# ShunyuYao/DFA-NeRF

Hardware: AMD Instinct MI355X
Metric: rays/sec (whole node) at 450x450, 64c+128f samples (higher is better)
Workload: dtype f16; 1 GPU; Obama head NeRF inference, 450x450, 64+128 hierarchical (configs[1]); H=450, W=450, n_coarse=64, n_fine=128, fields=1, frames=8, parallelism=single GPU

## Files before the change

### dfa-nerf_amd/csrc/dfn_api.hip

```cpp
#include <hip/hip_runtime.h>
#include <algorithm>
#include <climits>
#include <cstdio>
#include <cstdlib>
#include <cstring>
#include <mutex>
#include <string>
#include <utility>
#include <vector>

#include "dfanerf.h"
#include "dfn_layout.h"
#include "dfn_misc.h"
#include "dfn_mlp.h"
#include "dfn_params.h"
#include "dfn_plan.h"
#include "dfn_signal.h"
#include "dfn_train.h"

using namespace dfn;

namespace {

thread_local std::string g_err;
// ... 927 lines not shown
    if (!kept) return fail(DFN_E_ARG, "dfn_encode_signal_bwd_kept: kept is NULL");
    return encode_signal_bwd_impl(aud_params, exp_params, att_params, auds, exps, n_total, frame, smo_size, d_out, g_aud, g_exp,
                                  g_att, false, stream, kept);
}
int dfn_encode_signal_bwd_set(const float* aud_params, const float* exp_params, const float* att_params, const float* auds,
                              const float* exps, int n_total, int frame, int smo_size, const float* d_out, float* g_aud,
                              float* g_exp, float* g_att, void* stream) {
    return encode_signal_bwd_impl(aud_params, exp_params, att_params, auds, exps, n_total, frame, smo_size, d_out, g_aud, g_exp,
                                  g_att, true, stream);
}

static int encode_signal_torso_bwd_impl(const float* att_params, const float* poses, int pose_stride, int n_total, int frame,
                                        int smo_size, const float* d_out, float* g_att, bool set, void* stream) {
    if (!poses || !d_out || n_total <= 0 || (pose_stride != 12 && pose_stride != 16))
        return fail(DFN_E_ARG, "dfn_encode_signal_torso_bwd: bad argument");
    if (smo_ok(smo_size, "dfn_encode_signal_torso_bwd") != DFN_OK) return DFN_E_ARG;
    if (smo_size == 0) return DFN_OK;
    if (!att_params || !g_att) return fail(DFN_E_ARG, "dfn_encode_signal_torso_bwd: attention buffers missing");
    return launched(launch_encode_signal_torso_bwd(att_params, poses, pose_stride, n_total, frame, smo_size, d_out, g_att, set,
                                                   (hipStream_t)stream), "encode_signal_torso_bwd_kernel");
}
int dfn_encode_signal_torso_bwd(const float* att_params, const float* poses, int pose_stride, int n_total, int frame,
                                int smo_size, const float* d_out, float* g_att, void* stream) {
    return encode_signal_torso_bwd_impl(att_params, poses, pose_stride, n_total, frame, smo_size, d_out, g_att, false, stream);
}
int dfn_encode_signal_torso_bwd_set(const float* att_params, const float* poses, int pose_stride, int n_total, int frame,
                                    int smo_size, const float* d_out, float* g_att, void* stream) {
    return encode_signal_torso_bwd_impl(att_params, poses, pose_stride, n_total, frame, smo_size, d_out, g_att, true, stream);
}

static int decoder_impl(int tier, int width, int field, const void* packed, const float* bias, const float* points, const float* dirs,
                        long n, float* feat, float* sigma, float* samples, void* act_T, uint32_t* masks, const char* what, void* stream) {
    ProgramInfo pi;
    program_info(tier, prog_field(field), &pi, width);
    DecoderArgs A{};
    A.wblob = (const char*)packed;
    A.nslab = pi.n_slabs;
    A.field = prog_field(field);
    A.bias = bias;
    A.n_bias = pi.n_bias;
    A.points = points;
    A.dirs = dirs;
    A.n_points = n;
    A.feat = feat;
    A.sigma = sigma;
    A.samples = samples;
    A.act_T = act_T;
    A.masks = masks;
    return launched(launch_decoder(tier, A, (hipStream_t)stream, width), what);
}

int dfn_decoder_fwd(int tier, int field, const void* packed, const float* bias, const float* points,
                    const float* dirs, long n, float* feat, float* sigma, void* stream) {
    int width;
    if (take_width(tier, width, "dfn_decoder_fwd") != DFN_OK) return DFN_E_ARG;
    if (!tier_ok(tier) || !field_ok(field) || !packed || !bias || !points || !dirs || !feat || !sigma)
        return fail(DFN_E_ARG, "dfn_decoder_fwd: bad argument");
    if (n <= 0) return DFN_OK;
    return decoder_impl(tier, width, field, packed, bias, points, dirs, n, feat, sigma, nullptr, nullptr, nullptr, "decoder_kernel", stream);
}

int dfn_decoder_train_fwd(int tier, int field, const void* packed, const float* bias, const float* points,
                          const float* dirs, long n, float* feat, float* sigma, float* samples, void* act_T,
                          uint32_t* masks, void* stream) {
    if (no_width(tier, "dfn_decoder_train_fwd") != DFN_OK) return DFN_E_ARG;
    if (!train_tier_ok(tier) || !train_field_ok(field) || !packed || !bias || !points ||
        !dirs || !feat || !sigma || !samples || !act_T || !masks)
        return fail(DFN_E_ARG, "dfn_decoder_train_fwd: bad argument (tiers f32 / bf16, fields head / torso / listener)");
    if (n <= 0) return DFN_OK;
    const long NP = (n + 31) / 32 * 32;
    if (dfn_train_rows(1, 0) * NP >= (1L << 32)) return fail(DFN_E_ARG, "dfn_decoder_train_fwd: too many points per call");
    return decoder_impl(tier, 256, field, packed, bias, points, dirs, n, feat, sigma, samples, act_T, masks, "decoder_kernel(train)", stream);
}

int dfn_get_rays(int H, int W, float focal, float cx, float cy, const float* c2w_host, float* rays_o,
                 float* rays_d, void* stream) {
    return dfn_get_rays_strided(H, W, 1, focal, cx, cy, c2w_host, rays_o, rays_d, stream);
}

int dfn_get_rays_strided(int H, int W, int stride, float focal, float cx, float cy, const float* c2w_host, float* rays_o,
                         float* rays_d, void* stream) {
    if (H <= 0 || W <= 0 || stride <= 0 || H / stride <= 0 || W / stride <= 0 || !c2w_host || !rays_o || !rays_d)
        return fail(DFN_E_ARG, "dfn_get_rays: bad argument");
    return launched(launch_get_rays(H, W, stride, focal, cx, cy, c2w_host, rays_o, rays_d, (hipStream_t)stream), "get_rays_kernel");
}

int dfn_ndc_rays(int H, int W, float focal, float z_near, const float* rays_o, const float* rays_d, long n,
                 float* out_o, float* out_d, void* stream) {
    if (!rays_o || !rays_d || !out_o || !out_d || n < 0) return fail(DFN_E_ARG, "dfn_ndc_rays: bad argument");
    if (n == 0) return DFN_OK;
    return launched(launch_ndc_rays(H, W, focal, z_near, rays_o, rays_d, n, out_o, out_d, (hipStream_t)stream), "ndc_rays_kernel");
}

int dfn_sample_pdf(const float* bins, const float* weights, long R, int nb, int ns, const float* u, float* samples,
                   void* stream) {
    if (!bins || !weights || !samples || R < 0 || ns <= 0) return fail(DFN_E_ARG, "dfn_sample_pdf: bad argument");
    if (nb < 2 || nb > 256) return fail(DFN_E_ARG, "dfn_sample_pdf: need 2 <= nb <= 256");
    if (R == 0) return DFN_OK;
    return launched(launch_sample_pdf(bins, weights, R, nb, ns, u, samples, (hipStream_t)stream), "sample_pdf_kernel");
}

int dfn_composite(const float* sigma, const float* feat, int K, long N, float* sigma_sum, float* feat_w,
                  void* stream) {
    if (!sigma || !feat || !sigma_sum || !feat_w || K < 1 || N < 0) return fail(DFN_E_ARG, "dfn_composite: bad argument");
    if (N == 0) return DFN_OK;
    return launched(launch_composite(sigma, feat, K, N, sigma_sum, feat_w, (hipStream_t)stream), "composite_kernel");
}

int dfn_volume_weights(const float* z, const float* ray, const float* sigma, long R, int S, float last_dist,
                       float* weights, void* stream) {
    if (!z || !ray || !sigma || !weights || R < 0) return fail(DFN_E_ARG, "dfn_volume_weights: bad argument");
    if (S < 1 || S > 1024) return fail(DFN_E_ARG, "dfn_volume_weights: need 1 <= S <= 1024");
    if (R == 0) return DFN_OK;
    return launched(launch_volume_weights(z, ray, sigma, R, S, last_dist, weights, (hipStream_t)stream), "volume_weights_kernel");
}

int dfn_composite_grad(const float* sigma, const float* feat, int K, long N, const float* d_sigma_sum, const float* d_feat_w,
                       float* d_sigma, float* d_feat, void* stream) {
    if (!sigma || !feat || !d_sigma || !d_feat || K < 1 || N < 0) return fail(DFN_E_ARG, "dfn_composite_grad: bad argument");
    if (N == 0) return DFN_OK;
    return launched(launch_composite_grad(sigma, feat, K, N, d_sigma_sum, d_feat_w, d_sigma, d_feat, (hipStream_t)stream), "composite_grad_kernel");
}

int dfn_volume_weights_grad(const float* z, const float* ray, const float* sigma, long R, int S, float last_dist,
                            const float* d_weights, float* d_sigma, void* stream) {
    if (!z || !ray || !sigma || !d_weights || !d_sigma || R < 0)
        return fail(DFN_E_ARG, "dfn_volume_weights_grad: bad argument");
    if (S < 1 || S > 1024) return fail(DFN_E_ARG, "dfn_volume_weights_grad: need 1 <= S <= 1024");
    if (R == 0) return DFN_OK;
    return launched(launch_volume_weights_grad(z, ray, sigma, R, S, last_dist, d_weights, d_sigma, (hipStream_t)stream), "volume_weights_grad_kernel");
}

int dfn_to8b(const float* x, long n, uint8_t* out, void* stream) {
    if (!x || !out || n < 0) return fail(DFN_E_ARG, "dfn_to8b: bad argument");
    if (n == 0) return DFN_OK;
    return launched(launch_to8b(x, n, out, (hipStream_t)stream), "to8b_kernel");
}

int dfn_debug_mfma_chain(int tier, int lds_reads_per_2, int valu_per_2, const void* fragments, const void* operands_b, int iters,
                         int blocks, float* out, uint64_t* clock, void* stream) {
    if (no_width(tier, "dfn_debug_mfma_chain") != DFN_OK) return DFN_E_ARG;
    if ((tier != DFN_TIER_BF16 && tier != DFN_TIER_F16) || !fragments || !operands_b || !out || !clock || iters <= 0 || blocks <= 0)
        return fail(DFN_E_ARG, "dfn_debug_mfma_chain: bad argument");
    return launched(launch_mfma_chain(tier == DFN_TIER_F16, lds_reads_per_2, valu_per_2, fragments, operands_b, iters, blocks, out,
                                      (unsigned long long*)clock, (hipStream_t)stream),
                    "mfma_chain_kernel (variants: (0, 0) and (2, 4))");
}

int dfn_debug_clock_probe(uint64_t* probe) {
    g_clock_probe = (unsigned long long*)probe;
    return DFN_OK;
}

int dfn_debug_mfma_layout(float* out, void* stream) {
    if (!out) return fail(DFN_E_ARG, "dfn_debug_mfma_layout: bad argument");
    return launched(launch_mfma_probe(out, (hipStream_t)stream), "mfma_probe_kernel");
}

}
```

### dfa-nerf_amd/csrc/dfn_layout.h

```cpp
#pragma once
#include <stdint.h>
#include "dfn_devguard.h"

#if defined(__HIPCC__)
#define DFN_HD __host__ __device__ inline
#else
#define DFN_HD inline
#endif

namespace dfn {

enum Tier : int { TIER_F32 = 0, TIER_BF16 = 1, TIER_F16 = 2, TIER_F16X3 = 3 };
constexpr int TIER_W128 = 0x200, TIER_MASK = 0xff;
constexpr int TIER_AUX = 0x400;
constexpr int TIER_RAYS = 0x800;
constexpr int TIER_E4M3 = 0x100;
DFN_HD constexpr bool tier_trainable(int tier) { return tier == TIER_F32 || tier == TIER_BF16; }
DFN_HD constexpr bool tier_is16(int tier) { return tier == TIER_BF16 || tier == TIER_F16; }
DFN_HD constexpr bool tier_frag16(int tier) { return tier != TIER_F32; }
DFN_HD constexpr int tier_split(int tier) { return tier == TIER_F16X3 ? 2 : 1; }
DFN_HD int tier_E(int tier) { return tier_frag16(tier) ? 8 : 4; }
DFN_HD int tier_UPT(int tier) { return tier_frag16(tier) ? 2 : 4; }
DFN_HD int tier_elem_bytes(int tier) { return tier_frag16(tier) ? 2 : 4; }
constexpr float SPLIT_SCALE = 2048.0f, SPLIT_INV = 1.0f / 2048.0f;

constexpr int FRAG_BYTES = 1024;
constexpr int SLAB_FRAGS = 32;
constexpr int SLAB_BYTES = SLAB_FRAGS * FRAG_BYTES;

DFN_HD int tile_feat(int h, int r) { return (r & 3) + 8 * (r >> 2) + 4 * h; }
DFN_HD void tile_feat_inv(int f, int* h, int* r) {
    *h = (f >> 2) & 1;
    *r = (f & 3) + 4 * (f >> 3);
}
DFN_HD int kslot_to_slot(int tier, int u, int h, int e) {
    const int E = tier_E(tier), UPT = tier_UPT(tier);
    const int t = u / UPT, r = (u % UPT) * E + e;
    return 32 * t + tile_feat(h, r);
}

constexpr int HID = 256, ZDIM = 256, NPE = 60, NPEV = 24, NSIG = 96, NET = 42, DH = 64;

enum ParamId : int {
    P_DE0_W, P_DE0_B, P_DE1_W, P_DE1_B, P_DE2_W, P_DE2_B, P_DE3_W, P_DE3_B, P_DE4_W, P_DE4_B,
    P_DEO_W, P_DEO_B,
    P_DS0_W, P_DS0_B, P_DS1_W, P_DS1_B, P_DS2_W, P_DS2_B, P_DS3_W, P_DS3_B, P_DS4_W, P_DS4_B,
    P_DSO_W, P_DSO_B,
    P_DESK_W, P_DESK_B, P_DSSK_W, P_DSSK_B,
    P_FCIN_W, P_FCIN_B, P_FCINL_W, P_FCINL_B, P_FCINT_W, P_FCINT_B,
    P_FCZ_W, P_FCZ_B,
    P_BLK0_W, P_BLK0_B, P_BLK1_W, P_BLK1_B, P_BLK2_W, P_BLK2_B, P_BLK3_W, P_BLK3_B,
    P_BLK4_W, P_BLK4_B, P_BLK5_W, P_BLK5_B, P_BLK6_W, P_BLK6_B,
    P_FCZSK_W, P_FCZSK_B, P_FCPSK_W, P_FCPSK_B, P_FCPSKL_W, P_FCPSKL_B, P_FCPSKT_W, P_FCPSKT_B,
    P_SIGMA_W, P_SIGMA_B, P_FCZV_W, P_FCZV_B, P_FEATV_W, P_FEATV_B, P_FCV_W, P_FCV_B,
    P_FEATO_W, P_FEATO_B,
    P_COUNT
};

struct ParamShape { int rows, cols; };

DFN_HD constexpr ParamShape param_shape(int id) {
    switch (id) {
    case P_DE0_W: case P_DS0_W: return {DH, NPE + NET};
    case P_DE1_W: case P_DE2_W: case P_DE3_W: case P_DE4_W:
    case P_DS1_W: case P_DS2_W: case P_DS3_W: case P_DS4_W: return {DH, DH};
    case P_DE0_B: case P_DE1_B: case P_DE2_B: case P_DE3_B: case P_DE4_B:
    case P_DS0_B: case P_DS1_B: case P_DS2_B: case P_DS3_B: case P_DS4_B:
    case P_DESK_B: case P_DSSK_B: return {DH, 1};
    case P_DEO_W: return {NPE, DH};
    case P_DEO_B: return {NPE, 1};
    case P_DSO_W: return {NET, DH};
    case P_DSO_B: return {NET, 1};
    case P_DESK_W: return {DH, NPE};
    case P_DSSK_W: return {DH, NET};
    case P_FCIN_W: case P_FCPSK_W: return {HID, NPE + NSIG};
    case P_FCINL_W: case P_FCPSKL_W: return {HID, NPE};
    case P_FCINT_W: case P_FCPSKT_W: return {HID, NPE + NET};
    case P_FCZ_W: case P_FCZSK_W: case P_FCZV_W: return {HID, ZDIM};
    case P_BLK0_W: case P_BLK1_W: case P_BLK2_W: case P_BLK3_W: case P_BLK4_W: case P_BLK5_W:
    case P_BLK6_W: case P_FEATV_W: return {HID, HID};
    case P_SIGMA_W: return {1, HID};
    case P_SIGMA_B: return {1, 1};
    case P_FCV_W: return {HID, NPEV};
    case P_FEATO_W: return {3, HID};
    case P_FEATO_B: return {3, 1};
    default: return {HID, 1};
    }
}

DFN_HD constexpr int param_numel(int id) { return param_shape(id).rows * param_shape(id).cols; }
struct ParamOffsets { int v[P_COUNT + 1]; };
DFN_HD constexpr ParamOffsets make_param_offsets() {
    ParamOffsets t = {};
    int off = 0;
    for (int i = 0; i < P_COUNT; ++i) {
        t.v[i] = off;
        off += param_numel(i);
    }
    t.v[P_COUNT] = off;
    return t;
}
DFN_HD constexpr int param_offset(int id) {
    constexpr ParamOffsets T = make_param_offsets();
    return T.v[id];
}
static_assert(make_param_offsets().v[P_COUNT] == 955242, "flat decoder parameter count");
constexpr int N_DECODER_PARAMS = 955242;

DFN_HD int pe_slot_to_ref(int slot) { return slot < NPE ? slot : -1; }
DFN_HD int view_slot_to_ref(int slot) { return slot < NPEV ? slot : -1; }

enum Field : int { FIELD_HEAD = 0, FIELD_TORSO = 1 };

struct ProgramInfo {
    int n_frags;
    int n_slabs;
    int n_bias;
};

}
```

### dfa-nerf_amd/csrc/dfn_misc.h

```cpp
#pragma once
#include <hip/hip_runtime.h>
#include "dfanerf.h"

namespace dfn {
struct PrepareJobs {
    const float* params;
    int tier;
    const int* plan[4]; void* out[4]; long n[4]; int pack_blocks[4];
    const float* sig[2]; const float* zs[2]; const float* za[2]; float* bias[2]; int nb[2]; int fold_blocks[2];
};
hipError_t launch_prepare(PrepareJobs J, hipStream_t st);
hipError_t launch_pack(const int* plan, const float* params, void* out, long n, int tier, hipStream_t st);
hipError_t launch_fold_bwd(int field, const float* params, const float* sig, const float* zs, const float* za,
                           const float* dbias, float* grad_flat, float* dsig, int n, hipStream_t st);
hipError_t launch_fold_bwd_sig(int field, const float* params, const float* dbias, float* dsig, bool overwrite,
                               hipStream_t st);
int sig_term_elements(int field, int* out);
hipError_t launch_fold(int field, const float* params, const float* sig, const float* zs, const float* za,
                       float* out, int n, hipStream_t st);
hipError_t launch_get_rays(int H, int W, int stride, float focal, float cx, float cy, const float* c2w_host, float* ro,
                           float* rd, hipStream_t st);
hipError_t launch_ndc_rays(int H, int W, float focal, float z_near, const float* ro, const float* rd, long n,
                           float* oo, float* od, hipStream_t st);
hipError_t launch_sample_pdf(const float* bins, const float* weights, long R, int nb, int ns, const float* u,
                             float* out, hipStream_t st);
hipError_t launch_composite(const float* sigma, const float* feat, int K, long N, float* ssum, float* fw,
                            hipStream_t st);
hipError_t launch_volume_weights(const float* z, const float* ray, const float* sigma, long R, int S,
                                 float last_dist, float* w, hipStream_t st);
hipError_t launch_composite_grad(const float* sigma, const float* feat, int K, long N, const float* d_ssum, const float* d_fw,
                                 float* d_sigma, float* d_feat, hipStream_t st);
hipError_t launch_volume_weights_grad(const float* z, const float* ray, const float* sigma, long R, int S, float last_dist,
                                      const float* d_w, float* d_sigma, hipStream_t st);
hipError_t launch_zero_words(unsigned* p, long n, hipStream_t st);
hipError_t launch_mfma_chain(bool f16, int lds2, int valu2, const void* frags, const void* b, int iters, int blocks, float* out,
                             unsigned long long* clk, hipStream_t st);
hipError_t launch_to8b(const float* x, long n, unsigned char* out, hipStream_t st);
hipError_t launch_mfma_probe(float* out, hipStream_t st);
hipError_t launch_adam_multi(const DfnAdamItem* items, const void* chunks, int n_chunks, float lr, double beta1, double beta2,
                             float eps, float bias_c1, float bias_c2_sqrt, hipStream_t st);
}
```

### dfa-nerf_amd/csrc/dfn_misc.hip

```cpp
#include <hip/hip_runtime.h>
#include <algorithm>
#include <hip/hip_bf16.h>
#include "dfn_layout.h"
#include "dfn_mlp.h"
#include "dfn_misc.h"

namespace dfn {

__device__ __forceinline__ void pack_body(const int* __restrict__ plan, const float* __restrict__ params, void* out, long n,
                                          int tier, long i) {
    if (i >= n) return;
    const int src = plan[i];
    const float v = src >= 0 ? params[src] : 0.f;
    if (tier == TIER_BF16) ((__bf16*)out)[i] = (__bf16)v;
    else if (tier == TIER_F16) ((_Float16*)out)[i] = (_Float16)v;
    else if (tier == TIER_F16X3) {
        const _Float16 hi = (_Float16)v;
        ((_Float16*)out)[i] = ((i >> 9) & 1) ? (_Float16)((v - (float)hi) * SPLIT_SCALE) : hi;
    } else ((float*)out)[i] = v;
}
__global__ void pack_kernel(const int* __restrict__ plan, const float* __restrict__ params, void* out, long n,
                            int tier) {
    pack_body(plan, params, out, n, tier, (long)blockIdx.x * blockDim.x + threadIdx.x);
}
// ... 510 lines not shown
            B = b + f * B;
            F = f * F;
        }
    }
    float sF = F, sB = B;
    for (int d = 1; d < 64; d <<= 1) {
        const float oF = __shfl_down(sF, d), oB = __shfl_down(sB, d);
        if (lane + d < 64) { sB = sB + sF * oB; sF = sF * oF; }
    }
    float G = __shfl_down(sB, 1);
    if (lane == 63) G = 0.f;
    for (int k = per < 16 ? per - 1 : 15; k >= 0; --k) {
        const int s = s0 + k;
        if (s < S) {
            const float T = exc * pre[k];
            const float d_alpha = T * (gw[k] - G);
            d_sigma[r * S + s] = sigma[r * S + s] > 0.f ? d_alpha * dist[k] * ex[k] : 0.f;
            G = gw[k] * alpha[k] + __fadd_rn(__fsub_rn(1.0f, alpha[k]), 1e-10f) * G;
        }
    }
}
hipError_t launch_volume_weights_grad(const float* z, const float* ray, const float* sigma, long R, int S, float last_dist,
                                      const float* d_w, float* d_sigma, hipStream_t st) {
    hipLaunchKernelGGL(volume_weights_grad_kernel, dim3((unsigned)((R + 3) / 4)), dim3(256), 0, st, z, ray, sigma, R, S,
                       last_dist, d_w, d_sigma);
    return hipGetLastError();
}

__global__ void zero_words_kernel(unsigned* p, long n) {
    const long n4 = n >> 2;
    uint4* q = (uint4*)p;
    for (long i = (long)blockIdx.x * blockDim.x + threadIdx.x; i < n4; i += (long)gridDim.x * blockDim.x) q[i] = make_uint4(0, 0, 0, 0);
    if (blockIdx.x == 0 && threadIdx.x < (n & 3)) p[(n4 << 2) + threadIdx.x] = 0;
}
hipError_t launch_zero_words(unsigned* p, long n, hipStream_t st) {
    const long n4 = n >> 2;
    const int blocks = (int)std::min<long>(1024, std::max<long>(1, (n4 + 255) / 256));
    hipLaunchKernelGGL(zero_words_kernel, dim3(blocks), dim3(256), 0, st, p, n);
    return hipGetLastError();
}

typedef unsigned pc_u32x4 __attribute__((ext_vector_type(4)));
typedef __bf16 pc_bf16x8 __attribute__((ext_vector_type(8)));
typedef _Float16 pc_f16x8 __attribute__((ext_vector_type(8)));
template <bool F16, int LDS2, int VALU2>
__global__ __launch_bounds__(512) void mfma_chain_kernel(const pc_u32x4* __restrict__ frag_src, const pc_u32x4* __restrict__ b_src,
                                                         int iters, float* out, unsigned long long* clk) {
    extern __shared__ pc_u32x4 pc_slab[];
    const int lane = threadIdx.x & 63;
    for (int i = threadIdx.x; i < 32 * 64; i += 512) pc_slab[i] = frag_src[i];
    __syncthreads();
    pc_u32x4 b[4];
    for (int k = 0; k < 4; ++k) b[k] = b_src[(threadIdx.x * 4 + k) & 4095];
    f32x16 acc0 = {}, acc1 = {};
    pc_u32x4 a0 = pc_slab[lane], a1 = pc_slab[64 + lane];
    unsigned e0 = b[0][0], e1 = b[1][1], e2 = b[2][2], e3 = b[3][3];
    const unsigned long long c0 = __builtin_readcyclecounter(), r0 = __builtin_amdgcn_s_memrealtime();
    for (int it = 0; it < iters; ++it) {
#pragma unroll
        for (int k = 0; k < 16; ++k) {
            const int f = (2 * k) % 32;
            if (LDS2 >= 1) a0 = pc_slab[f * 64 + lane];
            if (LDS2 >= 2) a1 = pc_slab[(f + 1) * 64 + lane];
            if constexpr (F16) {
                acc0 = __builtin_amdgcn_mfma_f32_32x32x16_f16(__builtin_bit_cast(pc_f16x8, a0), __builtin_bit_cast(pc_f16x8, b[k & 3]), acc0, 0, 0, 0);
                acc1 = __builtin_amdgcn_mfma_f32_32x32x16_f16(__builtin_bit_cast(pc_f16x8, a1), __builtin_bit_cast(pc_f16x8, b[(k + 1) & 3]), acc1, 0, 0, 0);
            } else {
                acc0 = __builtin_amdgcn_mfma_f32_32x32x16_bf16(__builtin_bit_cast(pc_bf16x8, a0), __builtin_bit_cast(pc_bf16x8, b[k & 3]), acc0, 0, 0, 0);
                acc1 = __builtin_amdgcn_mfma_f32_32x32x16_bf16(__builtin_bit_cast(pc_bf16x8, a1), __builtin_bit_cast(pc_bf16x8, b[(k + 1) & 3]), acc1, 0, 0, 0);
            }
#pragma unroll
            for (int v = 0; v < VALU2; ++v) {
                unsigned& x = (v & 3) == 0 ? e0 : (v & 3) == 1 ? e1 : (v & 3) == 2 ? e2 : e3;
                if (v & 1) asm volatile("v_pk_max_i16 %0, %1, %2" : "=v"(x) : "v"(x), "v"(e0 ^ e2));
                else asm volatile("v_cvt_pk_bf16_f32 %0, %1, %2" : "=v"(x) : "v"(__builtin_bit_cast(float, x)), "v"(__builtin_bit_cast(float, x ^ 0x3f800000u)));
            }
        }
    }
    const unsigned long long c1 = __builtin_readcyclecounter(), r1 = __builtin_amdgcn_s_memrealtime();
    float sum = 0.f;
    for (int r = 0; r < 16; ++r) sum += acc0[r] + acc1[r];
    out[blockIdx.x * blockDim.x + threadIdx.x] = sum + (float)(e0 ^ e1 ^ e2 ^ e3);
    if (blockIdx.x == gridDim.x / 2 && threadIdx.x == 0) { clk[0] = c1 - c0; clk[1] = r1 - r0; }
}
hipError_t launch_mfma_chain(bool f16, int lds2, int valu2, const void* frags, const void* b, int iters, int blocks, float* out,
                             unsigned long long* clk, hipStream_t st) {
    constexpr int lds = 150 * 1024;
#define PC_GO(F, L, V)                                                                                                        \
    {                                                                                                                         \
        hipError_t e = hipFuncSetAttribute((const void*)mfma_chain_kernel<F, L, V>, hipFuncAttributeMaxDynamicSharedMemorySize, lds); \
        if (e != hipSuccess) return e;                                                                                        \
        hipLaunchKernelGGL((mfma_chain_kernel<F, L, V>), dim3(blocks), dim3(512), lds, st, (const pc_u32x4*)frags,              \
                           (const pc_u32x4*)b, iters, out, clk);                                                              \
        return hipGetLastError();                                                                                             \
    }
    if (lds2 == 0 && valu2 == 0) { if (f16) PC_GO(true, 0, 0) else PC_GO(false, 0, 0) }
    if (lds2 == 2 && valu2 == 4) { if (f16) PC_GO(true, 2, 4) else PC_GO(false, 2, 4) }
    if (lds2 == 1 && valu2 == 4) { if (f16) PC_GO(true, 1, 4) else PC_GO(false, 1, 4) }
    if (lds2 == 0 && valu2 == 4) { if (f16) PC_GO(true, 0, 4) else PC_GO(false, 0, 4) }
    if (lds2 == 2 && valu2 == 0) { if (f16) PC_GO(true, 2, 0) else PC_GO(false, 2, 0) }
    if (lds2 == 1 && valu2 == 2) { if (f16) PC_GO(true, 1, 2) else PC_GO(false, 1, 2) }
    if (lds2 == 2 && valu2 == 2) { if (f16) PC_GO(true, 2, 2) else PC_GO(false, 2, 2) }
#undef PC_GO
    return hipErrorInvalidValue;
}

__global__ void to8b_kernel(const float* x, long n, unsigned char* out) {
    const long i = (long)blockIdx.x * blockDim.x + threadIdx.x;
    if (i >= n) return;
    const float v = fminf(fmaxf(x[i], 0.f), 1.f);
    out[i] = (unsigned char)(int)__fmul_rn(255.0f, v);
}
hipError_t launch_to8b(const float* x, long n, unsigned char* out, hipStream_t st) {
    hipLaunchKernelGGL(to8b_kernel, dim3((unsigned)((n + 255) / 256)), dim3(256), 0, st, x, n, out);
    return hipGetLastError();
}

__global__ void mfma_probe_kernel(float* out) {
    const int lane = threadIdx.x, i = lane & 31, h = lane >> 5;
    {
        bf16x8 a, b;
        for (int e = 0; e < 8; ++e) {
            a[e] = (__bf16)((h == 1 && e == 5) ? (float)(i + 1) : 0.f);
            b[e] = (__bf16)((h == 1 && e == 5) ? (float)(2 * i + 1) : 0.f);
        }
        f32x16 c;
        for (int r = 0; r < 16; ++r) c[r] = 0.f;
        c = __builtin_amdgcn_mfma_f32_32x32x16_bf16(a, b, c, 0, 0, 0);
        for (int r = 0; r < 16; ++r) out[(tile_feat(h, r)) * 32 + i] = c[r];
    }
    {
        const float a = (h == 1) ? (float)(i + 1) : 0.f, b = (h == 1) ? (float)(2 * i + 1) : 0.f;
        f32x16 c;
        for (int r = 0; r < 16; ++r) c[r] = 0.f;
        c = __builtin_amdgcn_mfma_f32_32x32x2f32(a, b, c, 0, 0, 0);
        for (int r = 0; r < 16; ++r) out[1024 + (tile_feat(h, r)) * 32 + i] = c[r];
    }
    {
        f16x8 a, b;
        for (int e = 0; e < 8; ++e) {
            a[e] = (_Float16)((h == 1 && e == 5) ? (float)(i + 1) : 0.f);
            b[e] = (_Float16)((h == 1 && e == 5) ? (float)(2 * i + 1) : 0.f);
        }
        f32x16 c;
        for (int r = 0; r < 16; ++r) c[r] = 0.f;
        c = __builtin_amdgcn_mfma_f32_32x32x16_f16(a, b, c, 0, 0, 0);
        for (int r = 0; r < 16; ++r) out[2048 + (tile_feat(h, r)) * 32 + i] = c[r];
    }
}
hipError_t launch_mfma_probe(float* out, hipStream_t st) {
    hipLaunchKernelGGL(mfma_probe_kernel, dim3(1), dim3(64), 0, st, out);
    return hipGetLastError();
}


__global__ __launch_bounds__(256) void adam_multi_kernel(const DfnAdamItem* items, const int2* chunks, float lr, float beta2,
                                                          float om_beta1, float om_beta2, float eps, float bias_c1,
                                                          float bias_c2_sqrt) {
    const int2 ch = chunks[blockIdx.x];
    const DfnAdamItem it = items[ch.x];
    const long i0 = (long)ch.y * DFN_ADAM_CHUNK;
    const long i1 = (i0 + DFN_ADAM_CHUNK < it.n) ? i0 + DFN_ADAM_CHUNK : it.n;
    const float step_size = lr / bias_c1;
    for (long i = i0 + threadIdx.x; i < i1; i += 256) {
        const float g = it.grad[i];
        float m = it.exp_avg[i], v = it.exp_avg_sq[i];
        m = m + (g - m) * om_beta1;
        v = beta2 * v + om_beta2 * g * g;
        const float denom = sqrtf(v) / bias_c2_sqrt + eps;
        it.param[i] -= step_size * m / denom;
        it.exp_avg[i] = m;
        it.exp_avg_sq[i] = v;
    }
}
hipError_t launch_adam_multi(const DfnAdamItem* items, const void* chunks, int n_chunks, float lr, double beta1, double beta2,
                             float eps, float bias_c1, float bias_c2_sqrt, hipStream_t st) {
    if (n_chunks <= 0) return hipSuccess;
    hipLaunchKernelGGL(adam_multi_kernel, dim3(n_chunks), dim3(256), 0, st, items, (const int2*)chunks, lr, (float)beta2,
                       (float)(1.0 - beta1), (float)(1.0 - beta2), eps, bias_c1, bias_c2_sqrt);
    return hipGetLastError();
}

}
```

### dfa-nerf_amd/csrc/dfn_mlp.h

```cpp
#pragma once
#include <hip/hip_runtime.h>
#include <type_traits>
#include "dfn_layout.h"

namespace dfn {

typedef float f32x16 __attribute__((ext_vector_type(16)));
typedef float f32x4 __attribute__((ext_vector_type(4)));
typedef __bf16 bf16x8 __attribute__((ext_vector_type(8)));
typedef _Float16 f16x8 __attribute__((ext_vector_type(8)));
typedef unsigned u32x4 __attribute__((ext_vector_type(4)));

#define DFN_DEV __device__ __forceinline__
#ifndef DFN_ASM_FETCH
#define DFN_ASM_FETCH 1
#endif
#define DFN_LDS __attribute__((address_space(3)))
typedef DFN_LDS char lds_char;
typedef const __attribute__((address_space(1))) char gchar_c;
typedef DFN_LDS float lds_f32;
typedef DFN_LDS f32x4 lds_f32x4;
typedef DFN_LDS u32x4 lds_u32x4;

template <int TIER> struct TierCfg;
template <> struct TierCfg<TIER_BF16> {
    static constexpr int E = 8, UPT = 2, WAVES = 8, THREADS = 512, LOADS_PER_SLAB = 4;
};
template <> struct TierCfg<TIER_F16> : TierCfg<TIER_BF16> {};
template <> struct TierCfg<TIER_F32> {
    static constexpr int E = 4, UPT = 4, WAVES = 4, THREADS = 256, LOADS_PER_SLAB = 8;
};
template <> struct TierCfg<TIER_F16X3> {
    static constexpr int E = 8, UPT = 2, WAVES = 4, THREADS = 256, LOADS_PER_SLAB = 8;
};

constexpr int RING_SLOTS = 3;
constexpr int RING_BYTES = RING_SLOTS * SLAB_BYTES;

template <int TIER, int NT> struct Vec;
template <int NT> struct Vec<TIER_BF16, NT> {
    bf16x8 u[2 * NT];
    DFN_DEV void set(int L, float x) { u[L >> 3][L & 7] = (__bf16)x; }
    DFN_DEV float get(int L) const { return (float)u[L >> 3][L & 7]; }
};
template <int NT> struct Vec<TIER_F16, NT> {
    f16x8 u[2 * NT];
    DFN_DEV void set(int L, float x) { u[L >> 3][L & 7] = (_Float16)x; }
    DFN_DEV float get(int L) const { return (float)u[L >> 3][L & 7]; }
};
template <int NT> struct Vec<TIER_F32, NT> {
    float v[16 * NT];
    DFN_DEV void set(int L, float x) { v[L] = x; }
    DFN_DEV float get(int L) const { return v[L]; }
};
template <int NT> struct Vec<TIER_F16X3, NT> {
    f16x8 u[2 * NT];
    f16x8 l[2 * NT];
    DFN_DEV void set(int L, float x) {
        const _Float16 hi = (_Float16)x;
        u[L >> 3][L & 7] = hi;
        l[L >> 3][L & 7] = (_Float16)((x - (float)hi) * SPLIT_SCALE);
    }
    DFN_DEV float get(int L) const { return (float)u[L >> 3][L & 7] + (float)l[L >> 3][L & 7] * SPLIT_INV; }
};

struct Stream {
    const char* base0;
    const char* base1;
    int nslab0, nslab1;
    unsigned sched;
    const char* pf_ptr;
    int pf_left;
    int pass;
    const char* next_ptr;
    int next_left;
    unsigned pf_slot;
    unsigned rd_off;
    unsigned rd_slot;
    unsigned rd_vaddr;
    int pf_owed;
#ifdef DFN_TIMING
    unsigned long long t_wait, t_bar, t_issue, t_epi;
#endif
};

template <int TIER, bool ASM = false>
DFN_DEV void stream_issue_piece(const Stream& s, lds_char* ring, int wave, int lane, int k) {
    using C = TierCfg<TIER>;
    const int f = k * C::WAVES + wave;
    if constexpr (ASM) {
        const unsigned dst = __builtin_amdgcn_readfirstlane((unsigned)(unsigned long)ring + s.pf_slot * SLAB_BYTES +
                                                            (unsigned)f * FRAG_BYTES);
        const gchar_c* sb = (const gchar_c*)(s.pf_ptr + f * FRAG_BYTES);
        const unsigned voff = (unsigned)lane * 16u;
        asm volatile("s_mov_b32 m0, %2\n\ts_nop 0\n\tglobal_load_lds_dwordx4 %0, %1" ::"v"(voff), "s"(sb), "s"(dst) : "memory", "m0");
    } else {
        __builtin_amdgcn_global_load_lds(
            (const __attribute__((address_space(1))) void*)(s.pf_ptr + (size_t)lane * 16 + f * FRAG_BYTES),
            (DFN_LDS void*)(ring + s.pf_slot * SLAB_BYTES + f * FRAG_BYTES), 16, 0, 0);
    }
}
DFN_DEV void stream_cursor_next(Stream& s) {
    s.pf_slot = (s.pf_slot + 1 == RING_SLOTS) ? 0u : s.pf_slot + 1;
    const int left = s.pf_left - 1;
    const bool wrap = left == 0;
    s.pf_ptr = wrap ? s.next_ptr : s.pf_ptr + SLAB_BYTES;
    s.pf_left = wrap ? s.next_left : left;
}
DFN_DEV void stream_pass_begin(Stream& s) {
    const int np = s.pass + 1;
    const int f = (np < 32) ? ((s.sched >> np) & 1u) : 0;
    s.next_ptr = f ? s.base1 : s.base0;
    s.next_left = f ? s.nslab1 : s.nslab0;
    s.pass = np;
}
template <int TIER, bool ASM = false>
DFN_DEV void stream_issue(Stream& s, lds_char* ring, int wave, int lane) {
#pragma unroll
    for (int k = 0; k < TierCfg<TIER>::LOADS_PER_SLAB; ++k) stream_issue_piece<TIER, ASM>(s, ring, wave, lane, k);
    stream_cursor_next(s);
}
template <int TIER, bool ASM = false>
DFN_DEV void stream_flush(Stream& s, lds_char* ring, int wave, int lane) {
    constexpr int L = TierCfg<TIER>::LOADS_PER_SLAB;
    if (s.pf_owed > 0) {
        for (int k = L - s.pf_owed; k < L; ++k) stream_issue_piece<TIER, ASM>(s, ring, wave, lane, k);
        stream_cursor_next(s);
        s.pf_owed = 0;
    }
}

template <int TIER, bool ASM = false>
DFN_DEV void stream_begin(Stream& s, lds_char* ring, int wave, int lane) {
    s.pf_ptr = s.base0;
    s.pf_left = s.nslab0;
    s.pass = 0;
    s.next_ptr = s.base0;
    s.next_left = s.nslab0;
    s.pf_slot = 0;
    s.rd_slot = RING_SLOTS - 1;
    s.rd_off = 0;
    s.rd_vaddr = 0;
    s.pf_owed = 0;
    stream_issue<TIER, ASM>(s, ring, wave, lane);
    stream_issue<TIER, ASM>(s, ring, wave, lane);
}

template <int TIER>
DFN_DEV void slab_advance(Stream& s, lds_char* ring, int wave, int lane) {
    using C = TierCfg<TIER>;
#ifdef DFN_TIMING
    const unsigned long long t0 = __builtin_readcyclecounter();
#endif
#ifdef DFN_EXP_VMCNT
    asm volatile("s_waitcnt vmcnt(%0) lgkmcnt(0)" ::"n"(DFN_EXP_VMCNT) : "memory");
#else
    asm volatile("s_waitcnt vmcnt(%0) lgkmcnt(0)" ::"n"(C::LOADS_PER_SLAB) : "memory");
#endif
#ifdef DFN_TIMING
    const unsigned long long t1 = __builtin_readcyclecounter();
#endif
    __builtin_amdgcn_s_barrier();
    asm volatile("" ::: "memory");
#ifdef DFN_TIMING
    const unsigned long long t2 = __builtin_readcyclecounter();
    s.t_wait += t1 - t0; s.t_bar += t2 - t1;
#endif
    s.rd_slot = (s.rd_slot + 1 == RING_SLOTS) ? 0u : s.rd_slot + 1;
    s.rd_off = s.rd_slot * SLAB_BYTES;
    s.rd_vaddr = (unsigned)(unsigned long)ring + (unsigned)lane * 16u + s.rd_off;
    s.pf_owed += C::LOADS_PER_SLAB;
}

struct Rec {
    void* act_T;
    unsigned* masks;
    int rows;
    long pass;
    int mask_dwords;
};

template <bool REC, bool ASMF = false, bool ASMD = false, bool PIPE = false, bool ACT4 = false> struct CtxT {
    static constexpr bool rec_on = REC;
    static constexpr bool act_fp4 = ACT4;
#ifndef DFN_TRAIN_ASMF
#define DFN_TRAIN_ASMF 1
#endif
    static constexpr bool asm_fetch = (ASMF || (REC && DFN_TRAIN_ASMF != 0)) && (!REC || DFN_TRAIN_ASMF != 0) && (DFN_ASM_FETCH != 0);
    static constexpr bool asm_dma = asm_fetch || ASMD;
    static constexpr bool pipe = PIPE && !REC;
    lds_char* ring;
    int wave, lane, half;
    Rec rec;
};
typedef CtxT<false> Ctx;

template <int TIER> struct ActT;
template <> struct ActT<TIER_BF16> { typedef __bf16 type; };
template <> struct ActT<TIER_F16> { typedef _Float16 type; };
template <> struct ActT<TIER_F32> { typedef float type; };

typedef __attribute__((address_space(1))) char gchar;
DFN_DEV gchar* uniform_ptr(const void* p) {
    const unsigned long v = (unsigned long)p;
    const unsigned lo = __builtin_amdgcn_readfirstlane((unsigned)v), hi = __builtin_amdgcn_readfirstlane((unsigned)(v >> 32));
    return (gchar*)(((unsigned long)hi << 32) | lo);
}
#define DFN_GSTORE(INSN, TAIL, ubase, voff, off, x)                                                                            \
    do {                                                                                                                       \
        gchar* ub_ = (ubase) + ((off) & ~4095);                                                                                \
        asm volatile(INSN " %0, %1, %2 offset:%3" TAIL ::"v"(voff), "v"(x), "s"(ub_), "n"((off) & 4095));                      \
    } while (0)
#define DFN_GSTORE_B32_NT(ubase, voff, off, x) DFN_GSTORE("global_store_dword", " nt", ubase, voff, off, x)
#define DFN_GSTORE_B32(ubase, voff, off, x) DFN_GSTORE("global_store_dword", "", ubase, voff, off, x)
#define DFN_GSTORE_B64_NT(ubase, voff, off, x) DFN_GSTORE("global_store_dwordx2", " nt", ubase, voff, off, x)
#define DFN_GSTORE_B128_NT(ubase, voff, off, x) DFN_GSTORE("global_store_dwordx4", " nt\n\ts_nop 1", ubase, voff, off, x)

#ifndef DFN_DPP_ASM
#define DFN_DPP_ASM 1
#endif
constexpr int REC8_SCALE_BYTES = 128;
DFN_HD constexpr long rec8_tile_bytes(int rows) { return (long)rows * 32 + REC8_SCALE_BYTES; }
DFN_HD constexpr int act_row_bytes(bool fp4) { return fp4 ? 16 : 32; }
DFN_HD constexpr long act_tile_bytes(int rows, bool fp4) { return (long)rows * act_row_bytes(fp4) + REC8_SCALE_BYTES; }
struct Q8 {
    float scale;
    unsigned e8;
};
typedef unsigned short u16x2 __attribute__((ext_vector_type(2)));
typedef __bf16 bf16x2_q __attribute__((ext_vector_type(2)));
template <int NT, bool NONNEG = false, bool FP4 = false> DFN_DEV Q8 q8_of_tiles(const Vec<TIER_BF16, NT>& v, int t0, int n) {
    typedef unsigned u32x4_ __attribute__((ext_vector_type(4)));
    u16x2 m4[4] = {{0, 0}, {0, 0}, {0, 0}, {0, 0}};
#pragma unroll
    for (int t = 0; t < NT; ++t)
        if (t >= t0 && t < t0 + n)
#pragma unroll
            for (int h = 0; h < 2; ++h) {
                const u32x4_ q = __builtin_bit_cast(u32x4_, v.u[2 * t + h]);
#pragma unroll
                for (int e = 0; e < 4; ++e) {
                    const unsigned a = NONNEG ? q[e] : q[e] & 0x7fff7fffu;
                    m4[e] = __builtin_elementwise_max(m4[e], __builtin_bit_cast(u16x2, a));
                }
            }
    const u16x2 m = __builtin_elementwise_max(__builtin_elementwise_max(m4[0], m4[1]), __builtin_elementwise_max(m4[2], m4[3]));
    unsigned x = max((unsigned)m[0], (unsigned)m[1]);
#if !DFN_DPP_ASM
    x = max(x, (unsigned)__builtin_amdgcn_update_dpp((int)x, (int)x, 0xB1, 0xf, 0xf, false));
    x = max(x, (unsigned)__builtin_amdgcn_update_dpp((int)x, (int)x, 0x4E, 0xf, 0xf, false));
    x = max(x, (unsigned)__builtin_amdgcn_update_dpp((int)x, (int)x, 0x141, 0xf, 0xf, false));
    x = max(x, (unsigned)__builtin_amdgcn_update_dpp((int)x, (int)x, 0x140, 0xf, 0xf, false));
#else
    asm("s_nop 1\n\tv_max_u32_dpp %0, %0, %0 quad_perm:[1,0,3,2] row_mask:0xf bank_mask:0xf\n\t"
        "s_nop 1\n\tv_max_u32_dpp %0, %0, %0 quad_perm:[2,3,0,1] row_mask:0xf bank_mask:0xf\n\t"
        "s_nop 1\n\tv_max_u32_dpp %0, %0, %0 row_half_mirror row_mask:0xf bank_mask:0xf\n\t"
        "s_nop 1\n\tv_max_u32_dpp %0, %0, %0 row_mirror row_mask:0xf bank_mask:0xf\n\ts_nop 0"
        : "+v"(x));
#endif
    const unsigned a = max(max((unsigned)__builtin_amdgcn_readlane((int)x, 0), (unsigned)__builtin_amdgcn_readlane((int)x, 16)),
                           max((unsigned)__builtin_amdgcn_readlane((int)x, 32), (unsigned)__builtin_amdgcn_readlane((int)x, 48)));
    const unsigned E = a >> 7;
    Q8 q;
#ifdef DFN_REC8_NOAMAX
    q.e8 = 120u;
    q.scale = __builtin_bit_cast(float, q.e8 << 23);
    return q;
#endif
    if constexpr (FP4) {
        const unsigned e = E + ((a & 0x7fu) > 64u ? 1u : 0u);
        q.e8 = e > 3u ? e - 2u : 1u;
    } else {
        q.e8 = E > 8u ? E - 7u : 1u;
    }
    q.scale = __builtin_bit_cast(float, q.e8 << 23);
    return q;
}
template <int NT, class CT>
DFN_DEV void store_tile4(void* arr, int rows, long tile, int row0, const Vec<TIER_BF16, NT>& v, int t, int t_first, const Q8& q,
                         const CT& c) {
    typedef unsigned u32x4_ __attribute__((ext_vector_type(4)));
    typedef unsigned u32x2_ __attribute__((ext_vector_type(2)));
    u32x2_ out;
#pragma unroll
    for (int k = 0; k < 2; ++k) {
        const u32x4_ w = __builtin_bit_cast(u32x4_, v.u[2 * t + k]);
        const unsigned w0 = w[0], w1 = w[1], w2 = w[2], w3 = w[3];
        unsigned o = 0;
        o = __builtin_amdgcn_cvt_scalef32_pk_fp4_bf16(o, __builtin_bit_cast(bf16x2_q, w0), q.scale, 0);
        o = __builtin_amdgcn_cvt_scalef32_pk_fp4_bf16(o, __builtin_bit_cast(bf16x2_q, w1), q.scale, 1);
        o = __builtin_amdgcn_cvt_scalef32_pk_fp4_bf16(o, __builtin_bit_cast(bf16x2_q, w2), q.scale, 2);
        o = __builtin_amdgcn_cvt_scalef32_pk_fp4_bf16(o, __builtin_bit_cast(bf16x2_q, w3), q.scale, 3);
        out[k] = o;
    }
#ifdef DFN_REC8_NOSTORE
    asm volatile("" ::"v"(out));
    return;
#endif
    gchar* ubase = uniform_ptr((char*)arr + tile * act_tile_bytes(rows, true) + (long)row0 * 16);
    const unsigned voff = (unsigned)((c.lane & 31) * 16 + c.half * 8);
    DFN_GSTORE_B64_NT(ubase, voff, (t - t_first) * 512, out);
}
template <int NT, class CT>
DFN_DEV void store_tile_act(void* arr, int rows, long tile, int row0, const Vec<TIER_BF16, NT>& v, int t, int t_first, const Q8& q,
                            const CT& c);
template <class CT>
DFN_DEV void store_scale_act(void* arr, int rows, long tile, int row0, int t0, int t_first, int n, const Q8& q, const CT& c) {
    gchar* sb = uniform_ptr((char*)arr + tile * act_tile_bytes(rows, CT::act_fp4) + (long)rows * act_row_bytes(CT::act_fp4) + (row0 >> 5) + (t0 - t_first));
    if (c.lane < n) *(__attribute__((address_space(1))) unsigned char*)(sb + c.lane) = (unsigned char)q.e8;
}
template <int NT, class CT>
DFN_DEV void store_tile8(void* arr, int rows, long tile, int row0, const Vec<TIER_BF16, NT>& v, int t, int t_first, const Q8& q,
                         const CT& c) {
    typedef unsigned u32x4_ __attribute__((ext_vector_type(4)));
    typedef short s16x2_ __attribute__((ext_vector_type(2)));
    u32x4_ out;
#pragma unroll
    for (int k = 0; k < 4; ++k) {
        const u32x4_ w = __builtin_bit_cast(u32x4_, v.u[2 * t + (k >> 1)]);
        const unsigned w_lo = w[2 * (k & 1)], w_hi = w[2 * (k & 1) + 1];
        s16x2_ o;
        o = __builtin_amdgcn_cvt_scalef32_pk_fp8_bf16(o, __builtin_bit_cast(bf16x2_q, w_lo), q.scale, false);
        o = __builtin_amdgcn_cvt_scalef32_pk_fp8_bf16(o, __builtin_bit_cast(bf16x2_q, w_hi), q.scale, true);
        out[k] = __builtin_bit_cast(unsigned, o);
    }
#ifdef DFN_REC8_NOSTORE
    asm volatile("" ::"v"(out));
    return;
#endif
    gchar* ubase = uniform_ptr((char*)arr + tile * rec8_tile_bytes(rows) + (long)row0 * 32);
    const unsigned voff = (unsigned)((c.lane & 31) * 32 + c.half * 16);
    DFN_GSTORE_B128_NT(ubase, voff, (t - t_first) * 1024, out);
}
template <class CT>
DFN_DEV void store_scale8(void* arr, int rows, long tile, int row0, int t0, int t_first, int n, const Q8& q, const CT& c) {
    gchar* sb = uniform_ptr((char*)arr + tile * rec8_tile_bytes(rows) + (long)rows * 32 + (row0 >> 5) + (t0 - t_first));
    if (c.lane < n) *(__attribute__((address_space(1))) unsigned char*)(sb + c.lane) = (unsigned char)q.e8;
}
template <int NT, class CT>
DFN_DEV void store_tile_act(void* arr, int rows, long tile, int row0, const Vec<TIER_BF16, NT>& v, int t, int t_first, const Q8& q,
                            const CT& c) {
    if constexpr (CT::act_fp4) store_tile4<NT>(arr, rows, tile, row0, v, t, t_first, q, c);
    else store_tile8<NT>(arr, rows, tile, row0, v, t, t_first, q, c);
}
template <int TIER, int NT, class CT, bool ACT = false>
DFN_DEV void store_tiles_T(void* arr, int rows, long tile, int row0, const Vec<TIER, NT>& v, int t0, int n, const CT& c) {
    typedef typename ActT<TIER>::type T;
    gchar* ubase = uniform_ptr((T*)arr + (tile * rows + row0) * 32);
    if constexpr (TIER == TIER_BF16) {
#pragma unroll
        for (int t = 0; t < NT; t += 2)
            if (t >= t0 && t < t0 + n) {
                const int np = (t + 1 < t0 + n && t + 1 < NT) ? 2 : 1;
                const Q8 q = q8_of_tiles<NT, false, ACT && CT::act_fp4>(v, t, np);
                if constexpr (ACT) store_scale_act(arr, rows, tile, row0, t, t0, np, q, c);
                else store_scale8(arr, rows, tile, row0, t, t0, np, q, c);
#pragma unroll
                for (int k = 0; k < 2; ++k)
                    if (k < np && t + k < NT) {
                        if constexpr (ACT) store_tile_act<NT>(arr, rows, tile, row0, v, t + k, t0, q, c);
                        else store_tile8<NT>(arr, rows, tile, row0, v, t + k, t0, q, c);
                    }
            }
    } else {
#ifdef DFN_REC32_NOSTORE
        return;
#endif
#pragma unroll
        for (int L = 0; L < 16 * NT; ++L)
            if ((L >> 4) >= t0 && (L >> 4) < t0 + n) {
                const int f = 32 * ((L >> 4) - t0) + tile_feat(0, L & 15);
                const unsigned voff = (unsigned)(4 * c.half * 32 + (c.lane & 31)) * (unsigned)sizeof(T);
                if constexpr (sizeof(T) == 4) {
                    const float x = v.get(L);
                    DFN_GSTORE_B32_NT(ubase, voff, f * 128, x);
                } else {
                    __builtin_nontemporal_store((T)v.get(L), (__attribute__((address_space(1))) T*)(ubase + f * 32 * (int)sizeof(T) + voff));
                }
            }
    }
}
template <int TIER, int NT, class CT, bool ACT = false>
DFN_DEV void store_vec_T(void* arr, int rows, long tile, int row0, const Vec<TIER, NT>& v, const CT& c) {
    store_tiles_T<TIER, NT, CT, ACT>(arr, rows, tile, row0, v, 0, NT, c);
}
template <int TIER, int NT, class CT>
DFN_DEV void rec_vec(const CT& c, int row0, const Vec<TIER, NT>& v) {
    if constexpr (!CT::rec_on) return;
    else store_vec_T<TIER, NT, CT, true>(c.rec.act_T, c.rec.rows, c.rec.pass, row0, v, c);
}

template <class CT>
DFN_DEV void store_val_T32(void* arr, int rows, long tile, int row0, int L, float x, const CT& c) {
#ifdef DFN_REC32_NOSTORE
    return;
#endif
    gchar* ubase = uniform_ptr((float*)arr + (tile * rows + row0) * 32);
    const int f = 32 * (L >> 4) + tile_feat(0, L & 15);
    const unsigned voff = (unsigned)(4 * c.half * 32 + (c.lane & 31)) * 4u;
    DFN_GSTORE_B32_NT(ubase, voff, f * 128, x);
}

#ifndef DFN_TRUNK_UNROLL
#define DFN_TRUNK_UNROLL 0
#endif
#ifndef DFN_PF_DEPTH
#define DFN_PF_DEPTH 4
#endif
constexpr int PF_DEPTH = DFN_PF_DEPTH;
template <int TIER, class CT> constexpr bool use_asm_fetch() { return tier_is16(TIER) && CT::asm_fetch; }
#ifndef DFN_F32_PIN_FRAGS
#define DFN_F32_PIN_FRAGS 1
#endif
#ifndef DFN_X3_PIN_FRAGS
#define DFN_X3_PIN_FRAGS 1
#endif
#ifndef DFN_F32_ASM_DMA
#define DFN_F32_ASM_DMA 1
#endif
template <int TIER, class CT> constexpr bool use_asm_dma() { return tier_is16(TIER) ? CT::asm_dma : (DFN_F32_ASM_DMA != 0 || CT::asm_dma); }

#define DFN_FRAG_CASE(K)                                                                                      \
    case K:                                                                                                   \
        asm volatile("ds_read_b128 %0, %1 offset:%2" : "=v"(dst) : "v"(vaddr), "n"((K) * FRAG_BYTES) : "memory"); \
        break;
DFN_DEV void frag_read(u32x4& dst, unsigned vaddr, int pos) {
    switch (pos) {
        DFN_FRAG_CASE(0) DFN_FRAG_CASE(1) DFN_FRAG_CASE(2) DFN_FRAG_CASE(3) DFN_FRAG_CASE(4) DFN_FRAG_CASE(5)
        DFN_FRAG_CASE(6) DFN_FRAG_CASE(7) DFN_FRAG_CASE(8) DFN_FRAG_CASE(9) DFN_FRAG_CASE(10) DFN_FRAG_CASE(11)
        DFN_FRAG_CASE(12) DFN_FRAG_CASE(13) DFN_FRAG_CASE(14) DFN_FRAG_CASE(15) DFN_FRAG_CASE(16) DFN_FRAG_CASE(17)
        DFN_FRAG_CASE(18) DFN_FRAG_CASE(19) DFN_FRAG_CASE(20) DFN_FRAG_CASE(21) DFN_FRAG_CASE(22) DFN_FRAG_CASE(23)
        DFN_FRAG_CASE(24) DFN_FRAG_CASE(25) DFN_FRAG_CASE(26) DFN_FRAG_CASE(27) DFN_FRAG_CASE(28) DFN_FRAG_CASE(29)
        DFN_FRAG_CASE(30) DFN_FRAG_CASE(31)
        default: __builtin_unreachable();
    }
}
#undef DFN_FRAG_CASE
DFN_DEV void frag_wait(u32x4& r, int younger) {
    switch (younger) {
        case 0: asm volatile("s_waitcnt lgkmcnt(0)" : "+v"(r)); break;
        case 1: asm volatile("s_waitcnt lgkmcnt(1)" : "+v"(r)); break;
        case 2: asm volatile("s_waitcnt lgkmcnt(2)" : "+v"(r)); break;
        case 3: asm volatile("s_waitcnt lgkmcnt(3)" : "+v"(r)); break;
        case 4: asm volatile("s_waitcnt lgkmcnt(4)" : "+v"(r)); break;
        case 5: asm volatile("s_waitcnt lgkmcnt(5)" : "+v"(r)); break;
        case 6: asm volatile("s_waitcnt lgkmcnt(6)" : "+v"(r)); break;
        default: asm volatile("s_waitcnt lgkmcnt(7)" : "+v"(r)); break;
    }
}
static_assert(PF_DEPTH >= 1 && PF_DEPTH <= 8, "frag_wait covers up to 7 younger reads");
static_assert((PF_DEPTH & (PF_DEPTH - 1)) == 0, "PF_DEPTH must be a power of two");

struct NoHook { DFN_DEV void operator()() const {} };
struct NoSide { DFN_DEV void operator()(int) const {} };

template <int TIER> struct Fetch {
    u32x4 buf[PF_DEPTH];
    template <class CT> DFN_DEV void load(int slot, int fp, Stream& s, const CT& c) { load(slot, fp, s, c, NoHook{}); }
    template <class CT, class H> DFN_DEV void load(int slot, int fp, Stream& s, const CT& c, H&& hook) {
        using C = TierCfg<TIER>;
        constexpr int GAP = SLAB_FRAGS / C::LOADS_PER_SLAB;
        if (fp % SLAB_FRAGS == 0) {
            slab_advance<TIER>(s, c.ring, c.wave, c.lane);
            hook();
        }
        if constexpr (use_asm_fetch<TIER, CT>()) frag_read(buf[slot], s.rd_vaddr, fp % SLAB_FRAGS);
        else buf[slot] = *(const lds_u32x4*)(c.ring + c.lane * 16 + s.rd_off + (fp % SLAB_FRAGS) * FRAG_BYTES);
#ifdef DFN_EXP_DBLLDS
        {
            const u32x4 dup = *(const volatile lds_u32x4*)(c.ring + c.lane * 16 + s.rd_off + ((fp + 1) % SLAB_FRAGS) * FRAG_BYTES);
            asm volatile("" ::"v"(dup));
        }
#endif
        if (fp % GAP == GAP / 2) {
            const int k = (fp % SLAB_FRAGS) / GAP;
            stream_issue_piece<TIER, use_asm_dma<TIER, CT>()>(s, c.ring, c.wave, c.lane, k);
            --s.pf_owed;
            if (k == C::LOADS_PER_SLAB - 1) stream_cursor_next(s);
        }
    }
    template <class CT> DFN_DEV void prime(Stream& s, const CT& c) {
        stream_flush<TIER, use_asm_dma<TIER, CT>()>(s, c.ring, c.wave, c.lane);
        stream_pass_begin(s);
#pragma unroll
        for (int i = 0; i < PF_DEPTH; ++i) load(i, i, s, c);
    }
};

template <int TIER, int G, int KU, int NTB, int TAIL = -1, class CT, class H = NoHook, class SD = NoSide>
DFN_DEV void gemm_group(f32x16 (&acc)[G], const Vec<TIER, NTB>& b, int& f, Fetch<TIER>& fe, Stream& s,
                        const CT& c, H&& hook = H{}, SD&& side = SD{}) {
    if constexpr (TIER == TIER_F16X3) {
        constexpr int D = PF_DEPTH;
        f32x16 accx[G];
#pragma unroll
        for (int g = 0; g < G; ++g)
#pragma unroll
            for (int r = 0; r < 16; ++r) accx[g][r] = 0.f;
#pragma unroll
        for (int ku = 0; ku < KU; ++ku) {
#pragma unroll
            for (int g = 0; g < G; ++g) {
                const int left = ((KU - ku) * G - g) * 2 - 1;
                const u32x4 ah = fe.buf[f % D];
                if (TAIL < 0 || left + TAIL >= D) fe.load(f % D, f + D, s, c, hook);
                ++f;
                const u32x4 al = fe.buf[f % D];
                if (TAIL < 0 || left - 1 + TAIL >= D) fe.load(f % D, f + D, s, c, hook);
                ++f;
                const f16x8 wh = __builtin_bit_cast(f16x8, ah), wl = __builtin_bit_cast(f16x8, al);
                acc[g] = __builtin_amdgcn_mfma_f32_32x32x16_f16(wh, b.u[ku], acc[g], 0, 0, 0);
                accx[g] = __builtin_amdgcn_mfma_f32_32x32x16_f16(wh, b.l[ku], accx[g], 0, 0, 0);
                accx[g] = __builtin_amdgcn_mfma_f32_32x32x16_f16(wl, b.u[ku], accx[g], 0, 0, 0);
#ifdef DFN_GEMM_SCHEDBAR
                __builtin_amdgcn_sched_barrier(DFN_GEMM_SCHEDBAR);
#else
                if constexpr (!CT::rec_on && (DFN_X3_PIN_FRAGS != 0)) __builtin_amdgcn_sched_barrier(0);
#endif
            }
            side(ku);
#ifdef DFN_PIPE_SCHEDBAR
            if constexpr (!std::is_same<typename std::decay<SD>::type, NoSide>::value) __builtin_amdgcn_sched_barrier(0);
#endif
        }
#pragma unroll
        for (int g = 0; g < G; ++g)
#pragma unroll
            for (int r = 0; r < 16; ++r) acc[g][r] = __builtin_fmaf(accx[g][r], SPLIT_INV, acc[g][r]);
    } else {
#pragma unroll
        for (int ku = 0; ku < KU; ++ku) {
#pragma unroll
            for (int g = 0; g < G; ++g) {
                const int left = (KU - ku) * G - g - 1;
                constexpr bool ASM = use_asm_fetch<TIER, CT>();
                if constexpr (ASM) {
                    const int after = (TAIL < 0) ? PF_DEPTH : left + TAIL;
                    frag_wait(fe.buf[f % PF_DEPTH], after < PF_DEPTH - 1 ? after : PF_DEPTH - 1);
                }
                const u32x4 a = fe.buf[f % PF_DEPTH];
                if constexpr (!ASM) {
                    if (TAIL < 0 || left + TAIL >= PF_DEPTH) fe.load(f % PF_DEPTH, f + PF_DEPTH, s, c, hook);
                }
                if constexpr (TIER == TIER_BF16) {
                    acc[g] = __builtin_amdgcn_mfma_f32_32x32x16_bf16(__builtin_bit_cast(bf16x8, a), b.u[ku],
                                                                     acc[g], 0, 0, 0);
                } else if constexpr (TIER == TIER_F16) {
                    acc[g] = __builtin_amdgcn_mfma_f32_32x32x16_f16(__builtin_bit_cast(f16x8, a), b.u[ku],
                                                                    acc[g], 0, 0, 0);
                } else {
                    const f32x4 af = __builtin_bit_cast(f32x4, a);
#pragma unroll
                    for (int e = 0; e < 4; ++e)
                        acc[g] = __builtin_amdgcn_mfma_f32_32x32x2f32(af[e], b.v[4 * ku + e], acc[g], 0, 0, 0);
                }
                if constexpr (ASM) {
                    if (TAIL < 0 || left + TAIL >= PF_DEPTH) fe.load(f % PF_DEPTH, f + PF_DEPTH, s, c, hook);
                }
#ifdef DFN_GEMM_SCHEDBAR
                if constexpr (!ASM) __builtin_amdgcn_sched_barrier(DFN_GEMM_SCHEDBAR);
#else
                if constexpr (!ASM && TIER == TIER_F32 && !CT::rec_on && (DFN_F32_PIN_FRAGS != 0)) __builtin_amdgcn_sched_barrier(0);
#endif
                ++f;
            }
            side(ku);
#ifdef DFN_PIPE_SCHEDBAR
            if constexpr (!std::is_same<typename std::decay<SD>::type, NoSide>::value) __builtin_amdgcn_sched_barrier(0);
#endif
        }
    }
}

DFN_DEV float relu_(float x) { return __builtin_bit_cast(float, max(__builtin_bit_cast(int, x), 0)); }

template <int G>
DFN_DEV void acc_init(f32x16 (&acc)[G], const lds_f32* bias_lds, int half) {
#ifdef DFN_EXP_NOINIT
#pragma unroll
    for (int g = 0; g < G; ++g)
#pragma unroll
        for (int r = 0; r < 16; ++r) acc[g][r] = 0.f;
    return;
#endif
#pragma unroll
    for (int g = 0; g < G; ++g) {
        const lds_f32x4* p = (const lds_f32x4*)(bias_lds + g * 32 + half * 16);
#pragma unroll
        for (int q = 0; q < 4; ++q) {
            const f32x4 v = p[q];
#pragma unroll
            for (int e = 0; e < 4; ++e) acc[g][4 * q + e] = v[e];
        }
    }
}
template <int G>
DFN_DEV void acc_relu_add(f32x16 (&acc)[G], const lds_f32* bias_lds, int half) {
#pragma unroll
    for (int g = 0; g < G; ++g) {
        const lds_f32x4* p = (const lds_f32x4*)(bias_lds + g * 32 + half * 16);
#pragma unroll
        for (int q = 0; q < 4; ++q) {
            const f32x4 v = p[q];
#pragma unroll
            for (int e = 0; e < 4; ++e) acc[g][4 * q + e] = relu_(acc[g][4 * q + e]) + v[e];
        }
    }
}
typedef short s16x2 __attribute__((ext_vector_type(2)));
typedef __bf16 bf16x2 __attribute__((ext_vector_type(2)));
typedef float f32x2 __attribute__((ext_vector_type(2)));
typedef _Float16 f16x2 __attribute__((ext_vector_type(2)));
template <int TIER, int G, int NT, bool RELU>
DFN_DEV void acc_to_vec(const f32x16 (&acc)[G], Vec<TIER, NT>& v, int t0) {
#ifdef DFN_EXP_NOEPI
    {
#pragma unroll
        for (int g = 0; g < G; ++g) v.set(16 * (t0 + g), acc[g][0]);
        return;
    }
#endif
    if constexpr (tier_is16(TIER)) {
        typedef typename std::conditional<TIER == TIER_F16, f16x2, bf16x2>::type pk2;
        typedef typename std::conditional<TIER == TIER_F16, f16x8, bf16x8>::type pk8;
#pragma unroll
        for (int g = 0; g < G; ++g) {
#pragma unroll
            for (int h = 0; h < 2; ++h) {
                unsigned w[4];
#pragma unroll
                for (int e = 0; e < 4; ++e) {
                    const f32x2 x = {acc[g][8 * h + 2 * e], acc[g][8 * h + 2 * e + 1]};
                    const pk2 pk = __builtin_convertvector(x, pk2);
                    if constexpr (RELU) {
                        const s16x2 m = __builtin_elementwise_max(__builtin_bit_cast(s16x2, pk), (s16x2)(0));
                        w[e] = __builtin_bit_cast(unsigned, m);
                    } else {
                        w[e] = __builtin_bit_cast(unsigned, pk);
                    }
                }
                const u32x4 q = {w[0], w[1], w[2], w[3]};
                v.u[2 * (t0 + g) + h] = __builtin_bit_cast(pk8, q);
            }
        }
    } else if constexpr (TIER == TIER_F16X3) {
#pragma unroll
        for (int g = 0; g < G; ++g) {
#pragma unroll
            for (int h = 0; h < 2; ++h) {
                unsigned wh[4], wl[4];
#pragma unroll
                for (int e = 0; e < 4; ++e) {
                    f32x2 x = {acc[g][8 * h + 2 * e], acc[g][8 * h + 2 * e + 1]};
                    if constexpr (RELU) x = f32x2{relu_(x[0]), relu_(x[1])};
                    const f16x2 hi = __builtin_convertvector(x, f16x2);
                    const f32x2 d = (x - __builtin_convertvector(hi, f32x2)) * SPLIT_SCALE;
                    const f16x2 lo = __builtin_convertvector(d, f16x2);
                    wh[e] = __builtin_bit_cast(unsigned, hi);
                    wl[e] = __builtin_bit_cast(unsigned, lo);
                }
                const u32x4 qh = {wh[0], wh[1], wh[2], wh[3]}, ql = {wl[0], wl[1], wl[2], wl[3]};
                v.u[2 * (t0 + g) + h] = __builtin_bit_cast(f16x8, qh);
                v.l[2 * (t0 + g) + h] = __builtin_bit_cast(f16x8, ql);
            }
        }
    } else {
#pragma unroll
        for (int g = 0; g < G; ++g)
#pragma unroll
            for (int r = 0; r < 16; ++r) {
                const float x = RELU ? relu_(acc[g][r]) : acc[g][r];
                v.set(16 * (t0 + g) + r, x);
            }
    }
}

template <int TIER, int NT, class CT>
DFN_DEV void rec_vals(const CT& c, int row0, const Vec<TIER, NT>& out, int t0) {
    if constexpr (CT::rec_on)
        if (row0 >= 0) store_tiles_T<TIER, NT, CT, true>(c.rec.act_T, c.rec.rows, c.rec.pass, row0, out, t0, 2, c);
}
DFN_HD constexpr int mask_pos(int b) { return ((b & 1) << 4) | (b >> 1); }
template <class CT>
DFN_DEV void rec_mask_pair(const CT& c, int mask_dword, const f32x16 (&acc)[2]) {
#ifdef DFN_REC_NOMASK
    return;
#endif
    if constexpr (CT::rec_on) {
        if (mask_dword >= 0) {
            unsigned bits = 0;
#pragma unroll
            for (int b = 0; b < 32; ++b) bits |= (acc[b >> 4][b & 15] > 0.f) ? (1u << mask_pos(b)) : 0u;
            gchar* mb = uniform_ptr(c.rec.masks + ((long)c.rec.pass * c.rec.mask_dwords + mask_dword) * 64);
            DFN_GSTORE_B32(mb, (unsigned)c.lane * 4u, 0, bits);
        }
    }
}

template <int TIER, int NT, class CT>
DFN_DEV void rec_mask_pair_packed(const CT& c, int mask_dword, const Vec<TIER, NT>& out, int t0) {
#ifdef DFN_REC_NOMASK
    return;
#endif
    if constexpr (CT::rec_on && tier_is16(TIER)) {
        if (mask_dword >= 0) {
            typedef unsigned u32x4_ __attribute__((ext_vector_type(4)));
            unsigned b2[2] = {0, 0};
#pragma unroll
            for (int k = 0; k < 4; ++k) {
                const u32x4_ q = __builtin_bit_cast(u32x4_, out.u[2 * t0 + k]);
#pragma unroll
                for (int e = 0; e < 4; ++e) {
                    const unsigned w = q[e];
                    unsigned t;
                    asm("v_pk_min_u16 %0, %1, %2" : "=v"(t) : "v"(w), "s"(0x00010001u));
                    asm("v_lshl_or_b32 %0, %1, %2, %0" : "+v"(b2[e & 1]) : "v"(t), "n"(4 * k + e));
                }
            }
            const unsigned bits = b2[0] | b2[1];
#ifdef DFN_REC_NOMASKSTORE
            asm volatile("" ::"v"(bits));
            return;
#endif
            gchar* mb = uniform_ptr(c.rec.masks + ((long)c.rec.pass * c.rec.mask_dwords + mask_dword) * 64);
            DFN_GSTORE_B32(mb, (unsigned)c.lane * 4u, 0, bits);
        }
    }
}

template <int TIER, int NT, bool RELU>
DFN_DEV void epi_word(const f32x16 (&acc)[2], Vec<TIER, NT>& v, int t0, int w) {
    typedef typename std::conditional<TIER == TIER_F16, f16x2, bf16x2>::type pk2;
    typedef typename std::conditional<TIER == TIER_F16, f16x8, bf16x8>::type pk8;
    const int g = w >> 3, h = (w >> 2) & 1, e = w & 3;
    const f32x2 x = {acc[g][8 * h + 2 * e], acc[g][8 * h + 2 * e + 1]};
    const pk2 pk = __builtin_convertvector(x, pk2);
    unsigned word;
    if constexpr (RELU) word = __builtin_bit_cast(unsigned, __builtin_elementwise_max(__builtin_bit_cast(s16x2, pk), (s16x2)(0)));
    else word = __builtin_bit_cast(unsigned, pk);
    u32x4 q = __builtin_bit_cast(u32x4, v.u[2 * (t0 + g) + h]);
    q[e] = word;
    v.u[2 * (t0 + g) + h] = __builtin_bit_cast(pk8, q);
}
DFN_DEV void init_quad(f32x16 (&acc)[2], const lds_f32* bias_lds, int half, int q) {
    const int g = q >> 2, qq = q & 3;
    const f32x4 v = ((const lds_f32x4*)(bias_lds + g * 32 + half * 16))[qq];
#pragma unroll
    for (int e = 0; e < 4; ++e) acc[g][4 * qq + e] = v[e];
}
template <int TIER, int OT, int KU, bool RELU> struct PipeSide {
    static constexpr int ES = KU / 2 > 0 ? KU / 2 : 1, WPS = (16 + ES - 1) / ES;
    static constexpr int BS = KU - ES > 0 ? KU - ES : 1, QPS = (8 + BS - 1) / BS;
    f32x16 (&other)[2];
    Vec<TIER, OT>& out;
    const lds_f32* bias_next;
    int t_prev;
    int half;
    DFN_DEV void operator()(int ku) const {
        if (t_prev >= 0 && ku < ES) {
#pragma unroll
            for (int w = 0; w < WPS; ++w)
                if (ku * WPS + w < 16) epi_word<TIER, OT, RELU>(other, out, t_prev, ku * WPS + w);
        }
        if (bias_next && ku >= ES) {
#pragma unroll
            for (int q = 0; q < QPS; ++q)
                if ((ku - ES) * QPS + q < 8) init_quad(other, bias_next, half, (ku - ES) * QPS + q);
        }
    }
};
template <int TIER, int OT, int KU, int NTB, bool RELU, class CT>
DFN_DEV void layer_pipe(Vec<TIER, OT>& out, const Vec<TIER, NTB>& in, const lds_f32* bias, int& f, Fetch<TIER>& fe,
                        Stream& s, const CT& c) {
    static_assert(OT % 2 == 0 && KU >= 2, "tile pairs");
    f32x16 acc[2][2];
    acc_init<2>(acc[0], bias, c.half);
#pragma unroll
    for (int tg = 0; tg < OT / 2; ++tg) {
        const int cur = tg & 1;
        const PipeSide<TIER, OT, KU, RELU> side = {acc[cur ^ 1], out, tg + 1 < OT / 2 ? bias + (tg + 1) * 64 : nullptr,
                                                   tg > 0 ? 2 * (tg - 1) : -1, c.half};
        gemm_group<TIER, 2, KU, NTB>(acc[cur], in, f, fe, s, c, NoHook{}, side);
        if (KU - PipeSide<TIER, OT, KU, RELU>::ES < 1 && tg + 1 < OT / 2) acc_init<2>(acc[cur ^ 1], bias + (tg + 1) * 64, c.half);
    }
    acc_to_vec<TIER, 2, OT, RELU>(acc[(OT / 2 - 1) & 1], out, OT - 2);
}

#ifndef DFN_REC_SPREAD
#define DFN_REC_SPREAD 1
#endif
template <int TIER, int OT, int KU, class CT, bool NONNEG> struct RecSide {
    const CT& c;
    const Vec<TIER, OT>& out;
    int rec_row, prev;
    mutable Q8 q;
    static constexpr int S0 = KU > 1 ? 1 : 0, S1 = KU > 2 ? 1 + (KU - 1) / 2 : S0;
    DFN_DEV void operator()(int ku) const {
        if constexpr (CT::rec_on && TIER == TIER_BF16) {
            if (prev < 0 || rec_row < 0) return;
            if (ku == 0) {
                q = q8_of_tiles<OT, NONNEG, CT::act_fp4>(out, 2 * prev, 2);
                store_scale_act(c.rec.act_T, c.rec.rows, c.rec.pass, rec_row, 2 * prev, 0, 2, q, c);
            }
            if (ku == S0) store_tile_act<OT>(c.rec.act_T, c.rec.rows, c.rec.pass, rec_row, out, 2 * prev, 0, q, c);
            if (ku == S1) store_tile_act<OT>(c.rec.act_T, c.rec.rows, c.rec.pass, rec_row, out, 2 * prev + 1, 0, q, c);
        }
    }
};

#ifndef DFN_REC32_SPREAD
#define DFN_REC32_SPREAD 1
#endif
template <int OT, int KU, class CT> struct RecSide32 {
    const CT& c;
    const Vec<TIER_F32, OT>& out;
    int rec_row, mask_dword, prev;
    unsigned& bits;
    static constexpr int VPS = (32 + KU - 1) / KU;
    DFN_DEV void operator()(int ku) const {
        if constexpr (CT::rec_on) {
            if (prev < 0) return;
#pragma unroll
            for (int w = 0; w < VPS; ++w) {
                const int b = ku * VPS + w;
                if (b < 32) {
                    const float x = out.v[32 * prev + b];
                    if (rec_row >= 0) store_val_T32(c.rec.act_T, c.rec.rows, c.rec.pass, rec_row + 64 * prev, b, x, c);
#ifndef DFN_REC_NOMASK
                    if (mask_dword >= 0) bits |= (x > 0.f) ? (1u << mask_pos(b)) : 0u;
#endif
                }
            }
#ifndef DFN_REC_NOMASK
            if (ku == KU - 1 && mask_dword >= 0) {
                gchar* mb = uniform_ptr(c.rec.masks + ((long)c.rec.pass * c.rec.mask_dwords + mask_dword) * 64);
                DFN_GSTORE_B32(mb, (unsigned)c.lane * 4u, 0, bits);
            }
#endif
        }
    }
};

template <int TIER, int OT, int KU, int NTB, bool RELU, class CT>
DFN_DEV void layer(Vec<TIER, OT>& out, const Vec<TIER, NTB>& in, const lds_f32* bias, int& f, Fetch<TIER>& fe,
                   Stream& s, const CT& c, int rec_row = -1, int rec_mask = -1) {
    static_assert(OT % 2 == 0, "tile pairs");
    if constexpr (CT::pipe && tier_is16(TIER) && OT >= 4 && KU >= 2) {
        layer_pipe<TIER, OT, KU, NTB, RELU>(out, in, bias, f, fe, s, c);
        return;
    }
    if constexpr (CT::rec_on && TIER == TIER_F32 && (DFN_REC32_SPREAD != 0) && KU >= 8) {
        unsigned bits = 0;
#pragma unroll
        for (int tg = 0; tg < OT / 2; ++tg) {
            f32x16 acc[2];
            acc_init<2>(acc, bias + tg * 64, c.half);
            bits = 0;
            gemm_group<TIER, 2, KU, NTB>(acc, in, f, fe, s, c, NoHook{},
                                         RecSide32<OT, KU, CT>{c, out, rec_row, (rec_mask < 0 || tg == 0) ? -1 : rec_mask + tg - 1, tg - 1, bits});
            acc_to_vec<TIER, 2, OT, RELU>(acc, out, 2 * tg);
            if (tg == OT / 2 - 1) rec_mask_pair(c, rec_mask < 0 ? -1 : rec_mask + tg, acc);
        }
        if (rec_row >= 0) rec_vals<TIER>(c, rec_row + 64 * (OT / 2 - 1), out, OT - 2);
        return;
    }
    constexpr bool SPREAD = CT::rec_on && TIER == TIER_BF16 && (DFN_REC_SPREAD != 0);
    bool pend = false;
#pragma unroll
    for (int tg = 0; tg < OT / 2; ++tg) {
        f32x16 acc[2];
        acc_init<2>(acc, bias + tg * 64, c.half);
        if constexpr (SPREAD) {
            gemm_group<TIER, 2, KU, NTB>(acc, in, f, fe, s, c, NoHook{}, RecSide<TIER, OT, KU, CT, RELU>{c, out, rec_row, tg - 1, {}});
        } else {
            auto flush = [&] {
                if (pend) rec_vals<TIER>(c, rec_row + 64 * (tg - 1), out, 2 * (tg - 1));
                pend = false;
            };
            gemm_group<TIER, 2, KU, NTB>(acc, in, f, fe, s, c, flush);
            flush();
        }
        acc_to_vec<TIER, 2, OT, RELU>(acc, out, 2 * tg);
        if constexpr (RELU && tier_is16(TIER)) rec_mask_pair_packed<TIER, OT>(c, rec_mask < 0 ? -1 : rec_mask + tg, out, 2 * tg);
        else rec_mask_pair(c, rec_mask < 0 ? -1 : rec_mask + tg, acc);
        pend = CT::rec_on && rec_row >= 0;
    }
    if (pend) rec_vals<TIER>(c, rec_row + 64 * (OT / 2 - 1), out, OT - 2);
}
template <int TIER, int OT, int KU, int NTB, int KU2, int NTB2, class CT>
DFN_DEV void layer_skip(Vec<TIER, OT>& out, const Vec<TIER, NTB>& in, const lds_f32* bias,
                        const Vec<TIER, NTB2>& in2, const lds_f32* bias2, int& f, Fetch<TIER>& fe,
                        Stream& s, const CT& c, int rec_row = -1, int mask_dword0 = -1) {
    bool pend = false;
#pragma unroll
    for (int tg = 0; tg < OT / 2; ++tg) {
        f32x16 acc[2];
        acc_init<2>(acc, bias + tg * 64, c.half);
        auto flush = [&] {
            if (pend) rec_vals<TIER>(c, rec_row + 64 * (tg - 1), out, 2 * (tg - 1));
            pend = false;
        };
        gemm_group<TIER, 2, KU, NTB>(acc, in, f, fe, s, c, flush);
        rec_mask_pair(c, mask_dword0 < 0 ? -1 : mask_dword0 + tg, acc);
        acc_relu_add<2>(acc, bias2 + tg * 64, c.half);
        gemm_group<TIER, 2, KU2, NTB2>(acc, in2, f, fe, s, c, flush);
        flush();
        acc_to_vec<TIER, 2, OT, false>(acc, out, 2 * tg);
        pend = CT::rec_on && rec_row >= 0;
    }
    if (pend) rec_vals<TIER>(c, rec_row + 64 * (OT / 2 - 1), out, OT - 2);
}

__device__ __constant__ float PE_FREQ[10] = {
    (float)(1.0 * 3.14159265358979323846),   (float)(2.0 * 3.14159265358979323846),
    (float)(4.0 * 3.14159265358979323846),   (float)(8.0 * 3.14159265358979323846),
    (float)(16.0 * 3.14159265358979323846),  (float)(32.0 * 3.14159265358979323846),
    (float)(64.0 * 3.14159265358979323846),  (float)(128.0 * 3.14159265358979323846),
    (float)(256.0 * 3.14159265358979323846), (float)(512.0 * 3.14159265358979323846)};

template <int TIER, int NT, int NCOL>
DFN_DEV void posenc(Vec<TIER, NT>& v, const float (&p)[3], int half) {
    const float ph[3] = {p[0] * 0.5f, p[1] * 0.5f, p[2] * 0.5f};
#pragma unroll
    for (int L = 0; L < 16 * NT; ++L) {
        const int c0 = 32 * (L >> 4) + tile_feat(0, L & 15), c1 = c0 + 4;
        const bool ok0 = c0 < NCOL, ok1 = c1 < NCOL;
        if (!ok0 && !ok1) {
            v.set(L, 0.f);
            continue;
        }
        const int o0 = ok0 ? c0 / 6 : 0, o1 = ok1 ? c1 / 6 : 0;
        const int a0 = (c0 % 6) % 3, a1 = (c1 % 6) % 3;
        const bool cos0 = (c0 % 6) >= 3, cos1 = (c1 % 6) >= 3;
        float val;
        if constexpr (TIER == TIER_F32 || TIER == TIER_F16X3) {
            const float x = half ? __fmul_rn(PE_FREQ[o1], ph[a1]) : __fmul_rn(PE_FREQ[o0], ph[a0]);
            if (cos0 == cos1) {
                val = cos0 ? cosf(x) : sinf(x);
            } else {
                float sv, cv;
                sincosf(x, &sv, &cv);
                val = (half ? cos1 : cos0) ? cv : sv;
            }
        } else {
            const float r0 = ph[a0] * ((float)(1 << o0) * 0.5f), r1 = ph[a1] * ((float)(1 << o1) * 0.5f);
            const float q0 = cos0 ? 0.25f : 0.f, q1 = cos1 ? 0.25f : 0.f;
            const float rev = __builtin_amdgcn_fractf(half ? r1 : r0) + (half ? q1 : q0);
            val = __builtin_amdgcn_sinf(rev);
        }
        const bool ok = half ? ok1 : ok0;
        v.set(L, ok ? val : 0.f);
    }
}

template <int TIER, int HT = 8> struct Prog {
    static_assert(HT == 8 || HT == 4, "hidden tiles: 8 (256 wide) or 4 (128 wide)");
    static constexpr int UPT = TierCfg<TIER>::UPT;
    static constexpr int KU_PE = 2 * UPT, KU_VIEW = UPT, KU_ACT = HT * UPT, KU_D = 2 * UPT, KU_PD = 4 * UPT;
    static constexpr int FS = tier_split(TIER);
    static constexpr int F_LAYER = HT * KU_ACT * FS;
    static constexpr int F_TAIL = ((HT + 1) * (KU_ACT + KU_VIEW) + KU_ACT) * FS;
    static constexpr int H_FRAGS = HT * KU_PE * FS + 7 * F_LAYER + HT * KU_PE * FS + F_TAIL;
    static constexpr int H_SLABS = (H_FRAGS + SLAB_FRAGS - 1) / SLAB_FRAGS;
    static constexpr int H_B_IN = 0, H_B_L1 = 256, H_B_SKIP = 5 * 256, H_B_L5 = 6 * 256, H_B_VIEW = 9 * 256,
                         H_B_OUT = 9 * 256 + 288, H_NBIAS = 9 * 256 + 288 + 32;
    static constexpr int F_D = 2 * KU_D * FS;
    static constexpr int T_F_DEFORM = 4 * KU_PE * FS + 10 * F_D + 2 * KU_PE * FS;
    static constexpr int T_FRAGS = T_F_DEFORM + HT * KU_PD * FS + 7 * F_LAYER + HT * KU_PD * FS + F_TAIL;
    static constexpr int T_SLABS = (T_FRAGS + SLAB_FRAGS - 1) / SLAB_FRAGS;
    static constexpr int T_B_E0 = 0, T_B_S0 = 64, T_B_E1 = 128, T_B_S1 = 192, T_B_E2 = 256, T_B_S2 = 320,
                         T_B_E3 = 384, T_B_ESKIP = 448, T_B_S3 = 512, T_B_SSKIP = 576, T_B_E4 = 640,
                         T_B_S4 = 704, T_B_EO = 768, T_B_SO = 832, T_B_IN = 896;
    static constexpr int T_B_L1 = T_B_IN + 256, T_B_SKIP = T_B_IN + 5 * 256, T_B_L5 = T_B_IN + 6 * 256,
                         T_B_VIEW = T_B_IN + 9 * 256, T_B_OUT = T_B_VIEW + 288, T_NBIAS = T_B_OUT + 32;
};

struct DhatRef {
    const volatile lds_f32* p;
    int stride;
    DFN_DEV void load(float (&d)[3]) const {
        d[0] = p[0];
        d[1] = p[stride];
        d[2] = p[2 * stride];
    }
};

struct RecMap {
    static constexpr int T_A0 = 0, T_H = 8 * 256, T_VIEW = 9 * 256, T_ROWS = 9 * 256 + 32;
    static constexpr int TM_A0 = 0, TM_A4R = 4 * 4, TM_A5 = 5 * 4, TM_H = 8 * 4, TM_DWORDS = 9 * 4;
    static constexpr int H_PE = 0, H_TRUNK = 64, H_ROWS = 64 + T_ROWS, H_MTRUNK = 0, H_MDWORDS = TM_DWORDS;
    static constexpr int S_PE = 0, S_D0 = 64, S_PD = 64 + 640, S_TRUNK = S_PD + 128, S_ROWS = S_TRUNK + T_ROWS;
    static constexpr int S_MD0 = 0, S_MTRUNK = 10, S_MDWORDS = 10 + TM_DWORDS;
};

struct MlpOut {
    float sigma, r, g, b;
};

DFN_DEV float sigmoidf_(float x) { return 1.0f / (1.0f + expf(-x)); }

template <int TIER, int NTP, int KUP, int HT, class CT>
DFN_DEV MlpOut mlp_trunk(Vec<TIER, HT>& act, const Vec<TIER, NTP>& pvec, const DhatRef& dref,
                         const lds_f32* bias, int b_l1, int b_skip, int b_l5, int b_view, int b_out,
                         int f_l1, Fetch<TIER>& fe, Stream& s, const CT& c, int r_trunk, int m_trunk) {
    using P = Prog<TIER, HT>;
    Vec<TIER, HT> nxt;
    const auto blk_bias = [&](int k) { return bias + (k < 4 ? b_l1 + 256 * k : b_l5 + 256 * (k - 4)); };
    const auto blk_row = [&](int k) { return r_trunk + RecMap::T_A0 + 256 * (k + 1); };
    const auto blk_mask = [&](int k) { return m_trunk + (k < 4 ? RecMap::TM_A0 + 4 * (k + 1) : RecMap::TM_A5 + 4 * (k - 4)); };
    int f = f_l1;
    constexpr bool SAME_PHASE = P::F_LAYER % SLAB_FRAGS == 0 && (HT * KUP * P::FS) % SLAB_FRAGS == 0;
    static_assert(SAME_PHASE || HT != 8, "the 256-wide program resets the fragment index per layer");
    static_assert(P::F_LAYER % PF_DEPTH == 0 && (HT * KUP * P::FS) % PF_DEPTH == 0, "register ring turns");
    constexpr bool STRAIGHT = (DFN_TRUNK_UNROLL != 0) || !SAME_PHASE;
    if constexpr (!SAME_PHASE) {
        static_assert(!CT::rec_on, "the 128-wide program is inference only (no recorder rows for it)");
#define DFN_PLAIN(OUT, IN, K) layer<TIER, HT, P::KU_ACT, HT, true>(OUT, IN, blk_bias(K), f, fe, s, c)
        DFN_PLAIN(nxt, act, 0);
        DFN_PLAIN(act, nxt, 1);
        DFN_PLAIN(nxt, act, 2);
        layer_skip<TIER, HT, P::KU_ACT, HT, KUP, NTP>(act, nxt, bias + b_l1 + 256 * 3, pvec, bias + b_skip, f, fe, s, c);
        DFN_PLAIN(nxt, act, 4);
        DFN_PLAIN(act, nxt, 5);
        DFN_PLAIN(nxt, act, 6);
#undef DFN_PLAIN
    } else {
#if DFN_TRUNK_UNROLL
#define DFN_PLAIN(OUT, IN, K) f = f_l1; layer<TIER, HT, P::KU_ACT, HT, true>(OUT, IN, blk_bias(K), f, fe, s, c, blk_row(K), blk_mask(K))
    DFN_PLAIN(nxt, act, 0);
    DFN_PLAIN(act, nxt, 1);
    DFN_PLAIN(nxt, act, 2);
    f = f_l1;
    layer_skip<TIER, HT, P::KU_ACT, HT, KUP, NTP>(act, nxt, bias + b_l1 + 256 * 3, pvec, bias + b_skip, f, fe, s, c,
                                                  r_trunk + RecMap::T_A0 + 256 * 4, m_trunk + RecMap::TM_A4R);
    DFN_PLAIN(nxt, act, 4);
    DFN_PLAIN(act, nxt, 5);
    DFN_PLAIN(nxt, act, 6);
#undef DFN_PLAIN
#else
    for (int l = 0; l < 3; ++l) {
        f = f_l1;
        layer<TIER, HT, P::KU_ACT, HT, true>(nxt, act, bias + b_l1 + 256 * l, f, fe, s, c,
                                             r_trunk + RecMap::T_A0 + 256 * (l + 1), m_trunk + RecMap::TM_A0 + 4 * (l + 1));
        act = nxt;
    }
    f = f_l1;
    layer_skip<TIER, HT, P::KU_ACT, HT, KUP, NTP>(nxt, act, bias + b_l1 + 256 * 3, pvec, bias + b_skip, f, fe, s, c,
                                                  r_trunk + RecMap::T_A0 + 256 * 4, m_trunk + RecMap::TM_A4R);
    act = nxt;
    for (int l = 0; l < 3; ++l) {
        f = f_l1;
        layer<TIER, HT, P::KU_ACT, HT, true>(nxt, act, bias + b_l5 + 256 * l, f, fe, s, c,
                                             r_trunk + RecMap::T_A0 + 256 * (5 + l), m_trunk + RecMap::TM_A5 + 4 * l);
        act = nxt;
    }
#endif
    }
    Vec<TIER, HT>& a7 = STRAIGHT ? nxt : act;
    Vec<TIER, HT>& hid = STRAIGHT ? act : nxt;
    MlpOut o;
    {
        Vec<TIER, 1> vview;
        float dhat[3];
        dref.load(dhat);
        posenc<TIER, 1, NPEV>(vview, dhat, c.half);
        rec_vec<TIER, 1>(c, r_trunk + RecMap::T_VIEW, vview);
        bool pend = false;
        int ptg = 0;
        auto flush = [&] {
            if (pend) rec_vals<TIER>(c, r_trunk + RecMap::T_H + 64 * ptg, hid, 2 * ptg);
            pend = false;
        };
#pragma unroll
        for (int tg = 0; tg < HT / 2; ++tg) {
            f32x16 acc[2];
            acc_init<2>(acc, bias + b_view + tg * 64, c.half);
            gemm_group<TIER, 2, P::KU_ACT, HT>(acc, a7, f, fe, s, c, flush);
            gemm_group<TIER, 2, P::KU_VIEW, 1>(acc, vview, f, fe, s, c, flush);
            flush();
            acc_to_vec<TIER, 2, HT, true>(acc, hid, 2 * tg);
            if constexpr (tier_is16(TIER)) rec_mask_pair_packed<TIER, HT>(c, m_trunk + RecMap::TM_H + tg, hid, 2 * tg);
            else rec_mask_pair(c, m_trunk + RecMap::TM_H + tg, acc);
            pend = CT::rec_on;
            ptg = tg;
        }
        f32x16 acc1[1];
        acc_init<1>(acc1, bias + b_view + 256, c.half);
        gemm_group<TIER, 1, P::KU_ACT, HT>(acc1, a7, f, fe, s, c, flush);
        gemm_group<TIER, 1, P::KU_VIEW, 1>(acc1, vview, f, fe, s, c, flush);
        flush();
        o.sigma = acc1[0][0];
    }
    {
        f32x16 acc1[1];
        acc_init<1>(acc1, bias + b_out, c.half);
        gemm_group<TIER, 1, P::KU_ACT, HT, 0>(acc1, hid, f, fe, s, c);
        o.r = sigmoidf_(acc1[0][0]);
        o.g = sigmoidf_(acc1[0][1]);
        o.b = sigmoidf_(acc1[0][2]);
    }
    return o;
}

template <int TIER, int HT = 8, class CT>
DFN_DEV MlpOut mlp_head(const float (&p)[3], const DhatRef& dhat, const lds_f32* bias, Stream& s,
                        const CT& c) {
    using P = Prog<TIER, HT>;
    Vec<TIER, 2> pe;
    posenc<TIER, 2, NPE>(pe, p, c.half);
    rec_vec<TIER, 2>(c, RecMap::H_PE, pe);
    Vec<TIER, HT> act;
    int f = 0;
    Fetch<TIER> fe;
    fe.prime(s, c);
    layer<TIER, HT, P::KU_PE, 2, true>(act, pe, bias + P::H_B_IN, f, fe, s, c, RecMap::H_TRUNK + RecMap::T_A0,
                                      RecMap::H_MTRUNK + RecMap::TM_A0);
    return mlp_trunk<TIER, 2, P::KU_PE>(act, pe, dhat, bias, P::H_B_L1, P::H_B_SKIP, P::H_B_L5, P::H_B_VIEW,
                                        P::H_B_OUT, f % SLAB_FRAGS, fe, s, c, RecMap::H_TRUNK, RecMap::H_MTRUNK);
}

template <int TIER, int HT = 8, class CT>
DFN_DEV MlpOut mlp_torso(const float (&p)[3], const DhatRef& dhat, const lds_f32* bias, Stream& s,
                         const CT& c) {
    using P = Prog<TIER, HT>;
    Vec<TIER, 2> pe;
    posenc<TIER, 2, NPE>(pe, p, c.half);
    rec_vec<TIER, 2>(c, RecMap::S_PE, pe);
    Vec<TIER, 2> ve, vs, vn;
    int f = 0;
    Fetch<TIER> fe;
    fe.prime(s, c);
#define DFN_RD(k) RecMap::S_D0 + 64 * (k), RecMap::S_MD0 + (k)
    layer<TIER, 2, P::KU_PE, 2, true>(ve, pe, bias + P::T_B_E0, f, fe, s, c, DFN_RD(0));
    layer<TIER, 2, P::KU_PE, 2, true>(vs, pe, bias + P::T_B_S0, f, fe, s, c, DFN_RD(1));
    layer<TIER, 2, P::KU_D, 2, true>(vn, ve, bias + P::T_B_E1, f, fe, s, c, DFN_RD(2));  ve = vn;
    layer<TIER, 2, P::KU_D, 2, true>(vn, vs, bias + P::T_B_S1, f, fe, s, c, DFN_RD(3));  vs = vn;
    layer<TIER, 2, P::KU_D, 2, true>(vn, ve, bias + P::T_B_E2, f, fe, s, c, DFN_RD(4));  ve = vn;
    layer<TIER, 2, P::KU_D, 2, true>(vn, vs, bias + P::T_B_S2, f, fe, s, c, DFN_RD(5));  vs = vn;
    layer_skip<TIER, 2, P::KU_D, 2, P::KU_PE, 2>(vn, ve, bias + P::T_B_E3, pe, bias + P::T_B_ESKIP, f, fe, s, c,
                                                 DFN_RD(6));
    ve = vn;
    {
        f32x16 acc[2];
        acc_init<2>(acc, bias + P::T_B_S3, c.half);
        gemm_group<TIER, 2, P::KU_D, 2>(acc, vs, f, fe, s, c);
        rec_mask_pair(c, RecMap::S_MD0 + 7, acc);
        acc_relu_add<2>(acc, bias + P::T_B_SSKIP, c.half);
        acc_to_vec<TIER, 2, 2, false>(acc, vn, 0);
        rec_vals<TIER>(c, RecMap::S_D0 + 64 * 7, vn, 0);
        vs = vn;
    }
    layer<TIER, 2, P::KU_D, 2, true>(vn, ve, bias + P::T_B_E4, f, fe, s, c, DFN_RD(8));  ve = vn;
    layer<TIER, 2, P::KU_D, 2, true>(vn, vs, bias + P::T_B_S4, f, fe, s, c, DFN_RD(9));  vs = vn;
#undef DFN_RD
    Vec<TIER, 4> pd;
    {
        f32x16 acc[2];
        acc_init<2>(acc, bias + P::T_B_EO, c.half);
        gemm_group<TIER, 2, P::KU_D, 2>(acc, ve, f, fe, s, c);
#pragma unroll
        for (int L = 0; L < 32; ++L) pd.set(L, acc[L >> 4][L & 15] + pe.get(L));
        acc_init<2>(acc, bias + P::T_B_SO, c.half);
        gemm_group<TIER, 2, P::KU_D, 2>(acc, vs, f, fe, s, c);
#pragma unroll
        for (int L = 0; L < 32; ++L) pd.set(32 + L, acc[L >> 4][L & 15]);
    }
    rec_vec<TIER, 4>(c, RecMap::S_PD, pd);
    Vec<TIER, HT> act;
    layer<TIER, HT, P::KU_PD, 4, true>(act, pd, bias + P::T_B_IN, f, fe, s, c, RecMap::S_TRUNK + RecMap::T_A0,
                                      RecMap::S_MTRUNK + RecMap::TM_A0);
    return mlp_trunk<TIER, 4, P::KU_PD>(act, pd, dhat, bias, P::T_B_L1, P::T_B_SKIP, P::T_B_L5, P::T_B_VIEW,
                                        P::T_B_OUT, f % SLAB_FRAGS, fe, s, c, RecMap::S_TRUNK, RecMap::S_MTRUNK);
}

}
```

### dfa-nerf_amd/csrc/dfn_render_kernels.h

```cpp
#pragma once
#include <hip/hip_runtime.h>
#include "dfn_layout.h"
#include "dfn_mlp.h"
#include "dfn_params.h"

namespace dfn {

DFN_DEV float mul_(float a, float b) { return __fmul_rn(a, b); }
DFN_DEV float add_(float a, float b) { return __fadd_rn(a, b); }
DFN_DEV float sub_(float a, float b) { return __fsub_rn(a, b); }
DFN_DEV float div_(float a, float b) { return __fdiv_rn(a, b); }

DFN_DEV float linspace01(int i, int n) {
    const float step = div_(1.0f, (float)(n - 1));
    return (i < n / 2) ? mul_(step, (float)i) : fmaf(-step, (float)(n - 1 - i), 1.0f);
}

DFN_DEV void wave_lds_fence() {
    __builtin_amdgcn_fence(__ATOMIC_RELEASE, "wavefront");
    __builtin_amdgcn_wave_barrier();
    __builtin_amdgcn_fence(__ATOMIC_ACQUIRE, "wavefront");
}

DFN_DEV void make_ray(const float* pose, int pix, int W, float focal, float cx, float cy, float (&o)[3],
                      float (&d)[3]) {
    const int y = pix / W, x = pix - y * W;
    const float dx = div_(sub_((float)x, cx), focal);
    const float dy = div_(-sub_((float)y, cy), focal);
    const float dz = -1.0f;
#pragma unroll
    for (int k = 0; k < 3; ++k) {
        d[k] = add_(add_(mul_(dx, pose[4 * k + 0]), mul_(dy, pose[4 * k + 1])), mul_(dz, pose[4 * k + 2]));
        o[k] = pose[4 * k + 3];
    }
}

DFN_DEV float norm3(const float (&d)[3]) {
    return sqrtf(add_(add_(mul_(d[0], d[0]), mul_(d[1], d[1])), mul_(d[2], d[2])));
}

enum RayState : int {
    RS_OH = 0, RS_DH = 3, RS_OT = 6, RS_DT = 9, RS_NH = 12, RS_NT = 13, RS_DHAT_H = 14, RS_DHAT_T = 17,
    RS_BG = 20, RS_TH = 23, RS_TC = 24, RS_RGB_H = 25, RS_RGB_C = 28, RS_COUNT = 32
};

DFN_DEV float integrate_tile(volatile lds_f32* st, int rs_T, int rs_rgb, float sigma, float dist,
                             const float (&col)[3], int n, int lane) {
    const float alpha = sub_(1.0f, expf(-mul_(add_(fmaxf(sigma, 0.f), 1e-6f), dist)));
    const float v = add_(sub_(1.0f, alpha), 1e-10f);
    float inc = v;
#pragma unroll
    for (int dlt = 1; dlt < 32; dlt <<= 1) {
        const float up = __shfl_up(inc, dlt, 32);
        if (n >= dlt) inc *= up;
    }
    float exc = __shfl_up(inc, 1, 32);
    if (n == 0) exc = 1.0f;
    const float T = st[rs_T];
    const float w = alpha * (T * exc);
    float part[3];
#pragma unroll
    for (int k = 0; k < 3; ++k) {
        float x = w * col[k];
#pragma unroll
        for (int dlt = 16; dlt >= 1; dlt >>= 1) x += __shfl_xor(x, dlt, 32);
        part[k] = x;
    }
    const float Tn = T * __shfl(inc, 31, 32);
    const float r0 = st[rs_rgb + 0] + part[0], r1 = st[rs_rgb + 1] + part[1], r2 = st[rs_rgb + 2] + part[2];
    wave_lds_fence();
    if (lane == 0) {
        st[rs_T] = Tn;
        st[rs_rgb + 0] = r0;
        st[rs_rgb + 1] = r1;
        st[rs_rgb + 2] = r2;
    }
    wave_lds_fence();
    return w;
}

template <int TIER, bool TWO = false> struct KernelLds {
    using P = Prog<TIER>;
    static constexpr int BIAS_H = RING_BYTES;
    static constexpr int BIAS_T = BIAS_H + P::H_NBIAS * 4;
    static constexpr int SCRATCH = BIAS_T + P::T_NBIAS * 4;
    static constexpr int Z_ALL = 0, M_OFF = 192, M_STRIDE = 192, RANK8 = 960, STATE = 992, KEEPC = 1024;
    static constexpr int PARK_H = 256;
    static constexpr int SCRATCH_FLOATS = TWO ? 1280 : 1024;
    static constexpr int SCRATCH_PER_WAVE = SCRATCH_FLOATS * 4;
    static constexpr int TOTAL = SCRATCH + TierCfg<TIER>::WAVES * SCRATCH_PER_WAVE;
    static_assert(TOTAL <= 160 * 1024, "LDS budget");
};

template <int TW, bool TWO, int TRAIN, bool ACT4 = true>
__global__ __launch_bounds__(TierCfg<(TW & TIER_MASK)>::THREADS, TierCfg<(TW & TIER_MASK)>::THREADS / 256) void render_kernel(
    const RenderArgs A) {
    constexpr int TIER = TW & TIER_MASK, HT = (TW & TIER_W128) ? 4 : 8;
    static_assert(HT == 8 || TRAIN == 0, "the 128-wide program is inference only");
    constexpr bool AUX = (TW & TIER_AUX) != 0;
    static_assert(!AUX || TRAIN == 0, "the aux outputs are inference only");
    constexpr bool RAYS = (TW & TIER_RAYS) != 0;
    static_assert(!RAYS || TRAIN == 0, "caller-supplied rays are inference only");
    static_assert(!RAYS || !AUX, "no aux form for caller-supplied rays");
    using C = TierCfg<TIER>;
    using L = KernelLds<TIER, TWO>;
    using P = Prog<TIER, HT>;
    extern __shared__ __attribute__((aligned(16))) char smem[];
    const int tid = threadIdx.x;
    const int lane = tid & 63;
    const int wave = __builtin_amdgcn_readfirstlane(tid >> 6);
    const int n = lane & 31;
    const DfnFrame& F = A.frame;
    lds_char* lds = (lds_char*)smem;
#ifndef DFN_PIPE
#define DFN_PIPE 1
#endif
#ifndef DFN_PIPE_TWO
#define DFN_PIPE_TWO 0
#endif
#ifndef DFN_PIPE_TWO_HEAD
#define DFN_PIPE_TWO_HEAD 1
#endif
    typedef CtxT<TRAIN != 0, TRAIN == 0, TRAIN != 0, (DFN_PIPE != 0) && TRAIN == 0 && (!TWO || DFN_PIPE_TWO != 0), TRAIN != 0 && ACT4> CtxK;
    CtxK ctx = {lds, wave, lane, lane >> 5, {}};
    typedef CtxT<TRAIN != 0, TRAIN == 0, TRAIN != 0, (DFN_PIPE != 0) && TRAIN == 0 && (!TWO || DFN_PIPE_TWO != 0 || DFN_PIPE_TWO_HEAD != 0), TRAIN != 0 && ACT4> CtxH;
    constexpr bool two = TWO;
    const int NF = TRAIN == 1 ? 0 : F.n_fine;
    const bool hier = NF > 0;
    const int KF = NF / 32;
    const int NC = F.n_coarse;
    const int S = NC + NF;

    Stream s;
    s.base0 = A.wblob[0];
    s.base1 = A.wblob[1];
    s.nslab0 = A.nslab[0];
    s.nslab1 = A.nslab[1];
    const int KC = NC / 32;
    s.sched = two ? ((0xAAu & ((1u << (2 * KC)) - 1u)) | (((1u << KF) - 1u) << (2 * KC + KF))) : 0u;
#ifdef DFN_TIMING
    s.t_wait = s.t_bar = s.t_issue = 0;
    unsigned long long T_mlp = 0, T_pdf = 0;
    const unsigned long long T_start = __builtin_readcyclecounter();
    const unsigned long long R_start = __builtin_amdgcn_s_memrealtime();
#endif
#ifdef DFN_PRIO_YOUNG
    if (wave >= C::WAVES / 2) __builtin_amdgcn_s_setprio(1);
#endif
    const bool probe = A.clock_probe && blockIdx.x == gridDim.x / 2 && wave == 0;
    unsigned long long probe_c0 = 0, probe_r0 = 0;
    if (probe) {
        probe_c0 = __builtin_readcyclecounter();
        probe_r0 = __builtin_amdgcn_s_memrealtime();
    }
    stream_begin<TIER, use_asm_dma<TIER, CtxK>()>(s, lds, wave, lane);
    {
        lds_f32* bl = (lds_f32*)(lds + L::BIAS_H);
        const int nb = P::H_NBIAS + (TWO ? P::T_NBIAS : 0);
        for (int i = tid; i < nb; i += C::THREADS) bl[i] = A.bias[i];
    }
    const lds_f32* bias_h = (const lds_f32*)(lds + L::BIAS_H);
    const lds_f32* bias_t = (const lds_f32*)(lds + L::BIAS_T);

    lds_f32* scr = (lds_f32*)(lds + L::SCRATCH + wave * L::SCRATCH_PER_WAVE);
    lds_f32* zall = scr + L::Z_ALL;
    lds_f32* zc = zall;
    lds_f32* M = scr + L::M_OFF;
    lds_f32* tmp = M;
    lds_f32* cdf = M + 64;
    lds_f32* zf = M + 128;
    DFN_LDS unsigned char* rank8 = (DFN_LDS unsigned char*)(scr + L::RANK8);
    volatile lds_f32* st = scr + L::STATE;

    const int r_raw = blockIdx.x * C::WAVES + wave;
    const bool valid = r_raw < F.ray_count;
    {
        const int r = valid ? r_raw : F.ray_count - 1;
        int pix;
        if constexpr (RAYS) pix = r;
        else pix = A.pix_index ? A.pix_index[r] : F.ray_begin + r;
        float bg[3];
        if (A.bg_u8) {
#pragma unroll
            for (int k = 0; k < 3; ++k) bg[k] = div_((float)A.bg_u8[(size_t)pix * 3 + k], 255.0f);
        } else {
#pragma unroll
            for (int k = 0; k < 3; ++k) bg[k] = A.bg_f32[(size_t)pix * 3 + k];
        }
        float oh[3], dh[3], ot[3], dt[3];
        float z_near = F.z_near, z_far = F.z_far;
        if constexpr (RAYS) {
            const float* row = A.rays + (size_t)r * (TWO ? 12 : 6);
#pragma unroll
            for (int k = 0; k < 3; ++k) {
                oh[k] = row[k];
                dh[k] = row[3 + k];
                ot[k] = TWO ? row[6 + k] : oh[k];
                dt[k] = TWO ? row[9 + k] : dh[k];
            }
            if (A.bounds) {
                z_near = A.bounds[(size_t)r * 2];
                z_far = A.bounds[(size_t)r * 2 + 1];
            }
        } else {
            make_ray(F.pose, pix, F.W, F.focal, F.cx, F.cy, oh, dh);
            make_ray(F.pose_body, pix, F.W, F.focal, F.cx, F.cy, ot, dt);
        }
        const float nh = norm3(dh), nt = norm3(dt);
        if (lane == 0) {
#pragma unroll
            for (int k = 0; k < 3; ++k) {
                st[RS_OH + k] = oh[k];
                st[RS_DH + k] = dh[k];
                st[RS_OT + k] = ot[k];
                st[RS_DT + k] = dt[k];
                st[RS_DHAT_H + k] = div_(dh[k], nh);
                st[RS_DHAT_T + k] = div_(dt[k], nt);
                st[RS_BG + k] = bg[k];
            }
            st[RS_NH] = nh;
            st[RS_NT] = nt;
            st[RS_TH] = 1.0f;
            st[RS_TC] = 1.0f;
#pragma unroll
            for (int k = 0; k < 3; ++k) st[RS_RGB_H + k] = st[RS_RGB_C + k] = 0.f;
        }
        for (int i = lane; i < NC; i += 64) {
            const float t = linspace01(i, NC);
            zall[i] = add_(mul_(z_near, sub_(1.0f, t)), mul_(z_far, t));
        }
    }
    __syncthreads();

    const bool cbg = F.concate_bg != 0;
    const DhatRef dref_h = {st + RS_DHAT_H, 1}, dref_t = {st + RS_DHAT_T, 1};

    auto head_inputs = [&](float sg_h, float (&fh)[3], bool last, float& s1) {
        if (cbg && last) { fh[0] = st[RS_BG]; fh[1] = st[RS_BG + 1]; fh[2] = st[RS_BG + 2]; }
        s1 = fmaxf(sg_h, 0.f);
        if (cbg && last) s1 = add_(s1, 1e-6f);
    };
    auto combine = [&](float sg_h, const float (&fh)[3], float sg_t, const float (&ft)[3], bool last, float& ssum,
                       float (&fm)[3]) {
        if (cbg && last) sg_t = 0.f;
        const float sh = fmaxf(sg_h, 0.f);
        float stt = fmaxf(sg_t, 0.f);
        if (cbg && last) stt = add_(stt, 1e-6f);
        ssum = add_(sh, stt);
        const float den = (ssum == 0.f) ? 1e-4f : ssum;
        const float wh = div_(sh, den), wt = div_(stt, den);
#pragma unroll
        for (int k = 0; k < 3; ++k) fm[k] = add_(mul_(fh[k], wh), mul_(ft[k], wt));
    };
    float acc_h = 0.f, dep_h = 0.f, acc_c = 0.f, dep_c = 0.f;
    auto aux_tile = [&](float& acc, float& dep, float w, float z, bool fg) {
        float a = fg ? w : 0.f, d = fg ? mul_(w, z) : 0.f;
#pragma unroll
        for (int dlt = 16; dlt >= 1; dlt >>= 1) {
            a += __shfl_xor(a, dlt, 32);
            d += __shfl_xor(d, dlt, 32);
        }
        acc = __int_as_float(__builtin_amdgcn_readfirstlane(__float_as_int(acc + a)));
        dep = __int_as_float(__builtin_amdgcn_readfirstlane(__float_as_int(dep + d)));
    };
    auto composite_merged = [&](bool head_image, float* w_out) {
        for (int t = 0; t < S / 32; ++t) {
            const int si = t * 32 + n;
            const float z = ((volatile lds_f32*)zall)[si];
            const bool last = (si == S - 1);
            const float znext = ((volatile lds_f32*)zall)[last ? si : si + 1];
            const float dz = last ? F.last_dist : sub_(znext, z);
            const volatile lds_f32* Mv = M;
            float sg = Mv[si], col[3] = {Mv[L::M_STRIDE + si], Mv[2 * L::M_STRIDE + si], Mv[3 * L::M_STRIDE + si]};
            float w;
            if (head_image) {
                float s1;
                head_inputs(sg, col, last, s1);
// ... 251 lines not shown
                const float ft[3] = {b.r, b.g, b.b};
                combine(sg_h, fh, b.sigma, ft, last, ssum, fm);
                M[ri] = ssum;
                M[L::M_STRIDE + ri] = fm[0];
                M[2 * L::M_STRIDE + ri] = fm[1];
                M[3 * L::M_STRIDE + ri] = fm[2];
            }
            if (++tile < KF) continue;
            if (lane < NC) {
#pragma unroll
                for (int q = 0; q < 4; ++q) M[q * L::M_STRIDE + rank_c] = keepc[q * 64 + lane];
            }
            wave_lds_fence();
            composite_merged(false, A.w_com);
            break;
        }
    }
#ifdef DFN_TIMING
    if (!AUX && valid && lane == 0 && A.z_out) {
        const unsigned long long T_end = __builtin_readcyclecounter();
        const unsigned long long R_end = __builtin_amdgcn_s_memrealtime();
        float* o = A.z_out + (size_t)r_raw * S + 64;
        o[0] = (float)(T_end - T_start); o[1] = (float)(R_end - R_start); o[2] = (float)T_mlp; o[3] = (float)T_pdf;
        o[4] = (float)s.t_wait; o[5] = (float)s.t_bar; o[6] = (float)s.t_issue; o[7] = (float)wave;
    }
#endif
    if (valid && lane == 0) {
        if (A.out_u8) {
            unsigned char* o8h = (unsigned char*)A.rgb_head;
            unsigned char* o8c = (unsigned char*)A.rgb_com;
#pragma unroll
            for (int k = 0; k < 3; ++k) {
                o8h[(size_t)r_raw * 3 + k] = (unsigned char)(int)mul_(255.0f, fminf(fmaxf(st[RS_RGB_H + k], 0.f), 1.f));
                if (two && o8c)
                    o8c[(size_t)r_raw * 3 + k] = (unsigned char)(int)mul_(255.0f, fminf(fmaxf(st[RS_RGB_C + k], 0.f), 1.f));
            }
        } else {
#pragma unroll
            for (int k = 0; k < 3; ++k) {
                A.rgb_head[(size_t)r_raw * 3 + k] = st[RS_RGB_H + k];
                if (two && A.rgb_com) A.rgb_com[(size_t)r_raw * 3 + k] = st[RS_RGB_C + k];
            }
        }
    }
    if constexpr (AUX) {
        if (valid && lane == 0) {
            if (A.out_u8) {
                if (A.alpha8_head) A.alpha8_head[r_raw] = (unsigned char)(int)mul_(255.0f, fminf(fmaxf(acc_h, 0.f), 1.f));
                if (A.depth16_head)
                    A.depth16_head[r_raw] = (unsigned short)(int)mul_(65535.0f, fminf(fmaxf(div_(dep_h, F.z_far), 0.f), 1.f));
                if (two) {
                    if (A.alpha8_com) A.alpha8_com[r_raw] = (unsigned char)(int)mul_(255.0f, fminf(fmaxf(acc_c, 0.f), 1.f));
                    if (A.depth16_com)
                        A.depth16_com[r_raw] = (unsigned short)(int)mul_(65535.0f, fminf(fmaxf(div_(dep_c, F.z_far), 0.f), 1.f));
                }
            } else {
                A.aux_head[(size_t)r_raw * 2 + 0] = acc_h;
                A.aux_head[(size_t)r_raw * 2 + 1] = dep_h;
                if (two && A.aux_com) {
                    A.aux_com[(size_t)r_raw * 2 + 0] = acc_c;
                    A.aux_com[(size_t)r_raw * 2 + 1] = dep_c;
                }
            }
        }
    }
    if constexpr (TRAIN != 0) {
        if (A.loss.losses) {
            const int total = 3 * F.ray_count;
            if (lane == 0) {
                float se_h = 0.f, se_c = 0.f;
                if (valid) {
                    const int pix = A.pix_index ? A.pix_index[r_raw] : F.ray_begin + r_raw;
                    const float scale = div_(2.0f, (float)total);
                    unsigned char th[3], tc[3];
#pragma unroll
                    for (int k = 0; k < 3; ++k) {
                        th[k] = A.loss.img_head[(size_t)pix * 3 + k];
                        tc[k] = A.loss.img_com[(size_t)pix * 3 + k];
                    }
#pragma unroll
                    for (int k = 0; k < 3; ++k) {
                        const float dh = sub_(st[RS_RGB_H + k], div_((float)th[k], 255.0f));
                        const float dc = sub_(st[RS_RGB_C + k], div_((float)tc[k], 255.0f));
                        se_h = add_(se_h, mul_(dh, dh));
                        se_c = add_(se_c, mul_(dc, dc));
                        A.loss.d_rgb_head[(size_t)r_raw * 3 + k] = mul_(scale, dh);
                        A.loss.d_rgb_com[(size_t)r_raw * 3 + k] = mul_(scale, dc);
                    }
                }
                st[RS_TH] = se_h;
                st[RS_TC] = se_c;
            }
            __syncthreads();
            const int nwg = gridDim.x;
            float* part = A.loss.workspace;
            unsigned* ticket = (unsigned*)(A.loss.workspace + 2 * nwg);
            volatile lds_f32* st0 = (lds_f32*)(lds + L::SCRATCH) + L::STATE;
            if (tid == 0) {
                float a = 0.f, b = 0.f;
                for (int w = 0; w < C::WAVES; ++w) {
                    volatile lds_f32* sw = (lds_f32*)(lds + L::SCRATCH + w * L::SCRATCH_PER_WAVE) + L::STATE;
                    a = add_(a, sw[RS_TH]);
                    b = add_(b, sw[RS_TC]);
                }
                part[blockIdx.x] = a;
                part[nwg + blockIdx.x] = b;
                __threadfence();
                st0[RS_NH] = (atomicAdd(ticket, 1u) == (unsigned)nwg - 1u) ? 1.0f : 0.0f;
            }
            __syncthreads();
            if (st0[RS_NH] != 0.0f && wave == 0) {
                __threadfence();
                float a = 0.f, b = 0.f;
                for (int k = lane; k < nwg; k += 64) {
                    a = add_(a, ((volatile float*)part)[k]);
                    b = add_(b, ((volatile float*)part)[nwg + k]);
                }
#pragma unroll
                for (int m = 32; m >= 1; m >>= 1) {
                    a = add_(a, __shfl_xor(a, m, 64));
                    b = add_(b, __shfl_xor(b, m, 64));
                }
                if (lane == 0) {
                    const float lh = div_(a, (float)total), lc = div_(b, (float)total);
                    A.loss.losses[0] = lh;
                    A.loss.losses[1] = lc;
                    A.loss.losses[2] = add_(lc, lh);
                    *ticket = 0u;
                }
            }
        }
    }
    if (probe && lane == 0) {
        A.clock_probe[0] = __builtin_readcyclecounter() - probe_c0;
        A.clock_probe[1] = __builtin_amdgcn_s_memrealtime() - probe_r0;
    }
    asm volatile("s_waitcnt vmcnt(0)" ::: "memory");
}

template <int TW, bool TORSO, bool REC = false>
__global__ __launch_bounds__(TierCfg<(TW & TIER_MASK)>::THREADS, TierCfg<(TW & TIER_MASK)>::THREADS / 256) void decoder_kernel(
    const DecoderArgs A) {
    constexpr int TIER = TW & TIER_MASK, HT = (TW & TIER_W128) ? 4 : 8;
    static_assert(HT == 8 || !REC, "the 128-wide program is inference only");
    using C = TierCfg<TIER>;
    using L = KernelLds<TIER>;
    extern __shared__ __attribute__((aligned(16))) char smem[];
    const int tid = threadIdx.x;
    const int lane = tid & 63;
    const int wave = __builtin_amdgcn_readfirstlane(tid >> 6);
    const int n = lane & 31;
    lds_char* lds = (lds_char*)smem;
    typedef CtxT<REC, HT != 8, REC> CtxD;
    CtxD ctx = {lds, wave, lane, lane >> 5, {}};
    ctx.rec.act_T = nullptr;
    ctx.rec.masks = nullptr;

    Stream s;
    s.base0 = s.base1 = A.wblob;
    s.nslab0 = s.nslab1 = A.nslab;
    s.sched = 0;
    stream_begin<TIER, use_asm_dma<TIER, CtxD>()>(s, lds, wave, lane);
    constexpr bool torso = TORSO;
    lds_f32* bias_l = (lds_f32*)(lds + (torso ? L::BIAS_T : L::BIAS_H));
    for (int i = tid; i < A.n_bias; i += C::THREADS) bias_l[i] = A.bias[i];

    lds_f32* scr = (lds_f32*)(lds + L::SCRATCH + wave * L::SCRATCH_PER_WAVE);
    volatile lds_f32* dl = scr + 544;
    const long n_tiles = (A.n_points + 31) / 32;
    const long tile_raw = (long)blockIdx.x * C::WAVES + wave;
    const long tile = tile_raw < n_tiles ? tile_raw : n_tiles - 1;
    const long pt_raw = tile * 32 + n;
    const long pt = pt_raw < A.n_points ? pt_raw : A.n_points - 1;
    float p[3];
    {
        float d[3];
#pragma unroll
        for (int k = 0; k < 3; ++k) {
            p[k] = A.points[pt * 3 + k];
            d[k] = A.dirs[pt * 3 + k];
        }
        const float nd = norm3(d);
#pragma unroll
        for (int k = 0; k < 3; ++k) dl[64 * k + lane] = div_(d[k], nd);
    }
    __syncthreads();
    const DhatRef dref = {dl + lane, 64};
    if constexpr (REC)
        ctx.rec = {A.act_T, A.masks, torso ? RecMap::S_ROWS : RecMap::H_ROWS, tile, torso ? RecMap::S_MDWORDS : RecMap::H_MDWORDS};
    MlpOut o;
    if constexpr (torso) o = mlp_torso<TIER, HT>(p, dref, bias_l, s, ctx);
    else o = mlp_head<TIER, HT>(p, dref, bias_l, s, ctx);
    if (lane < 32) {
        if (tile_raw < n_tiles && pt_raw < A.n_points) {
            A.feat[pt_raw * 3 + 0] = o.r;
            A.feat[pt_raw * 3 + 1] = o.g;
            A.feat[pt_raw * 3 + 2] = o.b;
            A.sigma[pt_raw] = o.sigma;
        }
        if constexpr (REC) {
            float* so = A.samples + pt_raw * 8 + (torso ? 4 : 0);
            so[0] = o.sigma; so[1] = o.r; so[2] = o.g; so[3] = o.b;
        }
    }
    asm volatile("s_waitcnt vmcnt(0)" ::: "memory");
}

template <typename K> static hipError_t set_lds(K kernel, int lds) {
    return hipFuncSetAttribute((const void*)kernel, hipFuncAttributeMaxDynamicSharedMemorySize, lds);
}
template <int TIER, bool TWO, int TRAIN = 0, bool ACT4 = true, int W128 = 0> static hipError_t launch_render_t(const RenderArgs& A, hipStream_t st) {
    static_assert((W128 & ~(TIER_W128 | TIER_AUX | TIER_RAYS)) == 0 && (W128 == 0 || TRAIN == 0), "widths / aux / rays: inference only");
    using C = TierCfg<TIER>;
    const int lds = KernelLds<TIER, TWO>::TOTAL;
    static bool attr_done = false;
    if (!attr_done) {
        hipError_t e = set_lds(render_kernel<TIER | W128, TWO, TRAIN, ACT4>, lds);
        if (e != hipSuccess) return e;
        attr_done = true;
    }
    const int blocks = (A.frame.ray_count + C::WAVES - 1) / C::WAVES;
    hipLaunchKernelGGL((render_kernel<TIER | W128, TWO, TRAIN, ACT4>), dim3(blocks), dim3(C::THREADS), lds, st, A);
    return hipGetLastError();
}
template <int TIER, bool TORSO, bool REC = false, int W128 = 0> static hipError_t launch_decoder_t(const DecoderArgs& A, hipStream_t st) {
    static_assert(W128 == 0 || (W128 == TIER_W128 && !REC), "widths");
    using C = TierCfg<TIER>;
    const int lds = KernelLds<TIER>::TOTAL;
    static bool attr_done = false;
    if (!attr_done) {
        hipError_t e = set_lds(decoder_kernel<TIER | W128, TORSO, REC>, lds);
        if (e != hipSuccess) return e;
        attr_done = true;
    }
    const long per_block = (long)C::WAVES * 32;
    const int blocks = (int)((A.n_points + per_block - 1) / per_block);
    hipLaunchKernelGGL((decoder_kernel<TIER | W128, TORSO, REC>), dim3(blocks), dim3(C::THREADS), lds, st, A);
    return hipGetLastError();
}

template <int TIER, int FLAGS> hipError_t launch_render_tier(const RenderArgs& A, hipStream_t st) {
    if constexpr (FLAGS == TIER_E4M3) {
        return A.frame.n_fine > 0 ? launch_render_t<TIER, true, 2, false>(A, st) : launch_render_t<TIER, true, 1, false>(A, st);
    } else {
        if constexpr ((FLAGS & TIER_RAYS) != 0) {
            if (!A.use_rays || A.aux || !A.rays) return hipErrorInvalidValue;
        } else if constexpr ((FLAGS & TIER_AUX) != 0) {
            if (A.samples_out || !A.aux) return hipErrorInvalidValue;
        } else if (A.samples_out) {
            if constexpr (FLAGS == 0 && tier_trainable(TIER))
                return A.frame.n_fine > 0 ? launch_render_t<TIER, true, 2>(A, st) : launch_render_t<TIER, true, 1>(A, st);
            else return hipErrorInvalidValue;
        }
        return A.frame.fields == 2 ? launch_render_t<TIER, true, 0, true, FLAGS>(A, st) : launch_render_t<TIER, false, 0, true, FLAGS>(A, st);
    }
}
template <int TIER, int FLAGS> hipError_t launch_decoder_tier(const DecoderArgs& A, hipStream_t st) {
    if constexpr ((FLAGS & ~TIER_W128) != 0) return hipErrorInvalidValue;
    else {
        if (A.act_T) {
            if constexpr (FLAGS == 0 && tier_trainable(TIER))
                return A.field == FIELD_TORSO ? launch_decoder_t<TIER, true, true>(A, st) : launch_decoder_t<TIER, false, true>(A, st);
            else return hipErrorInvalidValue;
        }
        return A.field == FIELD_TORSO ? launch_decoder_t<TIER, true, false, FLAGS>(A, st) : launch_decoder_t<TIER, false, false, FLAGS>(A, st);
    }
}

}
```

### dfa-nerf_amd/dfanerf/_lib.py

```python
import ctypes as C
import os

import torch

_HERE = os.path.dirname(os.path.abspath(__file__))
LIB_PATH = os.environ.get("DFN_LIB") or os.path.join(_HERE, "libdfanerf.so")

TIER_F32, TIER_BF16, TIER_F16, TIER_F16X3 = 0, 1, 2, 3
TRAIN_ACT_E4M3 = 0x100
WIDTH_128 = 0x200
WIDTH_128_TIERS = (TIER_F32, TIER_F16, TIER_F16X3)
ACT_E4M3, ACT_E2M1 = 0, 1
FIELD_HEAD, FIELD_TORSO, FIELD_LISTENER = 0, 1, 2
N_DECODER_PARAMS = 955242
DECODER_UNUSED_PREFIXES = ("expnet.", "w2lnet.")


class DfnFrame(C.Structure):
    _fields_ = [("pose", C.c_float * 12), ("pose_body", C.c_float * 12), ("H", C.c_int), ("W", C.c_int),
                ("focal", C.c_float), ("cx", C.c_float), ("cy", C.c_float), ("z_near", C.c_float),
                ("z_far", C.c_float), ("last_dist", C.c_float), ("ray_begin", C.c_int), ("ray_count", C.c_int),
                ("n_coarse", C.c_int), ("n_fine", C.c_int), ("fields", C.c_int), ("concate_bg", C.c_int)]


class DfnTrainLoss(C.Structure):
    _fields_ = [("img_head", C.c_void_p), ("img_com", C.c_void_p), ("d_rgb_head", C.c_void_p), ("d_rgb_com", C.c_void_p),
                ("losses", C.c_void_p), ("workspace", C.c_void_p)]


class DfnError(RuntimeError):
    pass


def _load():
    if not os.path.exists(LIB_PATH):
        raise ImportError(
            f"{LIB_PATH} not found: build the HIP library first "
            f"(python -c 'import __graft_entry__ as g; g.build()' or dfa-nerf_amd/build.sh). "
            f"There is no CPU fallback for the render path.")
    lib = C.CDLL(LIB_PATH)
    vp, fp, ip, lg, i32 = C.c_void_p, C.c_void_p, C.c_void_p, C.c_long, C.c_int
    sig = {
        "dfn_last_error": (C.c_char_p, []),
        "dfn_version": (C.c_char_p, []),
        "dfn_packed_bytes": (lg, [i32, i32]),
        "dfn_pack_weights": (i32, [i32, i32, fp, vp, vp]),
        "dfn_pack_plan": (lg, [i32, i32, ip, lg]),
        "dfn_bias_floats": (lg, [i32, i32]),
        "dfn_encode_signal": (i32, [fp, fp, fp, fp, fp, i32, ip, i32, i32, fp, vp]),
        "dfn_encode_signal_torso": (i32, [fp, fp, i32, i32, ip, i32, i32, fp, vp]),
        "dfn_encode_signal_bwd": (i32, [fp, fp, fp, fp, fp, i32, i32, i32, fp, fp, fp, fp, vp]),
        "dfn_encode_signal_torso_bwd": (i32, [fp, fp, i32, i32, i32, i32, fp, fp, vp]),
        "dfn_encode_signal_bwd_set": (i32, [fp, fp, fp, fp, fp, i32, i32, i32, fp, fp, fp, fp, vp]),
        "dfn_encode_signal_keep": (i32, [fp, fp, fp, fp, fp, i32, ip, i32, fp, fp, vp]),
        "dfn_encode_signal_keep_floats": (lg, []),
        "dfn_encode_signal_bwd_kept": (i32, [fp, fp, fp, fp, fp, i32, i32, i32, fp, fp, fp, fp, fp, vp]),
        "dfn_encode_signal_torso_bwd_set": (i32, [fp, fp, i32, i32, i32, i32, fp, fp, vp]),
        "dfn_fold_bias": (i32, [i32, i32, fp, fp, fp, fp, fp, vp]),
        "dfn_fold_bias_bwd": (i32, [i32, i32, fp, fp, fp, fp, fp, fp, fp, vp]),
        "dfn_adam_multi": (i32, [vp, vp, i32, C.c_float, C.c_double, C.c_double, C.c_float, C.c_float, C.c_float, vp]),
        "dfn_render_fwd": (i32, [i32, C.POINTER(DfnFrame), vp, vp, fp, fp, fp, vp, ip, fp, fp, fp, fp, fp, vp]),
        "dfn_render_fwd_u8": (i32, [i32, C.POINTER(DfnFrame), vp, vp, fp, fp, fp, vp, ip, vp, vp, vp]),
        "dfn_render_fwd_aux": (i32, [i32, C.POINTER(DfnFrame), vp, vp, fp, fp, fp, vp, ip, fp, fp, fp, fp, vp]),
        "dfn_render_fwd_u8_aux": (i32, [i32, C.POINTER(DfnFrame), vp, vp, fp, fp, fp, vp, ip, vp, vp, vp, vp, vp, vp, vp]),
        "dfn_render_rays_fwd": (i32, [i32, C.POINTER(DfnFrame), vp, vp, fp, fp, fp, fp, fp, vp, fp, fp, fp, fp, fp, vp]),
        "dfn_render_rays_fwd_u8": (i32, [i32, C.POINTER(DfnFrame), vp, vp, fp, fp, fp, fp, fp, vp, vp, vp, vp]),
        "dfn_decoder_fwd": (i32, [i32, i32, vp, fp, fp, fp, lg, fp, fp, vp]),
        "dfn_decoder_train_fwd": (i32, [i32, i32, vp, fp, fp, fp, lg, fp, fp, fp, vp, vp, vp]),
        "dfn_get_rays": (i32, [i32, i32, C.c_float, C.c_float, C.c_float, C.POINTER(C.c_float), fp, fp, vp]),
        "dfn_get_rays_strided": (i32, [i32, i32, i32, C.c_float, C.c_float, C.c_float, C.POINTER(C.c_float), fp, fp, vp]),
        "dfn_ndc_rays": (i32, [i32, i32, C.c_float, C.c_float, fp, fp, lg, fp, fp, vp]),
        "dfn_sample_pdf": (i32, [fp, fp, lg, i32, i32, fp, fp, vp]),
        "dfn_composite": (i32, [fp, fp, i32, lg, fp, fp, vp]),
        "dfn_volume_weights": (i32, [fp, fp, fp, lg, i32, C.c_float, fp, vp]),
        "dfn_composite_grad": (i32, [fp, fp, i32, lg, fp, fp, fp, fp, vp]),
        "dfn_volume_weights_grad": (i32, [fp, fp, fp, lg, i32, C.c_float, fp, fp, vp]),
        "dfn_to8b": (i32, [fp, lg, vp, vp]),
        "dfn_debug_mfma_layout": (i32, [fp, vp]),
        "dfn_debug_clock_probe": (i32, [vp]),
        "dfn_debug_mfma_chain": (i32, [i32, i32, i32, vp, vp, i32, i32, fp, vp, vp]),
        "dfn_train_rows": (lg, [i32, i32]),
        "dfn_packed_bwd_bytes": (lg, [i32, i32]),
        "dfn_pack_weights_bwd": (i32, [i32, i32, fp, vp, vp]),
        "dfn_train_prepare": (i32, [i32, fp, fp, fp, fp, fp, vp, vp, vp, vp, fp, fp, vp]),
        "dfn_train_fwd": (i32, [i32, C.POINTER(DfnFrame), vp, vp, fp, fp, fp, vp, ip, fp, fp, fp, vp, vp, vp, vp, vp]),
        "dfn_train_fwd_hier": (i32, [i32, C.POINTER(DfnFrame), vp, vp, fp, fp, fp, vp, ip, fp, fp, fp, vp, vp, vp, vp, fp, vp, vp]),
        "dfn_train_loss_floats": (lg, [i32]),
        "dfn_train_fwd_loss": (i32, [i32, C.POINTER(DfnFrame), vp, vp, fp, fp, fp, vp, ip, fp, fp, fp, vp, vp, vp, vp,
                                     C.POINTER(DfnTrainLoss), vp]),
        "dfn_train_fwd_hier_loss": (i32, [i32, C.POINTER(DfnFrame), vp, vp, fp, fp, fp, vp, ip, fp, fp, fp, vp, vp, vp, vp, fp,
                                          vp, C.POINTER(DfnTrainLoss), vp]),
        "dfn_composite_bwd_hier": (i32, [C.POINTER(DfnFrame), ip, fp, vp, fp, fp, vp, fp, fp, fp, vp]),
        "dfn_composite_bwd_hier_z": (i32, [C.POINTER(DfnFrame), ip, fp, vp, fp, fp, vp, fp, fp, fp, fp, lg, vp]),
        "dfn_sample_pixels": (i32, [i32, i32, i32, i32, ip, C.c_uint64, C.c_uint64, ip, ip, vp]),
        "dfn_mse_loss_u8": (i32, [fp, fp, vp, vp, ip, i32, fp, fp, fp, vp]),
        "dfn_composite_bwd": (i32, [C.POINTER(DfnFrame), ip, fp, vp, fp, fp, fp, fp, vp]),
        "dfn_composite_bwd_z": (i32, [C.POINTER(DfnFrame), ip, fp, vp, fp, fp, fp, fp, fp, lg, vp]),
        "dfn_mlp_bwd": (i32, [i32, i32, vp, fp, fp, vp, lg, vp, vp]),
        "dfn_wgrad_plan": (lg, [i32, i32, ip, lg]),
        "dfn_weight_grad": (i32, [i32, i32, vp, vp, lg, fp, fp, vp]),
        "dfn_weight_bias_grad": (i32, [i32, i32, vp, vp, lg, fp, fp, fp, vp]),
        "dfn_weight_bias_grad_fmt": (i32, [i32, i32, i32, vp, vp, lg, fp, fp, fp, vp]),
        "dfn_weight_bias_grad_partials": (i32, [i32, i32, i32, vp, vp, lg, fp, fp, vp]),
        "dfn_weight_bias_grad_reduce": (i32, [i32, i32, lg, fp, fp, fp, vp]),
        "dfn_weight_bias_grad_partials_part": (i32, [i32, i32, i32, vp, vp, lg, fp, fp, i32, vp]),
        "dfn_bias_grad": (i32, [i32, i32, vp, lg, fp, fp, vp]),
        "dfn_zero_async": (i32, [vp, lg, vp]),
        "dfn_signal_grad": (i32, [i32, i32, fp, vp, lg, fp, fp, vp]),
    }
    for name, (res, args) in sig.items():
        fn = getattr(lib, name)
        fn.restype = res
        fn.argtypes = args
    if b"DEV" in lib.dfn_version() and not os.environ.get("DFN_LIB"):
        raise ImportError(f"{LIB_PATH} was built with developer switches ({lib.dfn_version().decode()}): rebuild it with "
                          "dfa-nerf_amd/build.sh --clean (no DFN_EXTRA_FLAGS), or select a variant library explicitly with DFN_LIB")
    return lib, sorted(sig)


lib, EXPORTS = _load()


def check(rc, what=""):
    if rc < 0:
        raise DfnError(f"{what}: {lib.dfn_last_error().decode()} (code {rc})")
    return rc


def pack_plan(tier, field):
    import numpy as np
    n = check(lib.dfn_pack_plan(tier, field, None, 0), "dfn_pack_plan")
    out = np.empty(n, np.int32)
    check(lib.dfn_pack_plan(tier, field, out.ctypes.data, n), "dfn_pack_plan")
    return out
```

### dfa-nerf_amd/dfanerf/engine.py

```python
import ctypes as C
import os

import numpy as np
import torch

from . import _lib
from ._lib import (DECODER_UNUSED_PREFIXES, DfnFrame, FIELD_HEAD, FIELD_LISTENER, FIELD_TORSO, N_DECODER_PARAMS, TIER_BF16, TIER_F16, TIER_F16X3,
                   TIER_F32, WIDTH_128, WIDTH_128_TIERS, check, lib)

TIERS = {"f32": TIER_F32, "bf16": TIER_BF16, "f16": TIER_F16, "f16x3": TIER_F16X3, TIER_F32: TIER_F32, TIER_BF16: TIER_BF16,
         TIER_F16: TIER_F16, TIER_F16X3: TIER_F16X3}
F16_RANGE_TIERS = (TIER_F16, TIER_F16X3)


def tier_name(tier):
    t = TIERS[tier]
    return next(k for k, v in TIERS.items() if isinstance(k, str) and v == t)


def _stream():
    return C.c_void_p(torch.cuda.current_stream().cuda_stream)


def _ptr(t):
# ... 308 lines not shown
        pix_index = pix_index.to(device=dev, dtype=torch.int32).contiguous()
    net = (packed.tier_arg, C.byref(frame), _ptr(packed.packed[FIELD_HEAD]), _ptr(packed.packed.get(FIELD_TORSO)) if two else None,
           _ptr(bias), bias_t)
    return net, bgs, pix_index, out_h, out_c


def render(packed, bias, frame, bg, pix_index=None, want_weights=False, out_head=None, out_com=None, want_z=False,
           want_aux=False, rays=None, bounds=None):
    if rays is None and bounds is not None:
        raise ValueError("render: bounds are per-ray depth ranges of supplied rays (rays=)")
    if rays is not None:
        rays, bounds = _rays_inputs("render", packed, frame, bg, rays, bounds, pix_index=pix_index, want_aux=want_aux)
    if want_aux and (want_weights or want_z):
        raise ValueError("render: want_aux cannot be combined with want_weights / want_z (dfn_render_fwd_aux has no per-sample "
                         "outputs; call render() twice, or reduce the weights yourself)")
    net, bgs, pix_index, rgb_h, rgb_c = _launch_inputs("render", torch.float32, packed, bias, frame, bg, pix_index, out_head, out_com)
    dev, n, two = packed.device, frame.ray_count, frame.fields == 2
    if want_aux:
        aux_h = torch.empty(n, 2, dtype=torch.float32, device=dev)
        aux_c = torch.empty(n, 2, dtype=torch.float32, device=dev) if two else None
        check(lib.dfn_render_fwd_aux(*net, *bgs, _ptr(pix_index), _ptr(rgb_h), _ptr(rgb_c), _ptr(aux_h), _ptr(aux_c), _stream()),
              "dfn_render_fwd_aux")
        return rgb_h, rgb_c, aux_h, aux_c
    S = frame.n_coarse + frame.n_fine
    w_h = torch.empty(n, S, dtype=torch.float32, device=dev) if want_weights else None
    w_c = torch.empty(n, S, dtype=torch.float32, device=dev) if (want_weights and two) else None
    z_v = torch.empty(n, S, dtype=torch.float32, device=dev) if want_z else None
    outs = (_ptr(rgb_h), _ptr(rgb_c), _ptr(w_h), _ptr(w_c), _ptr(z_v), _stream())
    if rays is not None:
        check(lib.dfn_render_rays_fwd(*net, _ptr(rays), _ptr(bounds), *bgs, *outs), "dfn_render_rays_fwd")
    else:
        check(lib.dfn_render_fwd(*net, *bgs, _ptr(pix_index), *outs), "dfn_render_fwd")
    out = (rgb_h, rgb_c)
    if want_weights:
        out += (w_h, w_c)
    if want_z:
        out += (z_v,)
    return out


def render_u8(packed, bias, frame, bg, pix_index=None, out_head=None, out_com=None, want_alpha=False, want_depth=False,
              rays=None, bounds=None):
    if rays is None and bounds is not None:
        raise ValueError("render_u8: bounds are per-ray depth ranges of supplied rays (rays=)")
    if rays is not None:
        rays, bounds = _rays_inputs("render_u8", packed, frame, bg, rays, bounds, pix_index=pix_index, want_alpha=want_alpha,
                                    want_depth=want_depth)
    net, bgs, pix_index, out_h, out_c = _launch_inputs("render_u8", torch.uint8, packed, bias, frame, bg, pix_index, out_head, out_com)
    dev, n, two = packed.device, frame.ray_count, frame.fields == 2
    if want_alpha or want_depth:
        a_h = torch.empty(n, dtype=torch.uint8, device=dev) if want_alpha else None
        a_c = torch.empty(n, dtype=torch.uint8, device=dev) if (want_alpha and two) else None
        d_h = torch.empty(n, dtype=torch.uint16, device=dev) if want_depth else None
        d_c = torch.empty(n, dtype=torch.uint16, device=dev) if (want_depth and two) else None
        check(lib.dfn_render_fwd_u8_aux(*net, *bgs, _ptr(pix_index), _ptr(out_h), _ptr(out_c), _ptr(a_h), _ptr(a_c), _ptr(d_h),
                                        _ptr(d_c), _stream()), "dfn_render_fwd_u8_aux")
        out = (out_h, out_c)
        if want_alpha:
            out += (a_h, a_c)
        if want_depth:
            out += (d_h, d_c)
        return out
    if rays is not None:
        check(lib.dfn_render_rays_fwd_u8(*net, _ptr(rays), _ptr(bounds), *bgs, _ptr(out_h), _ptr(out_c), _stream()), "dfn_render_rays_fwd_u8")
    else:
        check(lib.dfn_render_fwd_u8(*net, *bgs, _ptr(pix_index), _ptr(out_h), _ptr(out_c), _stream()), "dfn_render_fwd_u8")
    return out_h, out_c


def decoder_forward(packed, field, bias, points, dirs):
    dev = packed.device
    pts = _f32c(points, dev).reshape(-1, 3)
    dr = _f32c(dirs, dev).reshape(-1, 3)
    n = pts.shape[0]
    feat = torch.empty(n, 3, dtype=torch.float32, device=dev)
    sigma = torch.empty(n, dtype=torch.float32, device=dev)
    if n == 0:
        return feat, sigma
    check(lib.dfn_decoder_fwd(packed.tier_arg, field, _ptr(packed.packed[field]), _ptr(bias), _ptr(pts), _ptr(dr), n,
                              _ptr(feat), _ptr(sigma), _stream()), "dfn_decoder_fwd")
    return feat, sigma


def get_rays(H, W, focal, c2w, cx=None, cy=None, device="cuda", stride=1):
    require_gpu()
    cx = W * .5 if cx is None else cx
    cy = H * .5 if cy is None else cy
    m = (c2w.detach().cpu().numpy() if isinstance(c2w, torch.Tensor) else np.asarray(c2w)).astype(np.float32)
    m = np.ascontiguousarray(m[:3, :4]).reshape(-1)
    arr = (C.c_float * 12)(*[float(v) for v in m])
    stride = int(stride)
    ro = torch.empty(H // stride, W // stride, 3, dtype=torch.float32, device=device)
    rd = torch.empty(H // stride, W // stride, 3, dtype=torch.float32, device=device)
    check(lib.dfn_get_rays_strided(int(H), int(W), stride, float(focal), float(cx), float(cy), arr, _ptr(ro), _ptr(rd), _stream()),
          "dfn_get_rays")
    return ro, rd


def ndc_rays(H, W, focal, near, rays_o, rays_d):
    dev = rays_o.device
    ro, rd = _f32c(rays_o, dev), _f32c(rays_d, dev)
    oo, od = torch.empty_like(ro), torch.empty_like(rd)
    check(lib.dfn_ndc_rays(int(H), int(W), float(focal), float(near), _ptr(ro), _ptr(rd), ro.numel() // 3, _ptr(oo),
                           _ptr(od), _stream()), "dfn_ndc_rays")
    return oo, od


def sample_pdf(bins, weights, n_samples, det=False, u=None):
    dev = bins.device
    b, w = _f32c(bins, dev), _f32c(weights, dev)
    R, nb = b.shape
    if u is None and not det:
        u = torch.rand(R, n_samples, device=dev)
    uu = None if u is None else _f32c(u, dev)
    out = torch.empty(R, n_samples, dtype=torch.float32, device=dev)
    if R == 0:
        return out
    check(lib.dfn_sample_pdf(_ptr(b), _ptr(w), R, nb, int(n_samples), _ptr(uu), _ptr(out), _stream()),
          "dfn_sample_pdf")
    return out


def composite(sigma, feat):
    dev = sigma.device
    K = sigma.shape[0]
    s, f = _f32c(sigma, dev), _f32c(feat, dev)
    N = s.numel() // K
    ss = torch.empty(s.shape[1:], dtype=torch.float32, device=dev)
    fw = torch.empty(f.shape[1:], dtype=torch.float32, device=dev)
    check(lib.dfn_composite(_ptr(s), _ptr(f), K, N, _ptr(ss), _ptr(fw), _stream()), "dfn_composite")
    return ss, fw


def volume_weights(z_vals, ray_vector, sigma, last_dist=1e10):
    dev = sigma.device
    S = z_vals.shape[-1]
    z = _f32c(z_vals, dev).reshape(-1, S)
    r = _f32c(ray_vector, dev).reshape(-1, 3)
    sg = _f32c(sigma, dev).reshape(-1, S)
    w = torch.empty_like(sg)
    check(lib.dfn_volume_weights(_ptr(z), _ptr(r), _ptr(sg), z.shape[0], S, float(last_dist), _ptr(w), _stream()),
          "dfn_volume_weights")
    return w.reshape(sigma.shape)


def to8b(x):
    dev = x.device
    xx = _f32c(x, dev)
    out = torch.empty(xx.shape, dtype=torch.uint8, device=dev)
    check(lib.dfn_to8b(_ptr(xx), xx.numel(), _ptr(out), _stream()), "dfn_to8b")
    return out


def mfma_layout_probe(device="cuda"):
    out = torch.zeros(3, 32, 32, dtype=torch.float32, device=device)
    check(lib.dfn_debug_mfma_layout(_ptr(out), _stream()), "dfn_debug_mfma_layout")
    return out
```

### include/dfanerf.h

```cpp
#ifndef DFANERF_H_
#define DFANERF_H_

#include <stddef.h>
#include <stdint.h>

#ifdef __cplusplus
extern "C" {
#endif

#define DFN_OK 0
#define DFN_E_ARG (-1)
#define DFN_E_HIP (-2)
#define DFN_E_SIZE (-3)

#define DFN_TIER_F32 0
#define DFN_TIER_BF16 1
#define DFN_TIER_F16 2
#define DFN_TIER_F16X3 3

#define DFN_WIDTH_128 0x200

#define DFN_FIELD_HEAD 0
#define DFN_FIELD_TORSO 1
#define DFN_FIELD_LISTENER 2
// ... 40 lines not shown
int dfn_encode_signal_keep(const float* aud_params, const float* exp_params, const float* att_params, const float* auds,
                           const float* exps, int n_total, const int32_t* frame_id, int smo_size, float* out, float* keep,
                           void* stream);
long dfn_encode_signal_keep_floats(void);
int dfn_encode_signal_bwd_kept(const float* aud_params, const float* exp_params, const float* att_params, const float* auds,
                               const float* exps, int n_total, int frame, int smo_size, const float* d_out, const float* kept,
                               float* g_aud, float* g_exp, float* g_att, void* stream);
int dfn_encode_signal_bwd_set(const float* aud_params, const float* exp_params, const float* att_params, const float* auds,
                              const float* exps, int n_total, int frame, int smo_size, const float* d_out, float* g_aud,
                              float* g_exp, float* g_att, void* stream);
int dfn_encode_signal_torso_bwd_set(const float* att_params, const float* poses, int pose_stride, int n_total, int frame,
                                    int smo_size, const float* d_out, float* g_att, void* stream);

int dfn_render_fwd(int tier, const DfnFrame* frame, const void* packed_head, const void* packed_torso,
                   const float* bias_head, const float* bias_torso, const float* bg_f32,
                   const uint8_t* bg_u8, const int32_t* pix_index, float* rgb_head, float* rgb_com,
                   float* weights_head, float* weights_com, float* z_vals, void* stream);

int dfn_render_fwd_u8(int tier, const DfnFrame* frame, const void* packed_head, const void* packed_torso,
                      const float* bias_head, const float* bias_torso, const float* bg_f32, const uint8_t* bg_u8,
                      const int32_t* pix_index, uint8_t* rgb8_head, uint8_t* rgb8_com, void* stream);

int dfn_render_fwd_aux(int tier, const DfnFrame* frame, const void* packed_head, const void* packed_torso,
                       const float* bias_head, const float* bias_torso, const float* bg_f32, const uint8_t* bg_u8,
                       const int32_t* pix_index, float* rgb_head, float* rgb_com, float* aux_head, float* aux_com, void* stream);

int dfn_render_fwd_u8_aux(int tier, const DfnFrame* frame, const void* packed_head, const void* packed_torso,
                          const float* bias_head, const float* bias_torso, const float* bg_f32, const uint8_t* bg_u8,
                          const int32_t* pix_index, uint8_t* rgb8_head, uint8_t* rgb8_com, uint8_t* alpha8_head,
                          uint8_t* alpha8_com, uint16_t* depth16_head, uint16_t* depth16_com, void* stream);

int dfn_render_rays_fwd(int tier, const DfnFrame* frame, const void* packed_head, const void* packed_torso,
                        const float* bias_head, const float* bias_torso, const float* rays, const float* bounds,
                        const float* bg_f32, const uint8_t* bg_u8, float* rgb_head, float* rgb_com, float* weights_head,
                        float* weights_com, float* z_vals, void* stream);
int dfn_render_rays_fwd_u8(int tier, const DfnFrame* frame, const void* packed_head, const void* packed_torso,
                           const float* bias_head, const float* bias_torso, const float* rays, const float* bounds,
                           const float* bg_f32, const uint8_t* bg_u8, uint8_t* rgb8_head, uint8_t* rgb8_com, void* stream);

long dfn_train_rows(int field, int what);
#define DFN_TRAIN_ACT_E4M3 0x100
long dfn_packed_bwd_bytes(int tier, int field);
int dfn_pack_weights_bwd(int tier, int field, const float* params, void* packed_T, void* stream);

int dfn_train_prepare(int tier, const float* params, const float* signal_head, const float* signal_torso,
                      const float* z_shape, const float* z_app, void* packed_head, void* packed_torso, void* packed_T_head,
                      void* packed_T_torso, float* bias_head, float* bias_torso, void* stream);
int dfn_train_fwd(int tier, const DfnFrame* frame, const void* packed_head, const void* packed_torso,
                  const float* bias_head, const float* bias_torso, const float* bg_f32, const uint8_t* bg_u8,
                  const int32_t* pix_index, float* rgb_head, float* rgb_com, float* samples, void* act_head,
                  uint32_t* masks_head, void* act_torso, uint32_t* masks_torso, void* stream);
int dfn_train_fwd_hier(int tier, const DfnFrame* frame, const void* packed_head, const void* packed_torso,
                       const float* bias_head, const float* bias_torso, const float* bg_f32, const uint8_t* bg_u8,
                       const int32_t* pix_index, float* rgb_head, float* rgb_com, float* samples, void* act_head,
                       uint32_t* masks_head, void* act_torso, uint32_t* masks_torso, float* z_all, uint8_t* ranks,
                       void* stream);
int dfn_composite_bwd_hier(const DfnFrame* frame, const int32_t* pix_index, const float* bg_f32, const uint8_t* bg_u8,
                           const float* samples, const float* z_all, const uint8_t* ranks, const float* d_rgb_head,
                           const float* d_rgb_com, float* dsamples, void* stream);
int dfn_sample_pixels(int H, int W, int n, int rect_num, const int32_t* rect, uint64_t seed, uint64_t counter,
                      int32_t* pix_index, int32_t* status, void* stream);

int dfn_mse_loss_u8(const float* rgb_head, const float* rgb_com, const uint8_t* img_head, const uint8_t* img_com,
                    const int32_t* pix_index, int n, float* losses, float* d_rgb_head, float* d_rgb_com, void* stream);
typedef struct DfnTrainLoss {
    const uint8_t* img_head;
    const uint8_t* img_com;
    float* d_rgb_head;
    float* d_rgb_com;
    float* losses;
    float* workspace;
} DfnTrainLoss;
long dfn_train_loss_floats(int ray_count);
int dfn_train_fwd_loss(int tier, const DfnFrame* frame, const void* packed_head, const void* packed_torso,
                       const float* bias_head, const float* bias_torso, const float* bg_f32, const uint8_t* bg_u8,
                       const int32_t* pix_index, float* rgb_head, float* rgb_com, float* samples, void* act_head,
                       uint32_t* masks_head, void* act_torso, uint32_t* masks_torso, const DfnTrainLoss* loss, void* stream);
int dfn_train_fwd_hier_loss(int tier, const DfnFrame* frame, const void* packed_head, const void* packed_torso,
                            const float* bias_head, const float* bias_torso, const float* bg_f32, const uint8_t* bg_u8,
                            const int32_t* pix_index, float* rgb_head, float* rgb_com, float* samples, void* act_head,
                            uint32_t* masks_head, void* act_torso, uint32_t* masks_torso, float* z_all, uint8_t* ranks,
                            const DfnTrainLoss* loss, void* stream);
int dfn_composite_bwd(const DfnFrame* frame, const int32_t* pix_index, const float* bg_f32, const uint8_t* bg_u8,
                      const float* samples, const float* d_rgb_head, const float* d_rgb_com, float* dsamples,
                      void* stream);
int dfn_composite_bwd_z(const DfnFrame* frame, const int32_t* pix_index, const float* bg_f32, const uint8_t* bg_u8,
                        const float* samples, const float* d_rgb_head, const float* d_rgb_com, float* dsamples,
                        float* zero_buf, long zero_floats, void* stream);
int dfn_composite_bwd_hier_z(const DfnFrame* frame, const int32_t* pix_index, const float* bg_f32, const uint8_t* bg_u8,
                             const float* samples, const float* z_all, const uint8_t* ranks, const float* d_rgb_head,
                             const float* d_rgb_com, float* dsamples, float* zero_buf, long zero_floats, void* stream);
int dfn_mlp_bwd(int tier, int field, const void* packed_T, const float* samples, const float* dsamples,
                const uint32_t* masks, long NP, void* dy_T, void* stream);
long dfn_wgrad_plan(int field, int what, int32_t* out, long capacity);
int dfn_weight_grad(int tier, int field, const void* dy_T, const void* act_T, long NP, float* workspace,
                    float* grad_flat, void* stream);
int dfn_bias_grad(int tier, int field, const void* dy_T, long NP, float* workspace, float* dbias, void* stream);
int dfn_weight_bias_grad(int tier, int field, const void* dy_T, const void* act_T, long NP, float* workspace,
                         float* grad_flat, float* dbias, void* stream);
#define DFN_ACT_E4M3 0
#define DFN_ACT_E2M1 1
int dfn_weight_bias_grad_fmt(int tier, int field, int act_format, const void* dy_T, const void* act_T, long NP, float* workspace,
                             float* grad_flat, float* dbias, void* stream);
int dfn_weight_bias_grad_partials(int tier, int field, int act_format, const void* dy_T, const void* act_T, long NP,
                                  float* workspace, float* dbias, void* stream);
int dfn_weight_bias_grad_reduce(int tier, int field, long NP, float* workspace, float* grad_flat, float* dbias, void* stream);
int dfn_weight_bias_grad_partials_part(int tier, int field, int act_format, const void* dy_T, const void* act_T, long NP,
                                       float* workspace, float* dbias, int which, void* stream);
int dfn_fold_bias_bwd(int tier, int field, const float* params, const float* signal, const float* z_shape,
                      const float* z_app, const float* dbias, float* grad_flat, float* d_signal, void* stream);

int dfn_signal_grad(int tier, int field, const float* params, const void* dy_T, long NP, float* workspace, float* d_signal,
                    void* stream);

int dfn_zero_async(void* p, long bytes, void* stream);

#define DFN_ADAM_CHUNK 2048
typedef struct DfnAdamItem {
    float* param;
    const float* grad;
    float* exp_avg;
    float* exp_avg_sq;
    long n;
} DfnAdamItem;
int dfn_adam_multi(const DfnAdamItem* items_dev, const int32_t* chunks_dev, int n_chunks, float lr, double beta1,
                   double beta2, float eps, float bias_c1, float bias_c2_sqrt, void* stream);

int dfn_decoder_fwd(int tier, int field, const void* packed, const float* bias, const float* points,
                    const float* dirs, long n, float* feat, float* sigma, void* stream);

int dfn_decoder_train_fwd(int tier, int field, const void* packed, const float* bias, const float* points,
                          const float* dirs, long n, float* feat, float* sigma, float* samples, void* act_T,
                          uint32_t* masks, void* stream);

int dfn_get_rays(int H, int W, float focal, float cx, float cy, const float* c2w_host, float* rays_o,
                 float* rays_d, void* stream);
int dfn_get_rays_strided(int H, int W, int stride, float focal, float cx, float cy, const float* c2w_host, float* rays_o,
                         float* rays_d, void* stream);
int dfn_ndc_rays(int H, int W, float focal, float z_near, const float* rays_o, const float* rays_d, long n,
                 float* out_o, float* out_d, void* stream);
int dfn_sample_pdf(const float* bins, const float* weights, long R, int nb, int ns, const float* u,
                   float* samples, void* stream);
int dfn_composite(const float* sigma, const float* feat, int K, long N, float* sigma_sum, float* feat_w,
                  void* stream);
int dfn_volume_weights(const float* z, const float* ray, const float* sigma, long R, int S,
                       float last_dist, float* weights, void* stream);
int dfn_composite_grad(const float* sigma, const float* feat, int K, long N, const float* d_sigma_sum, const float* d_feat_w,
                       float* d_sigma, float* d_feat, void* stream);
int dfn_volume_weights_grad(const float* z, const float* ray, const float* sigma, long R, int S, float last_dist,
                            const float* d_weights, float* d_sigma, void* stream);
int dfn_to8b(const float* x, long n, uint8_t* out, void* stream);

int dfn_debug_mfma_layout(float* out, void* stream);
int dfn_debug_mfma_chain(int tier, int lds_reads_per_2, int valu_per_2, const void* fragments, const void* operands_b, int iters,
                         int blocks, float* out, uint64_t* clock, void* stream);
int dfn_debug_clock_probe(uint64_t* probe);

#ifdef __cplusplus
}
#endif
#endif
```

Baseline: 5.940 million rays/s.

## Switch f16 inference tier MLP to 16x16x32 MFMA with permuted LDS layout

Moves the f16 tier's GEMMs from the 32x32 MFMA fragment layout to the 16x16x32 f16 MFMA instruction. Weight fragments are DMA'd into LDS with an XOR-permuted lane order and read as fragment pairs. Bias init, posenc, output extraction and lane-half mapping are adapted to the new accumulator layout. The aim is higher MFMA throughput and fewer LDS bank conflicts on the inference path, at the cost of extra layout complexity and a probe/map API for checking it.

```diff
diff --git a/dfa-nerf_amd/csrc/dfn_api.hip b/dfa-nerf_amd/csrc/dfn_api.hip
--- a/dfa-nerf_amd/csrc/dfn_api.hip
+++ b/dfa-nerf_amd/csrc/dfn_api.hip
@@ -1103,6 +1103,24 @@
     return DFN_OK;
 }
 
+long dfn_mfma16_map(int32_t* out, long capacity) {
+    constexpr long N = 1024;
+    if (out) {
+        if (capacity < N) return fail(DFN_E_SIZE, "dfn_mfma16_map: capacity too small");
+        for (int lane = 0; lane < 64; ++lane) {
+            out[lane] = (int32_t)m16_dma_off(lane);
+            for (int j = 0; j < 4; ++j) out[64 + 64 * j + lane] = (int32_t)m16_lane_off(lane, 2) + m16_read_off(j, 2);
+            for (int T = 0; T < 2; ++T) out[320 + 64 * T + lane] = (int32_t)m16_lane_off(lane, 1) + m16_read_off(T, 1);
+            for (int e = 0; e < 8; ++e) out[448 + 8 * lane + e] = m16_feat(lane >> 4, e);
+            out[960 + lane] = 8 * m16_bias_oct(lane);
+        }
+    }
+    return N;
+}
+int dfn_debug_mfma16_layout(float* out, void* stream) {
+    if (!out) return fail(DFN_E_ARG, "dfn_debug_mfma16_layout: bad argument");
+    return launched(launch_mfma16_probe(out, (hipStream_t)stream), "mfma16_probe_kernel");
+}
 int dfn_debug_mfma_layout(float* out, void* stream) {
     if (!out) return fail(DFN_E_ARG, "dfn_debug_mfma_layout: bad argument");
     return launched(launch_mfma_probe(out, (hipStream_t)stream), "mfma_probe_kernel");
diff --git a/dfa-nerf_amd/csrc/dfn_layout.h b/dfa-nerf_amd/csrc/dfn_layout.h
--- a/dfa-nerf_amd/csrc/dfn_layout.h
+++ b/dfa-nerf_amd/csrc/dfn_layout.h
@@ -38,6 +38,27 @@
     const int t = u / UPT, r = (u % UPT) * E + e;
     return 32 * t + tile_feat(h, r);
 }
+
+#ifndef DFN_F16_LDS_PERM
+#define DFN_F16_LDS_PERM 1
+#endif
+DFN_HD constexpr bool tier_m16(int tier) { return tier == TIER_F16; }
+DFN_HD constexpr int m16_row(int i, int T) { return (i & 7) + 16 * (i >> 3) + 8 * T; }
+DFN_HD constexpr int m16_feat(int g, int e) { return (e & 3) + 8 * (e >> 2) + 4 * (g & 1) + 16 * (g >> 1); }
+constexpr int M16_T_BYTES = DFN_F16_LDS_PERM ? 256 : 128;
+DFN_HD constexpr unsigned m16_dma_off(int lane) {
+    const unsigned x = (DFN_F16_LDS_PERM != 0) ? ((((unsigned)lane >> 3) ^ ((unsigned)lane >> 4)) & 1u) : 0u;
+    return ((unsigned)lane ^ (x * 0x18u)) * 16u;
+}
+DFN_HD constexpr unsigned m16_lane_off(int lane, int G) {
+    const unsigned i = lane & 15, g = (unsigned)lane >> 4;
+    const unsigned slot = (DFN_F16_LDS_PERM != 0) ? i : (i & 7) + 16 * (i >> 3);
+    return (g >> 1) * (unsigned)(G * FRAG_BYTES) + (g & 1) * 512u + slot * 16u;
+}
+DFN_HD constexpr int m16_read_off(int pos, int G) {
+    return (G == 2 ? (pos & ~3) + ((pos >> 1) & 1) : (pos & ~1)) * FRAG_BYTES + (pos & 1) * M16_T_BYTES;
+}
+DFN_HD constexpr int m16_bias_oct(int lane) { return 2 * ((lane >> 4) & 1) + (lane >> 5); }
 
 constexpr int HID = 256, ZDIM = 256, NPE = 60, NPEV = 24, NSIG = 96, NET = 42, DH = 64;
 
diff --git a/dfa-nerf_amd/csrc/dfn_misc.h b/dfa-nerf_amd/csrc/dfn_misc.h
--- a/dfa-nerf_amd/csrc/dfn_misc.h
+++ b/dfa-nerf_amd/csrc/dfn_misc.h
@@ -37,6 +37,7 @@
                              unsigned long long* clk, hipStream_t st);
 hipError_t launch_to8b(const float* x, long n, unsigned char* out, hipStream_t st);
 hipError_t launch_mfma_probe(float* out, hipStream_t st);
+hipError_t launch_mfma16_probe(float* out, hipStream_t st);
 hipError_t launch_adam_multi(const DfnAdamItem* items, const void* chunks, int n_chunks, float lr, double beta1, double beta2,
                              float eps, float bias_c1, float bias_c2_sqrt, hipStream_t st);
 }
diff --git a/dfa-nerf_amd/csrc/dfn_misc.hip b/dfa-nerf_amd/csrc/dfn_misc.hip
--- a/dfa-nerf_amd/csrc/dfn_misc.hip
+++ b/dfa-nerf_amd/csrc/dfn_misc.hip
@@ -686,6 +686,22 @@
     hipLaunchKernelGGL(mfma_probe_kernel, dim3(1), dim3(64), 0, st, out);
     return hipGetLastError();
 }
+__global__ void mfma16_probe_kernel(float* out) {
+    const int lane = threadIdx.x, i = lane & 15, g = lane >> 4;
+    f16x8 a, b;
+    for (int e = 0; e < 8; ++e) {
+        const int k = 8 * g + e;
+        a[e] = (_Float16)(float)((7 * i + 3 * k) % 13 + 1);
+        b[e] = (_Float16)(float)((5 * k + 11 * i) % 17 + 1);
+    }
+    f32x4 d = {0.f, 0.f, 0.f, 0.f};
+    d = __builtin_amdgcn_mfma_f32_16x16x32_f16(a, b, d, 0, 0, 0);
+    for (int j = 0; j < 4; ++j) out[(4 * g + j) * 16 + i] = d[j];
+}
+hipError_t launch_mfma16_probe(float* out, hipStream_t st) {
+    hipLaunchKernelGGL(mfma16_probe_kernel, dim3(1), dim3(64), 0, st, out);
+    return hipGetLastError();
+}
 
 
 __global__ __launch_bounds__(256) void adam_multi_kernel(const DfnAdamItem* items, const int2* chunks, float lr, float beta2,
diff --git a/dfa-nerf_amd/csrc/dfn_mlp.h b/dfa-nerf_amd/csrc/dfn_mlp.h
--- a/dfa-nerf_amd/csrc/dfn_mlp.h
+++ b/dfa-nerf_amd/csrc/dfn_mlp.h
@@ -36,6 +36,11 @@
 
 constexpr int RING_SLOTS = 3;
 constexpr int RING_BYTES = RING_SLOTS * SLAB_BYTES;
+
+template <int TIER> DFN_DEV size_t dma_lane_off(int lane) {
+    if constexpr (tier_m16(TIER)) return m16_dma_off(lane);
+    else return (size_t)lane * 16;
+}
 
 template <int TIER, int NT> struct Vec;
 template <int NT> struct Vec<TIER_BF16, NT> {
@@ -92,11 +97,11 @@
         const unsigned dst = __builtin_amdgcn_readfirstlane((unsigned)(unsigned long)ring + s.pf_slot * SLAB_BYTES +
                                                             (unsigned)f * FRAG_BYTES);
         const gchar_c* sb = (const gchar_c*)(s.pf_ptr + f * FRAG_BYTES);
-        const unsigned voff = (unsigned)lane * 16u;
+        const unsigned voff = (unsigned)dma_lane_off<TIER>(lane);
         asm volatile("s_mov_b32 m0, %2\n\ts_nop 0\n\tglobal_load_lds_dwordx4 %0, %1" ::"v"(voff), "s"(sb), "s"(dst) : "memory", "m0");
     } else {
         __builtin_amdgcn_global_load_lds(
-            (const __attribute__((address_space(1))) void*)(s.pf_ptr + (size_t)lane * 16 + f * FRAG_BYTES),
+            (const __attribute__((address_space(1))) void*)(s.pf_ptr + (size_t)dma_lane_off<TIER>(lane) + f * FRAG_BYTES),
             (DFN_LDS void*)(ring + s.pf_slot * SLAB_BYTES + f * FRAG_BYTES), 16, 0, 0);
     }
 }
@@ -168,7 +173,11 @@
 #endif
     s.rd_slot = (s.rd_slot + 1 == RING_SLOTS) ? 0u : s.rd_slot + 1;
     s.rd_off = s.rd_slot * SLAB_BYTES;
-    s.rd_vaddr = (unsigned)(unsigned long)ring + (unsigned)lane * 16u + s.rd_off;
+    if constexpr (tier_m16(TIER)) {
+        int l = lane;
+        asm volatile("" : "+v"(l));
+        s.rd_vaddr = (unsigned)(unsigned long)ring + m16_lane_off(l, 2) + s.rd_off;
+    } else s.rd_vaddr = (unsigned)(unsigned long)ring + (unsigned)lane * 16u + s.rd_off;
     s.pf_owed += C::LOADS_PER_SLAB;
 }
 
@@ -436,6 +445,25 @@
     }
 }
 #undef DFN_FRAG_CASE
+#define DFN_FRAG_CASE(K)                                                                                      \
+    case 2 * (K):                                                                                             \
+        asm volatile("ds_read_b128 %0, %1 offset:%2" : "=v"(dst) : "v"(vaddr), "n"((K) * FRAG_BYTES) : "memory"); \
+        break;                                                                                                \
+    case 2 * (K) + 1:                                                                                         \
+        asm volatile("ds_read_b128 %0, %1 offset:%2" : "=v"(dst) : "v"(vaddr), "n"((K) * FRAG_BYTES + M16_T_BYTES) : "memory"); \
+        break;
+DFN_DEV void frag_read16(u32x4& dst, unsigned vaddr, int code) {
+    switch (code) {
+        DFN_FRAG_CASE(0) DFN_FRAG_CASE(1) DFN_FRAG_CASE(2) DFN_FRAG_CASE(3) DFN_FRAG_CASE(4) DFN_FRAG_CASE(5)
+        DFN_FRAG_CASE(6) DFN_FRAG_CASE(7) DFN_FRAG_CASE(8) DFN_FRAG_CASE(9) DFN_FRAG_CASE(10) DFN_FRAG_CASE(11)
+        DFN_FRAG_CASE(12) DFN_FRAG_CASE(13) DFN_FRAG_CASE(14) DFN_FRAG_CASE(15) DFN_FRAG_CASE(16) DFN_FRAG_CASE(17)
+        DFN_FRAG_CASE(18) DFN_FRAG_CASE(19) DFN_FRAG_CASE(20) DFN_FRAG_CASE(21) DFN_FRAG_CASE(22) DFN_FRAG_CASE(23)
+        DFN_FRAG_CASE(24) DFN_FRAG_CASE(25) DFN_FRAG_CASE(26) DFN_FRAG_CASE(27) DFN_FRAG_CASE(28) DFN_FRAG_CASE(29)
+        DFN_FRAG_CASE(30) DFN_FRAG_CASE(31)
+        default: __builtin_unreachable();
+    }
+}
+#undef DFN_FRAG_CASE
 DFN_DEV void frag_wait(u32x4& r, int younger) {
     switch (younger) {
         case 0: asm volatile("s_waitcnt lgkmcnt(0)" : "+v"(r)); break;
@@ -457,14 +485,24 @@
 template <int TIER> struct Fetch {
     u32x4 buf[PF_DEPTH];
     template <class CT> DFN_DEV void load(int slot, int fp, Stream& s, const CT& c) { load(slot, fp, s, c, NoHook{}); }
-    template <class CT, class H> DFN_DEV void load(int slot, int fp, Stream& s, const CT& c, H&& hook) {
+    template <class CT, class H> DFN_DEV void load(int slot, int fp, Stream& s, const CT& c, H&& hook, int gl = 2) {
         using C = TierCfg<TIER>;
         constexpr int GAP = SLAB_FRAGS / C::LOADS_PER_SLAB;
         if (fp % SLAB_FRAGS == 0) {
             slab_advance<TIER>(s, c.ring, c.wave, c.lane);
             hook();
         }
-        if constexpr (use_asm_fetch<TIER, CT>()) frag_read(buf[slot], s.rd_vaddr, fp % SLAB_FRAGS);
+        if constexpr (tier_m16(TIER)) {
+            const int off = m16_read_off(fp % SLAB_FRAGS, gl);
+            unsigned vaddr = s.rd_vaddr;
+            if (gl != 2) {
+                unsigned l = (unsigned)c.lane;
+                asm volatile("" : "+v"(l));
+                vaddr -= (l >> 5) << 10;
+            }
+            if constexpr (use_asm_fetch<TIER, CT>()) frag_read16(buf[slot], vaddr, 2 * (off / FRAG_BYTES) + (off % FRAG_BYTES != 0));
+            else buf[slot] = *(const lds_u32x4*)(c.ring + m16_lane_off(c.lane, gl) + s.rd_off + off);
+        } else if constexpr (use_asm_fetch<TIER, CT>()) frag_read(buf[slot], s.rd_vaddr, fp % SLAB_FRAGS);
         else buf[slot] = *(const lds_u32x4*)(c.ring + c.lane * 16 + s.rd_off + (fp % SLAB_FRAGS) * FRAG_BYTES);
 #ifdef DFN_EXP_DBLLDS
         {
@@ -487,10 +525,56 @@
     }
 };
 
-template <int TIER, int G, int KU, int NTB, int TAIL = -1, class CT, class H = NoHook, class SD = NoSide>
+template <int TIER, int G, int KU, int NTB, int TAIL = -1, int GN = G, class CT, class H = NoHook, class SD = NoSide>
 DFN_DEV void gemm_group(f32x16 (&acc)[G], const Vec<TIER, NTB>& b, int& f, Fetch<TIER>& fe, Stream& s,
                         const CT& c, H&& hook = H{}, SD&& side = SD{}) {
-    if constexpr (TIER == TIER_F16X3) {
+    if constexpr (tier_m16(TIER)) {
+        static_assert(KU % 2 == 0 && (G == 1 || G == 2) && PF_DEPTH == 4, "K = 32 steps are fragment pairs; the ring holds one quad");
+        static_assert(!CT::rec_on, "the f16 tier is inference only: no recorder for the 16x16x32 layout");
+        static_assert(GN <= G, "a two-tile group behind a one-tile group: the ring would have read its first fragments as a pair");
+        constexpr bool ASM = use_asm_fetch<TIER, CT>();
+#pragma unroll
+        for (int v = 0; v < KU / 2; ++v) {
+#pragma unroll
+            for (int g = 0; g < G; ++g) {
+#pragma unroll
+                for (int T = 0; T < 2; ++T) {
+                    const int left = (KU / 2 - v) * 2 * G - 2 * g - T - 1;
+                    if constexpr (ASM) {
+                        const int after = (TAIL < 0) ? PF_DEPTH : left + TAIL;
+                        frag_wait(fe.buf[f % PF_DEPTH], after < PF_DEPTH - 1 ? after : PF_DEPTH - 1);
+                    }
+                    const f16x8 a = __builtin_bit_cast(f16x8, fe.buf[f % PF_DEPTH]);
+                    if constexpr (!ASM) {
+                        if (TAIL < 0 || left + TAIL >= PF_DEPTH) fe.load(f % PF_DEPTH, f + PF_DEPTH, s, c, hook, left >= PF_DEPTH ? G : GN);
+                    }
+#pragma unroll
+                    for (int P = 0; P < 2; ++P) {
+                        const int o = 8 * P + 4 * T;
+                        f32x4 d = {acc[g][o], acc[g][o + 1], acc[g][o + 2], acc[g][o + 3]};
+                        d = __builtin_amdgcn_mfma_f32_16x16x32_f16(a, b.u[2 * v + P], d, 0, 0, 0);
+#pragma unroll
+                        for (int j = 0; j < 4; ++j) acc[g][o + j] = d[j];
+                    }
+                    if constexpr (ASM) {
+                        if (TAIL < 0 || left + TAIL >= PF_DEPTH) fe.load(f % PF_DEPTH, f + PF_DEPTH, s, c, hook, left >= PF_DEPTH ? G : GN);
+                    }
+#ifdef DFN_GEMM_SCHEDBAR
+                    if constexpr (!ASM) __builtin_amdgcn_sched_barrier(DFN_GEMM_SCHEDBAR);
+#endif
+                    ++f;
+                }
+                if (G == 2) side(2 * v + g);
+            }
+            if (G == 1) {
+                side(2 * v);
+                side(2 * v + 1);
+            }
+#ifdef DFN_PIPE_SCHEDBAR
+            if constexpr (!std::is_same<typename std::decay<SD>::type, NoSide>::value) __builtin_amdgcn_sched_barrier(0);
+#endif
+        }
+    } else if constexpr (TIER == TIER_F16X3) {
         constexpr int D = PF_DEPTH;
         f32x16 accx[G];
 #pragma unroll
@@ -574,7 +658,7 @@
 
 DFN_DEV float relu_(float x) { return __builtin_bit_cast(float, max(__builtin_bit_cast(int, x), 0)); }
 
-template <int G>
+template <int G, bool M16 = false>
 DFN_DEV void acc_init(f32x16 (&acc)[G], const lds_f32* bias_lds, int half) {
 #ifdef DFN_EXP_NOINIT
 #pragma unroll
@@ -585,23 +669,23 @@
 #endif
 #pragma unroll
     for (int g = 0; g < G; ++g) {
-        const lds_f32x4* p = (const lds_f32x4*)(bias_lds + g * 32 + half * 16);
+        const lds_f32x4* p = (const lds_f32x4*)(bias_lds + g * 32 + half * (M16 ? 8 : 16));
 #pragma unroll
         for (int q = 0; q < 4; ++q) {
-            const f32x4 v = p[q];
+            const f32x4 v = p[M16 ? (q & 1) : q];
 #pragma unroll
             for (int e = 0; e < 4; ++e) acc[g][4 * q + e] = v[e];
         }
     }
 }
-template <int G>
+template <int G, bool M16 = false>
 DFN_DEV void acc_relu_add(f32x16 (&acc)[G], const lds_f32* bias_lds, int half) {
 #pragma unroll
     for (int g = 0; g < G; ++g) {
-        const lds_f32x4* p = (const lds_f32x4*)(bias_lds + g * 32 + half * 16);
+        const lds_f32x4* p = (const lds_f32x4*)(bias_lds + g * 32 + half * (M16 ? 8 : 16));
 #pragma unroll
         for (int q = 0; q < 4; ++q) {
-            const f32x4 v = p[q];
+            const f32x4 v = p[M16 ? (q & 1) : q];
 #pragma unroll
             for (int e = 0; e < 4; ++e) acc[g][4 * q + e] = relu_(acc[g][4 * q + e]) + v[e];
         }
@@ -742,9 +826,10 @@
     q[e] = word;
     v.u[2 * (t0 + g) + h] = __builtin_bit_cast(pk8, q);
 }
+template <bool M16 = false>
 DFN_DEV void init_quad(f32x16 (&acc)[2], const lds_f32* bias_lds, int half, int q) {
     const int g = q >> 2, qq = q & 3;
-    const f32x4 v = ((const lds_f32x4*)(bias_lds + g * 32 + half * 16))[qq];
+    const f32x4 v = ((const lds_f32x4*)(bias_lds + g * 32 + half * (M16 ? 8 : 16)))[M16 ? (qq & 1) : qq];
 #pragma unroll
     for (int e = 0; e < 4; ++e) acc[g][4 * qq + e] = v[e];
 }
@@ -765,7 +850,7 @@
         if (bias_next && ku >= ES) {
 #pragma unroll
             for (int q = 0; q < QPS; ++q)
-                if ((ku - ES) * QPS + q < 8) init_quad(other, bias_next, half, (ku - ES) * QPS + q);
+                if ((ku - ES) * QPS + q < 8) init_quad<tier_m16(TIER)>(other, bias_next, half, (ku - ES) * QPS + q);
         }
     }
 };
@@ -774,14 +859,14 @@
                         Stream& s, const CT& c) {
     static_assert(OT % 2 == 0 && KU >= 2, "tile pairs");
     f32x16 acc[2][2];
-    acc_init<2>(acc[0], bias, c.half);
+    acc_init<2, tier_m16(TIER)>(acc[0], bias, c.half);
 #pragma unroll
     for (int tg = 0; tg < OT / 2; ++tg) {
         const int cur = tg & 1;
         const PipeSide<TIER, OT, KU, RELU> side = {acc[cur ^ 1], out, tg + 1 < OT / 2 ? bias + (tg + 1) * 64 : nullptr,
                                                    tg > 0 ? 2 * (tg - 1) : -1, c.half};
         gemm_group<TIER, 2, KU, NTB>(acc[cur], in, f, fe, s, c, NoHook{}, side);
-        if (KU - PipeSide<TIER, OT, KU, RELU>::ES < 1 && tg + 1 < OT / 2) acc_init<2>(acc[cur ^ 1], bias + (tg + 1) * 64, c.half);
+        if (KU - PipeSide<TIER, OT, KU, RELU>::ES < 1 && tg + 1 < OT / 2) acc_init<2, tier_m16(TIER)>(acc[cur ^ 1], bias + (tg + 1) * 64, c.half);
     }
     acc_to_vec<TIER, 2, OT, RELU>(acc[(OT / 2 - 1) & 1], out, OT - 2);
 }
@@ -854,7 +939,7 @@
 #pragma unroll
         for (int tg = 0; tg < OT / 2; ++tg) {
             f32x16 acc[2];
-            acc_init<2>(acc, bias + tg * 64, c.half);
+            acc_init<2, tier_m16(TIER)>(acc, bias + tg * 64, c.half);
             bits = 0;
             gemm_group<TIER, 2, KU, NTB>(acc, in, f, fe, s, c, NoHook{},
                                          RecSide32<OT, KU, CT>{c, out, rec_row, (rec_mask < 0 || tg == 0) ? -1 : rec_mask + tg - 1, tg - 1, bits});
@@ -869,7 +954,7 @@
 #pragma unroll
     for (int tg = 0; tg < OT / 2; ++tg) {
         f32x16 acc[2];
-        acc_init<2>(acc, bias + tg * 64, c.half);
+        acc_init<2, tier_m16(TIER)>(acc, bias + tg * 64, c.half);
         if constexpr (SPREAD) {
             gemm_group<TIER, 2, KU, NTB>(acc, in, f, fe, s, c, NoHook{}, RecSide<TIER, OT, KU, CT, RELU>{c, out, rec_row, tg - 1, {}});
         } else {
@@ -895,14 +980,14 @@
 #pragma unroll
     for (int tg = 0; tg < OT / 2; ++tg) {
         f32x16 acc[2];
-        acc_init<2>(acc, bias + tg * 64, c.half);
+        acc_init<2, tier_m16(TIER)>(acc, bias + tg * 64, c.half);
         auto flush = [&] {
             if (pend) rec_vals<TIER>(c, rec_row + 64 * (tg - 1), out, 2 * (tg - 1));
             pend = false;
         };
         gemm_group<TIER, 2, KU, NTB>(acc, in, f, fe, s, c, flush);
         rec_mask_pair(c, mask_dword0 < 0 ? -1 : mask_dword0 + tg, acc);
-        acc_relu_add<2>(acc, bias2 + tg * 64, c.half);
+        acc_relu_add<2, tier_m16(TIER)>(acc, bias2 + tg * 64, c.half);
         gemm_group<TIER, 2, KU2, NTB2>(acc, in2, f, fe, s, c, flush);
         flush();
         acc_to_vec<TIER, 2, OT, false>(acc, out, 2 * tg);
@@ -950,6 +1035,59 @@
         }
         const bool ok = half ? ok1 : ok0;
         v.set(L, ok ? val : 0.f);
+    }
+}
+
+template <int NT, int NCOL>
+DFN_DEV void posenc16(Vec<TIER_F16, NT>& v, const float (&p0)[3], const float (&p1)[3], int lane) {
+    const bool g0 = (lane & 16) != 0, g1 = (lane & 32) != 0;
+    const float ph[2][3] = {{p0[0] * 0.5f, p0[1] * 0.5f, p0[2] * 0.5f}, {p1[0] * 0.5f, p1[1] * 0.5f, p1[2] * 0.5f}};
+#pragma unroll
+    for (int L = 0; L < 16 * NT; ++L) {
+        const int P = (L >> 3) & 1, e = L & 7;
+        const int base = 32 * (L >> 4) + 8 * (e >> 2) + (e & 3);
+        float r[4], q[4];
+        bool ok[4];
+#pragma unroll
+        for (int k = 0; k < 4; ++k) {
+            const int col = base + 4 * (k & 1) + 16 * (k >> 1);
+            ok[k] = col < NCOL;
+            const int o = ok[k] ? col / 6 : 0, a = ok[k] ? (col % 6) % 3 : 0;
+            r[k] = ph[P][a] * ((float)(1 << o) * 0.5f);
+            q[k] = (ok[k] && (col % 6) >= 3) ? 0.25f : 0.f;
+        }
+        if (!ok[0] && !ok[1] && !ok[2] && !ok[3]) {
+            v.set(L, 0.f);
+            continue;
+        }
+        const float rr = g1 ? (g0 ? r[3] : r[2]) : (g0 ? r[1] : r[0]);
+        const float qq = g1 ? (g0 ? q[3] : q[2]) : (g0 ? q[1] : q[0]);
+        const bool okk = g1 ? (g0 ? ok[3] : ok[2]) : (g0 ? ok[1] : ok[0]);
+        const float val = __builtin_amdgcn_sinf(__builtin_amdgcn_fractf(rr) + qq);
+        v.set(L, okk ? val : 0.f);
+    }
+}
+DFN_DEV void m16_pair(const float (&x)[3], int lane, float (&x0)[3], float (&x1)[3]) {
+    const bool up = (lane & 16) != 0;
+#pragma unroll
+    for (int k = 0; k < 3; ++k) {
+        const float o = __shfl_xor(x[k], 16);
+        x0[k] = up ? o : x[k];
+        x1[k] = up ? x[k] : o;
+    }
+}
+DFN_DEV float m16_out(const f32x16& acc, int j, int lane) {
+    const float o = __shfl_xor(acc[8 + j], 16);
+    return (lane & 16) ? o : acc[j];
+}
+template <int TIER, int NT, int NCOL>
+DFN_DEV void posenc_of(Vec<TIER, NT>& v, const float (&p)[3], int half, int lane) {
+    if constexpr (tier_m16(TIER)) {
+        float p0[3], p1[3];
+        m16_pair(p, lane, p0, p1);
+        posenc16<NT, NCOL>(v, p0, p1, lane);
+    } else {
+        posenc<TIER, NT, NCOL>(v, p, half);
     }
 }
 
@@ -1063,7 +1201,7 @@
         Vec<TIER, 1> vview;
         float dhat[3];
         dref.load(dhat);
-        posenc<TIER, 1, NPEV>(vview, dhat, c.half);
+        posenc_of<TIER, 1, NPEV>(vview, dhat, c.half, c.lane);
         rec_vec<TIER, 1>(c, r_trunk + RecMap::T_VIEW, vview);
         bool pend = false;
         int ptg = 0;
@@ -1074,9 +1212,14 @@
 #pragma unroll
         for (int tg = 0; tg < HT / 2; ++tg) {
             f32x16 acc[2];
-            acc_init<2>(acc, bias + b_view + tg * 64, c.half);
+            acc_init<2, tier_m16(TIER)>(acc, bias + b_view + tg * 64, c.half);
             gemm_group<TIER, 2, P::KU_ACT, HT>(acc, a7, f, fe, s, c, flush);
-            gemm_group<TIER, 2, P::KU_VIEW, 1>(acc, vview, f, fe, s, c, flush);
+            if constexpr (tier_m16(TIER)) {
+                if (tg == HT / 2 - 1) gemm_group<TIER, 2, P::KU_VIEW, 1, -1, 1>(acc, vview, f, fe, s, c, flush);
+                else gemm_group<TIER, 2, P::KU_VIEW, 1>(acc, vview, f, fe, s, c, flush);
+            } else {
+                gemm_group<TIER, 2, P::KU_VIEW, 1>(acc, vview, f, fe, s, c, flush);
+            }
             flush();
             acc_to_vec<TIER, 2, HT, true>(acc, hid, 2 * tg);
             if constexpr (tier_is16(TIER)) rec_mask_pair_packed<TIER, HT>(c, m_trunk + RecMap::TM_H + tg, hid, 2 * tg);
@@ -1085,19 +1228,26 @@
             ptg = tg;
         }
         f32x16 acc1[1];
-        acc_init<1>(acc1, bias + b_view + 256, c.half);
+        acc_init<1, tier_m16(TIER)>(acc1, bias + b_view + 256, c.half);
         gemm_group<TIER, 1, P::KU_ACT, HT>(acc1, a7, f, fe, s, c, flush);
         gemm_group<TIER, 1, P::KU_VIEW, 1>(acc1, vview, f, fe, s, c, flush);
         flush();
-        o.sigma = acc1[0][0];
+        if constexpr (tier_m16(TIER)) o.sigma = m16_out(acc1[0], 0, c.lane);
+        else o.sigma = acc1[0][0];
     }
     {
         f32x16 acc1[1];
-        acc_init<1>(acc1, bias + b_out, c.half);
+        acc_init<1, tier_m16(TIER)>(acc1, bias + b_out, c.half);
         gemm_group<TIER, 1, P::KU_ACT, HT, 0>(acc1, hid, f, fe, s, c);
-        o.r = sigmoidf_(acc1[0][0]);
-        o.g = sigmoidf_(acc1[0][1]);
-        o.b = sigmoidf_(acc1[0][2]);
+        if constexpr (tier_m16(TIER)) {
+            o.r = sigmoidf_(m16_out(acc1[0], 0, c.lane));
+            o.g = sigmoidf_(m16_out(acc1[0], 1, c.lane));
+            o.b = sigmoidf_(m16_out(acc1[0], 2, c.lane));
+        } else {
+            o.r = sigmoidf_(acc1[0][0]);
+            o.g = sigmoidf_(acc1[0][1]);
+            o.b = sigmoidf_(acc1[0][2]);
+        }
     }
     return o;
 }
@@ -1107,7 +1257,7 @@
                         const CT& c) {
     using P = Prog<TIER, HT>;
     Vec<TIER, 2> pe;
-    posenc<TIER, 2, NPE>(pe, p, c.half);
+    posenc_of<TIER, 2, NPE>(pe, p, c.half, c.lane);
     rec_vec<TIER, 2>(c, RecMap::H_PE, pe);
     Vec<TIER, HT> act;
     int f = 0;
@@ -1124,7 +1274,7 @@
                          const CT& c) {
     using P = Prog<TIER, HT>;
     Vec<TIER, 2> pe;
-    posenc<TIER, 2, NPE>(pe, p, c.half);
+    posenc_of<TIER, 2, NPE>(pe, p, c.half, c.lane);
     rec_vec<TIER, 2>(c, RecMap::S_PE, pe);
     Vec<TIER, 2> ve, vs, vn;
     int f = 0;
@@ -1142,10 +1292,10 @@
     ve = vn;
     {
         f32x16 acc[2];
-        acc_init<2>(acc, bias + P::T_B_S3, c.half);
+        acc_init<2, tier_m16(TIER)>(acc, bias + P::T_B_S3, c.half);
         gemm_group<TIER, 2, P::KU_D, 2>(acc, vs, f, fe, s, c);
         rec_mask_pair(c, RecMap::S_MD0 + 7, acc);
-        acc_relu_add<2>(acc, bias + P::T_B_SSKIP, c.half);
+        acc_relu_add<2, tier_m16(TIER)>(acc, bias + P::T_B_SSKIP, c.half);
         acc_to_vec<TIER, 2, 2, false>(acc, vn, 0);
         rec_vals<TIER>(c, RecMap::S_D0 + 64 * 7, vn, 0);
         vs = vn;
@@ -1156,11 +1306,11 @@
     Vec<TIER, 4> pd;
     {
         f32x16 acc[2];
-        acc_init<2>(acc, bias + P::T_B_EO, c.half);
+        acc_init<2, tier_m16(TIER)>(acc, bias + P::T_B_EO, c.half);
         gemm_group<TIER, 2, P::KU_D, 2>(acc, ve, f, fe, s, c);
 #pragma unroll
         for (int L = 0; L < 32; ++L) pd.set(L, acc[L >> 4][L & 15] + pe.get(L));
-        acc_init<2>(acc, bias + P::T_B_SO, c.half);
+        acc_init<2, tier_m16(TIER)>(acc, bias + P::T_B_SO, c.half);
         gemm_group<TIER, 2, P::KU_D, 2>(acc, vs, f, fe, s, c);
 #pragma unroll
         for (int L = 0; L < 32; ++L) pd.set(32 + L, acc[L >> 4][L & 15]);
diff --git a/dfa-nerf_amd/csrc/dfn_render_kernels.h b/dfa-nerf_amd/csrc/dfn_render_kernels.h
--- a/dfa-nerf_amd/csrc/dfn_render_kernels.h
+++ b/dfa-nerf_amd/csrc/dfn_render_kernels.h
@@ -122,7 +122,7 @@
 #define DFN_PIPE_TWO_HEAD 1
 #endif
     typedef CtxT<TRAIN != 0, TRAIN == 0, TRAIN != 0, (DFN_PIPE != 0) && TRAIN == 0 && (!TWO || DFN_PIPE_TWO != 0), TRAIN != 0 && ACT4> CtxK;
-    CtxK ctx = {lds, wave, lane, lane >> 5, {}};
+    CtxK ctx = {lds, wave, lane, tier_m16(TIER) ? m16_bias_oct(lane) : lane >> 5, {}};
     typedef CtxT<TRAIN != 0, TRAIN == 0, TRAIN != 0, (DFN_PIPE != 0) && TRAIN == 0 && (!TWO || DFN_PIPE_TWO != 0 || DFN_PIPE_TWO_HEAD != 0), TRAIN != 0 && ACT4> CtxH;
     constexpr bool two = TWO;
     const int NF = TRAIN == 1 ? 0 : F.n_fine;
@@ -680,7 +680,7 @@
     const int n = lane & 31;
     lds_char* lds = (lds_char*)smem;
     typedef CtxT<REC, HT != 8, REC> CtxD;
-    CtxD ctx = {lds, wave, lane, lane >> 5, {}};
+    CtxD ctx = {lds, wave, lane, tier_m16(TIER) ? m16_bias_oct(lane) : lane >> 5, {}};
     ctx.rec.act_T = nullptr;
     ctx.rec.masks = nullptr;
 
diff --git a/dfa-nerf_amd/dfanerf/_lib.py b/dfa-nerf_amd/dfanerf/_lib.py
--- a/dfa-nerf_amd/dfanerf/_lib.py
+++ b/dfa-nerf_amd/dfanerf/_lib.py
@@ -77,6 +77,8 @@
         "dfn_volume_weights_grad": (i32, [fp, fp, fp, lg, i32, C.c_float, fp, fp, vp]),
         "dfn_to8b": (i32, [fp, lg, vp, vp]),
         "dfn_debug_mfma_layout": (i32, [fp, vp]),
+        "dfn_mfma16_map": (lg, [ip, lg]),
+        "dfn_debug_mfma16_layout": (i32, [fp, vp]),
         "dfn_debug_clock_probe": (i32, [vp]),
         "dfn_debug_mfma_chain": (i32, [i32, i32, i32, vp, vp, i32, i32, fp, vp, vp]),
         "dfn_train_rows": (lg, [i32, i32]),
@@ -109,7 +111,12 @@
         "dfn_signal_grad": (i32, [i32, i32, fp, vp, lg, fp, fp, vp]),
     }
     for name, (res, args) in sig.items():
-        fn = getattr(lib, name)
+        try:
+            fn = getattr(lib, name)
+        except AttributeError:
+            if not (os.environ.get("DFN_LIB") and name in ("dfn_mfma16_map", "dfn_debug_mfma16_layout")):
+                raise
+            continue
         fn.restype = res
         fn.argtypes = args
     if b"DEV" in lib.dfn_version() and not os.environ.get("DFN_LIB"):
@@ -127,6 +134,15 @@
     return rc
 
 
+def mfma16_map():
+    import numpy as np
+    n = check(lib.dfn_mfma16_map(None, 0), "dfn_mfma16_map")
+    t = np.empty(n, np.int32)
+    check(lib.dfn_mfma16_map(t.ctypes.data, n), "dfn_mfma16_map")
+    return {"dma": t[:64].copy(), "rd2": t[64:320].reshape(4, 64).copy(), "rd1": t[320:448].reshape(2, 64).copy(),
+            "feat": t[448:960].reshape(64, 8).copy(), "bias": t[960:1024].copy()}
+
+
 def pack_plan(tier, field):
     import numpy as np
     n = check(lib.dfn_pack_plan(tier, field, None, 0), "dfn_pack_plan")
diff --git a/dfa-nerf_amd/dfanerf/engine.py b/dfa-nerf_amd/dfanerf/engine.py
--- a/dfa-nerf_amd/dfanerf/engine.py
+++ b/dfa-nerf_amd/dfanerf/engine.py
@@ -484,6 +484,12 @@
     return out
 
 
+def mfma16_layout_probe(device="cuda"):
+    out = torch.zeros(16, 16, dtype=torch.float32, device=device)
+    check(lib.dfn_debug_mfma16_layout(_ptr(out), _stream()), "dfn_debug_mfma16_layout")
+    return out
+
+
 def mfma_layout_probe(device="cuda"):
     out = torch.zeros(3, 32, 32, dtype=torch.float32, device=device)
     check(lib.dfn_debug_mfma_layout(_ptr(out), _stream()), "dfn_debug_mfma_layout")
diff --git a/include/dfanerf.h b/include/dfanerf.h
--- a/include/dfanerf.h
+++ b/include/dfanerf.h
@@ -216,6 +216,8 @@
 int dfn_to8b(const float* x, long n, uint8_t* out, void* stream);
 
 int dfn_debug_mfma_layout(float* out, void* stream);
+long dfn_mfma16_map(int32_t* out, long capacity);
+int dfn_debug_mfma16_layout(float* out, void* stream);
 int dfn_debug_mfma_chain(int tier, int lds_reads_per_2, int valu_per_2, const void* fragments, const void* operands_b, int iters,
                          int blocks, float* out, uint64_t* clock, void* stream);
 int dfn_debug_clock_probe(uint64_t* probe);
```

Result: faster. 6.062 million rays/s, median of 6 (+2.1%).
